# ucbrise/graphtrans

Hardware: AMD Instinct MI355X
Metric: graphs/sec (fwd+bwd) OGBG-Code2 GCN-Virtual b256 (higher is better)
Workload: dtype fp32+bf16; 1 GPU; OGBG-Code2-like synthetic, GraphTrans GCN-Virtual L5 D300 JK=cat cls norm_input, 4 enc layers d128; mode=mixed, graphs_per_gpu=256, global_batch=256, avg_nodes_per_batch=31598, avg_edges_per_batch=87502, parallelism=dp1, step=zero_grad+graph_prep+fwd+loss+bwd+allreduce+AdamW

## Files before the change

### graphtrans_amd/_lib.py

```python
import ctypes as C
import os

import torch

_HERE = os.path.dirname(os.path.abspath(__file__))
LIB_PATH = os.environ.get("GT_LIB_PATH") or os.path.join(_HERE, "libgraphtrans_hip.so")

GT_F32, GT_BF16 = 0, 1
GT_COMPUTE_F32_HIGH = 2
GT_CONV_GCN, GT_CONV_GIN = 0, 1
GT_EDGE_NONE, GT_EDGE_LINEAR, GT_EDGE_TABLES, GT_EDGE_DENSE = 0, 1, 2, 3

_p = C.c_void_p
_i64 = C.c_int64
_i = C.c_int
_f = C.c_float
_sz = C.c_size_t
_u64 = C.c_uint64
_d = C.c_double

SIGNATURES = {
    "gt_version": (_i, []),
    "gt_last_error": (C.c_char_p, []),
    "gt_option_set": (_i, [C.c_char_p, _i]),
    "gt_option_get": (_i, [C.c_char_p]),
    "gt_profile_enable": (_i, [C.c_uint]),
    "gt_profile_resume": (_i, [C.c_uint]),
    "gt_profile_count": (_i64, []),
    "gt_profile_get": (_i, [_i64, C.c_char_p, _i64, C.POINTER(C.c_float), C.POINTER(C.c_int64)]),
    "gt_attr_rank": (_i, [_p, _i64, _p, _p]),
    "gt_collate_workspace_bytes": (_sz, [_i64]),
    "gt_collate": (_i, [_p, _p, _i64, _i64, _i64, _p, _p, _sz, _p]),
    "gt_graph_prep_workspace_bytes": (_sz, [_i64, _i64, _i64]),
    "gt_graph_prep": (_i, [_p, _p, _i64, _i64, _i64, _p, _p, _p, _p, _p, _p, _p, _p, _p, _p, _p, _p, _sz, _p]),
    "gt_aggregate_fwd": (_i, [_i, _i, _i, _p, _i64, _i64, _i64, _p, _p, _p, _p, _p, _p, _p, _i64, _p, _p,
                              C.POINTER(C.c_int32), _i64, _p, _p, _p]),
    "gt_aggregate_bwd_workspace_bytes": (_sz, [_i, _i, _i64, _i64, _i64]),
    "gt_aggregate_bwd": (_i, [_i, _i, _i, _p, _p, _i64, _i64, _i64, _p, _p, _p, _p, _p, _p, _p, _i64, _p, _p,
                              C.POINTER(C.c_int32), _i64, _p, _p, _p, _p, _p, _p, _p, _sz, _p]),
    "gt_pna_aggregate_fwd": (_i, [_p, _p, _i64, _i64, _i, _p, _p, _p, _p, _p, _p, _p]),
    "gt_pna_aggregate_bwd": (_i, [_p, _p, _p, _p, _p, _i64, _i64, _i, _p, _p, _p, _p, _p, _p, _p]),
    "gt_scale_combine_fwd": (_i, [_p, _p, _i64, _i, _i, _i, _p, _p]),
    "gt_scale_combine_bwd": (_i, [_p, _p, _i64, _i, _i, _i, _p, _p]),
    "gt_embed_sum_fwd": (_i, [_i, _p, _p, _p, _p, _i64, _i64, _p, _p]),
    "gt_embed_sum_bwd_workspace_bytes": (_sz, [_i, _p, _i64]),
    "gt_embed_sum_bwd": (_i, [_i, _p, _p, _p, _p, _p, _i64, _i64, _p, _p, _sz, _p]),
    "gt_embed_sort_plan_bytes": (_sz, [_i, _p, _i64]),
    "gt_embed_sort_workspace_bytes": (_sz, [_i, _p, _i64]),
    "gt_embed_sort": (_i, [_i, _p, _p, _p, _p, _i64, _p, _sz, _p, _sz, _p]),
    "gt_embed_sum_bwd_sorted_workspace_bytes": (_sz, [_i, _i64, _i64]),
    "gt_embed_sum_bwd_sorted": (_i, [_i, _p, _p, _i64, _i64, _p, _p, _p, _sz, _p]),
    "gt_segment_bcast_add": (_i, [_i, _p, _p, _p, _i64, _i64, _i64, _p, _p]),
    "gt_segment_sum": (_i, [_i, _p, _p, _p, _i64, _i64, _i64, _p, _p]),
    "gt_seq_layout_packed": (_i, [_p, _i64, _i64, _i, _p, _p, _p, _i64, _p, _p]),
    "gt_segment_sum_workspace_bytes": (_sz, [_i64, _i64]),
    "gt_segment_sum_ws": (_i, [_i, _p, _p, _p, _i64, _i64, _i64, _p, _p, _sz, _p]),
    "gt_seq_gather": (_i, [_i, _p, _p, _p, _p, _i64, _i64, _i64, _i, _i64, _p, _p, _p]),
    "gt_seq_scatter": (_i, [_i, _p, _p, _p, _p, _p, _i64, _i64, _i, _i64, _i64, _p, _p, _p]),
    "gt_batchnorm_workspace_bytes": (_sz, [_i64, _i64]),
    "gt_batchnorm_fwd": (_i, [_i, _p, _p, _p, _p, _p, _p, _f, _f, _i, _i, _p, _i64, _i64, _p, _p, _p, _f, _u64, _p, _sz, _p]),
    "gt_batchnorm_apply": (_i, [_i, _p, _p, _p, _p, _p, _i, _p, _i64, _i64, _p, _f, _u64, _p]),
    "gt_batchnorm_bwd_apply": (_i, [_i, _p, _p, _p, _p, _p, _p, _p, _p, _d, _i, _i64, _i64, _p, _f, _u64, _p]),
    "gt_batchnorm_fwd_bcast": (_i, [_i, _p, _p, _p, _p, _p, _p, _f, _f, _i, _i, _p, _p, _p, _p, _i64, _i64, _p, _p, _p, _f, _u64, _p, _sz, _p]),
    "gt_batchnorm_bwd": (_i, [_i, _p, _p, _p, _p, _p, _p, _i, _i, _i64, _i64, _p, _p, _p, _f, _u64, _p, _sz, _p]),
    "gt_layernorm_fwd": (_i, [_i, _p, _p, _p, _p, _f, _f, _u64, _i64, _i64, _p, _p, _p, _p]),
    "gt_layernorm_bwd_workspace_bytes": (_sz, [_i64, _i64]),
    "gt_layernorm_bwd": (_i, [_i, _p, _p, _p, _p, _p, _p, _f, _u64, _i64, _i64, _p, _p, _p, _p, _p, _sz, _p]),
    "gt_linear_fwd": (_i, [_i, _i, _i, _p, _p, _p, _p, _i64, _i64, _i64, _i, _f, _u64, _p]),
    "gt_colsum_rows_f32": (_i, [_i, _p, _p, _i64, _i64, _p, _p]),
    "gt_seq_token_rows_layernorm": (_i, [_i, _p, _p, _p, _p, _i64, _i64, _i, _i64, _i64, _p, _p, _p, _p, _f, _p, _p, _p, _p]),
    "gt_seq_token_rows": (_i, [_i, _p, _p, _p, _p, _i64, _i64, _i, _i64, _i64, _p, _p, _p]),
    "gt_defer_begin": (_i, [_p, _sz]),
    "gt_defer_limit": (_i, [_sz]),
    "gt_defer_take": (_p, [_sz]),
    "gt_defer_push": (_i, [_p, _i, _i64, _i64, _p, _p, _i64, _i64, _p]),
    "gt_defer_push_strided": (_i, [_p, _i, _i64, _i64, _p, _i64]),
    "gt_defer_room": (_i, [_i]),
    "gt_defer_flush": (_i, [_p]),
    "gt_defer_end": (_i, []),
    "gt_linear_rows_ok": (_i, [_i, _i, _i, _p, _i64, _i64, _i64]),
    "gt_linear_products": (_i, [_i, _i, _i, _i, _p, _i64, _i64, _i64]),
    "gt_linear_set_rows": (_i, [_p]),
    "gt_linear_rows_layernorm_ok": (_i, [_i64]),
    "gt_linear_set_rows_layernorm": (_i, [_p, _p, _p, _f, _p, _p, _p]),
    "gt_linear_fwd_ld": (_i, [_i, _i, _i, _p, _p, _p, _p, _i64, _i64, _i64, _i64, _i, _f, _u64, _p]),
    "gt_linear_bwd_ld": (_i, [_i, _i, _i, _p, _p, _p, _p, _p, _p, _p, _p, _p, _i64, _i64, _i64, _i64, _f, _p, _sz, _p]),
    "gt_adamw_chunk_elems": (_i, []),
    "gt_adamw_step": (_i, [_p, _p, _p, _i64, _i64, _i, _i, _p, _f, _f, _f, _f, _f, _i64, _p, _p]),
    "gt_grad_sqnorm": (_i, [_p, _p, _p, _i64, _i64, _i, _i, _p, _p, _p]),
    "gt_grad_clip_coef": (_i, [_p, _i64, _f, _p, _p]),
    "gt_linear_fwd_gelu": (_i, [_i, _i, _i, _p, _p, _p, _p, _p, _i64, _i64, _i64, _i64, _i64, _f, _u64, _p]),
    "gt_linear_bwd_mul": (_i, [_i, _i, _i, _p, _p, _p, _p, _p, _p, _p, _p, _p, _i64, _i64, _i64, _i64, _i64, _p, _sz, _p]),
    "gt_stream_create": (_p, [_i]),
    "gt_stream_destroy": (None, [_p]),
    "gt_stream_priority_range": (_i, [C.POINTER(_i), C.POINTER(_i)]),
    "gt_linear_bwd_dw_forked": (_i, [_i, _i, _i, _p, _p, _p, _p, _p, _p, _i64, _i64, _i64, _i64, _i64, _f, _p, _sz, _p]),
    "gt_linear_bwd_mul_dw_forked": (_i, [_i, _i, _i, _p, _p, _p, _p, _p, _p, _i64, _i64, _i64, _i64, _i64, _p, _sz, _p]),
    "gt_linear_bwd_wt": (_i, [_i, _i, _i, _p, _p, _p, _p, _p, _p, _p, _p, _p, _p, _i64, _i64, _i64, _f, _p, _sz, _p]),
    "gt_transpose": (_i, [_p, _p, _i64, _i64, _p]),
    "gt_bn_sync_set": (_i, [_p, _p, _i]),
    "gt_vn_update_bwd_dt0": (_p, [_p, _p]),
    "gt_linear_bwd_bcast_ok": (_i, [_i, _i, _i, _p, _i64, _i64, _i64]),
    "gt_linear_bwd_bcast": (_i, [_p, _p]),
    "gt_linear_cat2_ok": (_i, [_i, _p, _i64, _i64, _i64, _i64]),
    "gt_linear_fwd_cat2": (_i, [_i, _i, _p, _i64, _i64, _p, _i64, _i64, _p, _p, _p, _i64, _i64, _i64, _p]),
    "gt_linear_bwd_cat2": (_i, [_i, _i, _p, _i64, _i64, _p, _i64, _i64, _p, _p, _p, _i64, _p, _i64, _p, _p, _i64, _i64, _i64, _p, _sz, _p]),
    "gt_w3_image_bytes": (_sz, [_i64, _i64]),
    "gt_w3_images": (_i, [_i, _p, _p, _p, _p, _p, _p]),
    "gt_w3_bind": (_i, [_i, _p, _p, _p, _p, _p]),
    "gt_w3_unbind": (_i, []),
    "gt_w1_image_bytes": (_sz, [_i64, _i64]),
    "gt_w1_images": (_i, [_i, _p, _p, _p, _p, _p, _p]),
    "gt_w1_bind": (_i, [_i, _p, _p, _p, _p, _p]),
    "gt_w1_unbind": (_i, []),
    "gt_linear_layernorm_fwd_ok": (_i, [_i, _i, _p, _i64, _i64, _i64]),
    "gt_linear_bwd_dx_layernorm_ok": (_i, [_i, _i, _p, _i64, _i64, _i64]),
    "gt_linear_bwd_dx_layernorm_workspace_bytes": (_sz, [_i64, _i64, _i64]),
    "gt_linear_bwd_dx_layernorm": (_i, [_i, _i, _p, _p, _p, _p, _i64, _i64, _i64, _p, _p, _p, _p, _p, _f, _u64, _p, _p, _p, _p, _p, _sz, _p]),
    "gt_layernorm_bwd_finish": (_i, [_p, _i, _i64, _p, _p, _p]),
    "gt_linear_layernorm_fwd": (_i, [_i, _i, _p, _p, _p, _p, _i64, _i64, _i64, _p, _p, _p, _f, _f, C.c_uint64, _p, _p, _p, _p]),
    "gt_linear_bwd_gate_out_ok": (_i, [_i, _i, _i, _p, _i64, _i64, _i64]),
    "gt_linear_bwd_gate_out": (_i, [_i, _i, _i, _p, _p, _p, _p, _p, _p, _p, _p, _p, _i64, _i64, _i64, _i64, _i64, _f, _p, _sz, _p]),
    "gt_dropout": (_i, [_i, _p, _p, _i64, _f, _u64, _p]),
    "gt_linear_bwd_bnstats_ok": (_i, [_i, _i, _i, _i64]),
    "gt_linear_bwd_bnstats_rows": (_i64, [_i64]),
    "gt_linear_bwd_bnstats_rows_for": (_i64, [_i, _i, _i, _p, _i64, _i64, _i64]),
    "gt_linear_bwd_bnstats": (_i, [_p, _i64, _p, _p, _p, _p, _i, _p]),
    "gt_batchnorm_bwd_parts": (_i, [_i, _p, _p, _p, _p, _p, _p, _i, _i, _i64, _i64, _p, _p, _p, _p, _i64, _p]),
    "gt_overlap_dw_begin": (_i, [_p, _p]),
    "gt_overlap_dw_sync": (_i, []),
    "gt_overlap_dw_release": (_i, [_p, _sz]),
    "gt_overlap_dw_urgent": (_i, [_i]),
    "gt_overlap_dw_fork": (_p, [_p, C.c_uint]),
    "gt_overlap_dw_booked": (None, [_p, _sz]),
    "gt_overlap_dw_end": (_i, []),
    "gt_linear_fwd_ld2": (_i, [_i, _i, _i, _p, _p, _p, _p, _i64, _i64, _i64, _i64, _i64, _i, _f, _u64, _p]),
    "gt_linear_fwd_grouped": (_i, [_i, _i, _i, _p, _p, _p, _p, _i64, _i64, _i64, _i64, _i64, _i, _i64, _i64, _i, _f, _u64, _p]),
    "gt_linear_bwd_grouped_workspace_bytes": (_sz, [_i, _i64, _i64, _i64, _i]),
    "gt_linear_bwd_grouped": (_i, [_i, _i, _i, _p, _p, _p, _p, _p, _p, _p, _p, _p, _i64, _i64, _i64, _i64, _i64, _i, _i64, _i64, _f,
                                   _p, _sz, _p]),
    "gt_linear_bwd_ld2": (_i, [_i, _i, _i, _p, _p, _p, _p, _p, _p, _p, _p, _p, _i64, _i64, _i64, _i64, _i64, _f, _p, _sz, _p]),
    "gt_xent_fwd": (_i, [_p, _i64, _i64, _i64, _i64, _p, _i64, _p, _p, _p, _p, _p]),
    "gt_xent_bwd": (_i, [_p, _p, _p, _p, _i64, _p, _i64, _i64, _i64, _i64, _p, _p]),
    "gt_bce_masked_fwd": (_i, [_p, _p, _i64, _i64, _i64, _i64, _p, _p, _p, _p, _p]),
    "gt_bce_masked_bwd": (_i, [_p, _p, _p, _p, _i64, _i64, _i64, _i64, _p, _p]),
    "gt_linear_bwd_workspace_bytes": (_sz, [_i, _i64, _i64, _i64]),
    "gt_linear_bwd": (_i, [_i, _i, _i, _p, _p, _p, _p, _p, _p, _p, _p, _p, _i64, _i64, _i64, _f, _p, _sz, _p]),
    "gt_encoder_layer_saved_bytes": (_sz, [_p]),
    "gt_encoder_layer_workspace_bytes": (_sz, [_p]),
    "gt_encoder_layer_grad_elems": (_i64, [_p]),
    "gt_encoder_layer_fwd": (_i, [_p, _p, _p, _p, _p]),
    "gt_encoder_layer_bwd": (_i, [_p, _p, _p, _p, _p, _p, _p, _sz, _p]),
    "gt_gcn_layer_saved_bytes": (_sz, [_p]),
    "gt_gcn_layer_workspace_bytes": (_sz, [_p]),
    "gt_gcn_layer_grad_elems": (_i64, [_p]),
    "gt_gcn_layer_fwd": (_i, [_p, _p, _p, _p, _p, _p, _p, _sz, _p]),
    "gt_gcn_layer_bwd": (_i, [_p, _p, _p, _p, _p, _p, _p, _p, _p, _sz, _p]),
    "gt_vn_update_saved_bytes": (_sz, [_p]),
    "gt_vn_update_workspace_bytes": (_sz, [_p]),
    "gt_vn_update_grad_elems": (_i64, [_p]),
    "gt_vn_update_fwd": (_i, [_p, _p, _p, _p, _p, _p, _sz, _p]),
    "gt_vn_update_bwd": (_i, [_p, _p, _p, _p, _p, _p, _p, _p, _sz, _p]),
    "gt_event_create": (_p, []),
    "gt_event_destroy": (None, [_p]),
    "gt_event_record": (_i, [_p, _p]),
    "gt_stream_wait_event": (_i, [_p, _p]),
    "gt_gin_layer_saved_bytes": (_sz, [_p]),
    "gt_gin_layer_workspace_bytes": (_sz, [_p]),
    "gt_gin_layer_grad_elems": (_i64, [_p]),
    "gt_gin_layer_fwd": (_i, [_p, _p, _p, _p, _p, _p, _p, _sz, _p]),
    "gt_gin_layer_bwd": (_i, [_p, _p, _p, _p, _p, _p, _p, _p, _p, _sz, _p]),
    "gt_add3": (_i, [_p, _p, _p, _i64, _p, _p]),
    "gt_copy2d": (_i, [_p, _i64, _p, _i64, _i64, _i64, _p]),
    "gt_repitch": (_i, [_p, _i64, _p, _i64, _i64, _i, _p]),
    "gt_rows_gather": (_i, [_i, _p, _p, _i64, _i64, _p, _p]),
    "gt_rows_scatter": (_i, [_i, _p, _p, _i64, _i64, _i64, _p, _p]),
    "gt_seq_layout_packed_host": (_i, [_p, _i64, _i64, _i, _p, _sz, _p]),
    "gt_pna_layer_saved_bytes": (_sz, [_p]),
    "gt_pna_layer_workspace_bytes": (_sz, [_p]),
    "gt_pna_layer_grad_elems": (_i64, [_p]),
    "gt_pna_layer_fwd": (_i, [_p, _p, _p, _p, _p, _sz, _p]),
    "gt_pna_layer_bwd": (_i, [_p, _p, _p, _p, _p, _p, _p, _sz, _p]),
    "gt_pna_scales": (_i, [_p, _i64, _i, _p, _f, _f, _p, _p]),
    "gt_gather_f32": (_i, [_p, _p, _p, _i64, _p]),
    "gt_pna_aggregate_fwd_uv": (_i, [_p, _p, _i64, _i64, _i, _p, _p, _p, _p, _p, _p, _p]),
    "gt_pna_aggregate_bwd_uv": (_i, [_p, _p, _p, _p, _p, _i64, _i64, _i, _p, _p, _p, _p, _p, _p, _p]),
    "gt_rows_take": (_i, [_i, _p, _p, _i64, _i64, _p, _p]),
    "gt_rows_put": (_i, [_i, _p, _p, _i64, _i64, _i64, _p, _p]),
    "gt_rows_add": (_i, [_i, _p, _p, _i64, _i64, _p, _p]),
    "gt_attn_fwd_last": (_i, [_i, _p, _p, _p, _i64, _i64, _i, _p, _i64, _i64, _i64, _f, _f, _u64, _p]),
    "gt_attn_bwd_last": (_i, [_i, _p, _p, _p, _p, _p, _p, _i64, _i64, _i, _p, _i64, _i64, _i64, _p, _i64, _f, _f, _u64, _p]),
    "gt_encoder_layer_pooled_saved_bytes": (_sz, [_p]),
    "gt_encoder_layer_pooled_workspace_bytes": (_sz, [_p]),
    "gt_encoder_layer_pooled_fwd": (_i, [_p, _p, _p, _p, _p, _p]),
    "gt_encoder_layer_pooled_bwd": (_i, [_p, _p, _p, _p, _p, _p, _p, _p, _sz, _p]),
    "gt_model_ctx_bytes": (_sz, []),
    "gt_model_abi_sizes": (_i, [_p]),
    "gt_model_grad_ranges": (_i, [_p, _p, _p]),
    "gt_model_prepare": (_i, [_p, _p, _p, _p]),
    "gt_model_forward": (_i, [_p, _p, _p, _p, _p]),
    "gt_model_backward": (_i, [_p, _p, _p, _p, _p, _i, _p]),
    "gt_seq_gather_cls32": (_i, [_i, _p, _p, _p, _p, _i64, _i64, _i64, _i, _i64, _p, _p]),
    "gt_colsum_f32": (_i, [_i, _p, _i64, _i64, _p, _p]),
    "gt_attn_head_dim_ok": (_i, [_i, _i64, _i]),
    "gt_attn_fwd": (_i, [_i, _p, _p, _p, _i64, _i64, _i, _p, _i64, _i64, _i64, _p, _i64, _p, _p, _f, _f, _f, _u64, _p]),
    "gt_attn_bwd": (_i, [_i, _p, _p, _p, _p, _p, _p, _i64, _i64, _i, _p, _i64, _i64, _i64, _p, _i64, _p, _p, _f, _f, _f,
                         _u64, _p]),
}

_lib = None


def lib():
    global _lib
    if _lib is None:
        if not os.path.exists(LIB_PATH):
            raise RuntimeError(
                f"{LIB_PATH} is missing: build it with `python -m graphtrans_amd.build` "
                "(graphtrans_amd has no CPU or eager fallback)")
        h = C.CDLL(LIB_PATH)
        for name, (res, args) in SIGNATURES.items():
            try:
                fn = getattr(h, name)
            except AttributeError:
                if not os.environ.get("GT_LIB_PATH"):
                    raise
                continue
            fn.restype = res
            fn.argtypes = args
        if os.environ.get("GT_F32_GEMM", "split") == "exact":
            h.gt_option_set(b"attn_f32_exact", 1)
        _lib = h
    return _lib


class KernelTimer:

    def __init__(self, names):
        self.names = set(names)
        self.records = []

    def summary(self):
        torch.cuda.synchronize()
        out = {}
# ... 66 lines not shown
```

### graphtrans_amd/csrc/common.hip

```cpp
#include <stdarg.h>
#include <atomic>
#include <mutex>
#include <string.h>

#include "gt_common.h"

static thread_local char g_err[512] = "";

void gt_set_error(const char* fmt, ...) {
  va_list ap;
  va_start(ap, fmt);
  vsnprintf(g_err, sizeof(g_err), fmt, ap);
  va_end(ap);
}

extern "C" int gt_version(void) { return 100;  }
extern "C" const char* gt_last_error(void) { return g_err; }

#include <mutex>
#include <vector>

namespace {
struct ProfRecord {
  const char* name;
  hipEvent_t e0, e1;
  int64_t dims[6];
};
std::mutex g_prof_mu;
std::vector<ProfRecord> g_prof;
std::vector<hipEvent_t> g_pool;
size_t g_pool_next = 0;
unsigned g_prof_mask = 0;
constexpr size_t POOL_EVENTS = 16384;
}

unsigned gt_prof_mask() { return g_prof_mask; }

int64_t gt_prof_begin(const char* name, hipStream_t stream, const int64_t* dims, int ndims) {
  ProfRecord r{};
  r.name = name;
  for (int i = 0; i < 6; ++i) r.dims[i] = i < ndims ? dims[i] : 0;
  std::lock_guard<std::mutex> lk(g_prof_mu);
  if (g_pool_next + 2 > g_pool.size()) return -1;
  r.e0 = g_pool[g_pool_next++];
  r.e1 = g_pool[g_pool_next++];
  (void)hipEventRecord(r.e0, stream);
  g_prof.push_back(r);
  return (int64_t)g_prof.size() - 1;
}

void gt_prof_end(int64_t id, hipStream_t stream) {
  if (id < 0) return;
  std::lock_guard<std::mutex> lk(g_prof_mu);
  if ((size_t)id < g_prof.size()) (void)hipEventRecord(g_prof[id].e1, stream);
}

namespace {
std::atomic<int> g_options[GT_OPT_COUNT];
const char* const OPTION_NAMES[GT_OPT_COUNT] = {"attn_f32_exact", "bnstats_rows_kernel", "lin_ring"};
int option_id(const char* name) {
  if (name)
    for (int i = 0; i < GT_OPT_COUNT; ++i)
      if (strcmp(name, OPTION_NAMES[i]) == 0) return i;
  return -1;
}
}
int gt_opt(int id) { return g_options[id].load(std::memory_order_relaxed); }
extern "C" int gt_option_set(const char* name, int value) {
  const int id = option_id(name);
  if (id < 0) { gt_set_error("gt_option_set: unknown option '%s'", name ? name : "(null)"); return GT_ERR_INVALID_ARG; }
  return g_options[id].exchange(value < 0 ? 0 : value);
}
extern "C" int gt_option_get(const char* name) {
  const int id = option_id(name);
  if (id < 0) { gt_set_error("gt_option_get: unknown option '%s'", name ? name : "(null)"); return GT_ERR_INVALID_ARG; }
  return gt_opt(id);
}

extern "C" int gt_profile_enable(unsigned mask) {
  std::lock_guard<std::mutex> lk(g_prof_mu);
  if (mask) {
    g_prof.clear();
    g_pool_next = 0;
    while (g_pool.size() < POOL_EVENTS) {
      hipEvent_t e;
      if (hipEventCreate(&e) != hipSuccess) break;
      g_pool.push_back(e);
    }
  }
  g_prof_mask = mask;
  return GT_OK;
}

extern "C" int gt_profile_resume(unsigned mask) {
  std::lock_guard<std::mutex> lk(g_prof_mu);
  g_prof_mask = mask;
  return GT_OK;
}

extern "C" int64_t gt_profile_count(void) {
  std::lock_guard<std::mutex> lk(g_prof_mu);
  return (int64_t)g_prof.size();
}

extern "C" int gt_profile_get(int64_t i, char* name_out, int64_t name_cap, float* ms, int64_t* dims6) {
  std::lock_guard<std::mutex> lk(g_prof_mu);
  if (i < 0 || (size_t)i >= g_prof.size() || !name_out || !ms || !dims6) return GT_ERR_INVALID_ARG;
  const ProfRecord& r = g_prof[i];
  snprintf(name_out, (size_t)name_cap, "%s", r.name);
  if (hipEventElapsedTime(ms, r.e0, r.e1) != hipSuccess) return GT_ERR_LAUNCH;
  for (int k = 0; k < 6; ++k) dims6[k] = r.dims[k];
  return GT_OK;
}


extern "C" void* gt_stream_create(int level) {
  int least = 0, greatest = 0;
  (void)hipDeviceGetStreamPriorityRange(&least, &greatest);
  const int prio = level < 0 ? greatest : (level > 0 ? least : 0);
  hipStream_t st = nullptr;
  if (hipStreamCreateWithPriority(&st, hipStreamNonBlocking, prio) != hipSuccess) return nullptr;
  return st;
}
extern "C" void gt_stream_destroy(void* stream) {
  if (stream) (void)hipStreamDestroy((hipStream_t)stream);
}
extern "C" int gt_stream_priority_range(int* least, int* greatest) {
  return hipDeviceGetStreamPriorityRange(least, greatest) == hipSuccess ? GT_OK : GT_ERR_LAUNCH;
}

extern "C" void* gt_event_create(void) {
  hipEvent_t ev = nullptr;
  if (hipEventCreateWithFlags(&ev, hipEventDisableTiming) != hipSuccess) return nullptr;
  return ev;
}
extern "C" void gt_event_destroy(void* event) {
  if (event) (void)hipEventDestroy((hipEvent_t)event);
}
extern "C" int gt_event_record(void* event, gt_stream_t stream) {
  GT_CHECK_ARG(event, "null event");
  if (hipEventRecord((hipEvent_t)event, (hipStream_t)stream) != hipSuccess) { gt_set_error("gt_event_record failed"); return GT_ERR_LAUNCH; }
  return GT_OK;
// ... 7 lines not shown
```

### graphtrans_amd/csrc/gt_common.h

```cpp
#pragma once
#include <hip/hip_runtime.h>
#ifdef GT_DEBUG_SKIP
#include <cstdlib>
#include <cstring>
static inline bool gt_dbg_skip(const char* kernel) {
  static const char* e = getenv("GT_SKIP");
  if (!e || !*e) return false;
  const char* p = e;
  while (*p) {
    const char* q = strchr(p, ',');
    const size_t n = q ? (size_t)(q - p) : strlen(p);
    char buf[128];
    if (n > 0 && n < sizeof(buf)) {
      memcpy(buf, p, n);
      buf[n] = 0;
      if (strstr(kernel, buf)) return true;
    }
    if (!q) break;
    p = q + 1;
  }
  return false;
}
static __global__ void gt_dbg_empty_kernel() {}
static inline bool gt_dbg_empty() {
  static const bool on = [] { const char* e = getenv("GT_EMPTY"); return e && *e && *e != '0'; }();
  return on;
}
#undef hipLaunchKernelGGL
#define hipLaunchKernelGGL(k, g, b, l, s, ...)                                                              \
  do {                                                                                                      \
    if (gt_dbg_empty()) hipLaunchKernelGGLInternal(gt_dbg_empty_kernel, dim3(1), dim3(64), 0, (s));        \
    else if (!gt_dbg_skip(#k)) hipLaunchKernelGGLInternal((k), (g), (b), (l), (s), __VA_ARGS__);           \
  } while (0)
#endif
#include <stdint.h>
#include <stdio.h>

#include <initializer_list>

#include "../../include/graphtrans_hip.h"

static inline int gt_compute_base(int compute) { return compute == GT_COMPUTE_F32_HIGH ? GT_F32 : compute; }

#define GT_WAVE 64

void gt_set_error(const char* fmt, ...);

#define GT_CHECK_ARG(cond, msg)                     \
  do {                                              \
    if (!(cond)) {                                  \
      gt_set_error("%s: %s", __func__, msg);        \
      return GT_ERR_INVALID_ARG;                    \
    }                                               \
  } while (0)

#define GT_CHECK_LAUNCH()                                                        \
  do {                                                                           \
    hipError_t e__ = hipGetLastError();                                          \
    if (e__ != hipSuccess) {                                                     \
      gt_set_error("%s: launch failed: %s", __func__, hipGetErrorString(e__));   \
      return GT_ERR_LAUNCH;                                                      \
    }                                                                            \
  } while (0)

enum { GT_PROF_AGGREGATE = 1, GT_PROF_ATTENTION = 2, GT_PROF_LINEAR = 4, GT_PROF_NORM = 8, GT_PROF_SEGMENT = 16,
       GT_PROF_GEMM_KERNEL = 32 };
unsigned gt_prof_mask();
enum { GT_OPT_ATTN_F32_EXACT = 0, GT_OPT_BNSTATS_ROWS_KERNEL = 1, GT_OPT_LIN_RING = 2, GT_OPT_COUNT };
int gt_opt(int id);
int64_t gt_prof_begin(const char* name, hipStream_t stream, const int64_t* dims, int ndims);
void gt_prof_end(int64_t id, hipStream_t stream);
struct GtProfScope {
  int64_t id;
  hipStream_t stream;
  GtProfScope(unsigned cat, const char* name, gt_stream_t st, std::initializer_list<int64_t> dims)
      : id(-1), stream((hipStream_t)st) {
    if (gt_prof_mask() & cat) id = gt_prof_begin(name, stream, dims.begin(), (int)dims.size());
  }
  ~GtProfScope() { gt_prof_end(id, stream); }
};

static inline int64_t gt_cdiv(int64_t a, int64_t b) { return (a + b - 1) / b; }

typedef uint16_t gt_bf16;

__device__ __forceinline__ float gt_bf16_to_f32(gt_bf16 v) { return __uint_as_float(((uint32_t)v) << 16); }
__device__ __forceinline__ gt_bf16 gt_f32_to_bf16(float f) {
  uint32_t u = __float_as_uint(f);
  if ((u & 0x7fffffffu) > 0x7f800000u) return (gt_bf16)((u >> 16) | 0x40);
  u += 0x7fffu + ((u >> 16) & 1u);
  return (gt_bf16)(u >> 16);
}

typedef __bf16 gt_v2bf __attribute__((ext_vector_type(2)));
typedef float gt_v2f __attribute__((ext_vector_type(2)));
__device__ __forceinline__ uint32_t gt_pack_bf16(float lo, float hi) {
  const gt_v2f f = {lo, hi};
  return __builtin_bit_cast(uint32_t, __builtin_convertvector(f, gt_v2bf));
}

__device__ __forceinline__ void gt_gelu(float z, float& y, float& dydz) {
  const float cdf = 0.5f * (1.f + erff(z * 0.70710678118654752f));
  y = z * cdf;
  dydz = cdf + z * 0.3989422804014327f * __expf(-0.5f * z * z);
}
__device__ __forceinline__ float gt_gate(float dy, float m, float inv_keep) {
  return inv_keep == 0.f ? dy * m : (m > 0.f ? dy * inv_keep : 0.f);
}

struct gt_f4 {
  float x, y, z, w;
};

template <typename T>
__device__ __forceinline__ float4 gt_load4(const T* p);
template <>
__device__ __forceinline__ float4 gt_load4<float>(const float* p) {
  return *reinterpret_cast<const float4*>(p);
}
template <>
__device__ __forceinline__ float4 gt_load4<gt_bf16>(const gt_bf16* p) {
  uint2 u = *reinterpret_cast<const uint2*>(p);
  float4 r;
  r.x = __uint_as_float(u.x << 16);
  r.y = __uint_as_float(u.x & 0xffff0000u);
  r.z = __uint_as_float(u.y << 16);
  r.w = __uint_as_float(u.y & 0xffff0000u);
  return r;
}
template <typename T>
__device__ __forceinline__ void gt_store4(T* p, float4 v);
template <>
__device__ __forceinline__ void gt_store4<float>(float* p, float4 v) {
  *reinterpret_cast<float4*>(p) = v;
}
template <>
__device__ __forceinline__ void gt_store4<gt_bf16>(gt_bf16* p, float4 v) {
  uint2 u;
  u.x = gt_pack_bf16(v.x, v.y);
  u.y = gt_pack_bf16(v.z, v.w);
  *reinterpret_cast<uint2*>(p) = u;
}

__device__ __forceinline__ float4 gt_zero4() { return make_float4(0.f, 0.f, 0.f, 0.f); }
__device__ __forceinline__ float4 gt_add4(float4 a, float4 b) { return make_float4(a.x + b.x, a.y + b.y, a.z + b.z, a.w + b.w); }
__device__ __forceinline__ float4 gt_scale4(float4 a, float s) { return make_float4(a.x * s, a.y * s, a.z * s, a.w * s); }
__device__ __forceinline__ float4 gt_fma4(float4 a, float s, float4 c) {
  return make_float4(fmaf(a.x, s, c.x), fmaf(a.y, s, c.y), fmaf(a.z, s, c.z), fmaf(a.w, s, c.w));
}
__device__ __forceinline__ float4 gt_relu4(float4 a) {
  return make_float4(fmaxf(a.x, 0.f), fmaxf(a.y, 0.f), fmaxf(a.z, 0.f), fmaxf(a.w, 0.f));
}
```

### graphtrans_amd/csrc/layers.hip

```cpp
#include "host_seq.h"
#include "linear_call.h"

namespace {

struct Bump {
  char* base;
  size_t off;
  explicit Bump(void* p) : base(reinterpret_cast<char*>(p)), off(0) {}
  void* take(size_t bytes) {
    void* p = base ? base + off : nullptr;
    off += (bytes + 255) & ~size_t(255);
    return p;
  }
};

struct EncRowsSaved {
  void *a, *x1, *f1, *f2, *g1;
  float *st1, *st2;
};
struct EncSaved {
  void *qkv, *ctx, *xp, *ctxp;
  float* lse;
  EncRowsSaved r;
  size_t bytes;
// ... 364 lines not shown
  Bump b(p);
  GinWork w;
  w.m = mlp2_work(L->compute, L->N, L->D, b);
  w.m.lin_ws1 = b.take(w.m.lin_ws_bytes);
  w.m.w1_t = L->w1_t; w.m.w2_t = L->w2_t;
  w.d_x = b.take((size_t)L->N * L->D * 4);
  w.agg_ws_bytes = gt_aggregate_bwd_workspace_bytes(GT_CONV_GIN, L->edge_mode, L->D, L->edge_cols, L->table_rows);
  w.agg_ws = b.take(w.agg_ws_bytes);
  w.seg_ws_bytes = gt_segment_sum_workspace_bytes(L->N, L->D);
  w.seg_ws = b.take(w.seg_ws_bytes);
  w.bytes = b.off;
  return w;
}

}

extern "C" size_t gt_encoder_layer_saved_bytes(const gt_encoder_layer* L) { return L ? enc_saved(L, false, nullptr).bytes : 0; }
extern "C" size_t gt_encoder_layer_workspace_bytes(const gt_encoder_layer* L) { return L ? enc_work(L, false, nullptr).bytes : 0; }
extern "C" int64_t gt_encoder_layer_grad_elems(const gt_encoder_layer* L) {
  if (!L) return 0;
  const int64_t d = L->d_model, F = L->ffn;
  return 3 * d * d + 3 * d + d * d + d + F * d + F + d * F + d + 4 * d;
}

extern "C" int gt_encoder_layer_fwd(const gt_encoder_layer* L, const void* x, void* y, void* saved, gt_stream_t st) {
  GT_TRY(enc_check("gt_encoder_layer_fwd", L));
  GT_CHECK_ARG(x && y && saved, "null buffer");
  if (L->rows == 0) return GT_OK;
  const EncSaved s = enc_saved(L, false, saved);
  const int t = L->dtype, c = t == GT_BF16 ? GT_BF16 : L->compute;
  const int64_t R = L->rows, d = L->d_model;
  const float p = L->training ? L->dropout_p : 0.f;
  const float scale = 1.0f / sqrtf((float)(d / L->nhead));
  GT_TRY(gt_linear_fwd(t, t, c, x, L->in_w, L->in_b, s.qkv, R, 3 * d, d, 0, 0.f, 0, st));
  GT_TRY(gt_attn_fwd(t, s.qkv, s.ctx, s.lse, R, d, L->nhead, L->seq_desc, L->num_seqs, L->row_stride, L->max_npos,
                     L->work_items, L->num_work, nullptr, nullptr, 0.f, scale, p, L->seed, st));
  return enc_rows_fwd(L, R, x, s.ctx, s.r, y, st);
}

extern "C" int gt_encoder_layer_bwd(const gt_encoder_layer* L, const void* x, const void* dy, const void* saved, void* dx,
                                    float* grads, void* workspace, size_t workspace_bytes, gt_stream_t st) {
  GT_TRY(enc_check("gt_encoder_layer_bwd", L));
  GT_CHECK_ARG(x && dy && saved && dx && grads && workspace, "null buffer");
  const EncWork w = enc_work(L, false, workspace);
  if (workspace_bytes < w.bytes) { gt_set_error("gt_encoder_layer_bwd: workspace too small"); return GT_ERR_WORKSPACE; }
  if (L->rows == 0) return GT_OK;
  const EncSaved s = enc_saved(L, false, const_cast<void*>(saved));
  const EncGrads g = enc_grads(L, grads);
  const int t = L->dtype, c = t == GT_BF16 ? GT_BF16 : L->compute;
  const int64_t R = L->rows, d = L->d_model;
  const float p = L->training ? L->dropout_p : 0.f;
  const float scale = 1.0f / sqrtf((float)(d / L->nhead));
  GT_TRY(enc_rows_bwd(L, R, x, s.ctx, dy, s.r, w.r, g, w.d_ctx, dx, true, st));
  GT_TRY(gt_attn_bwd(t, s.qkv, s.ctx, w.d_ctx, s.lse, w.delta, w.d_qkv, R, d, L->nhead, L->seq_desc, L->num_seqs,
                     L->row_stride, L->max_npos, L->work_items, L->num_work, nullptr, nullptr, 0.f, scale, p, L->seed, st));
  GT_TRY(gt_linear_bwd_dw_forked(t, t, c, x, L->in_w, w.d_qkv, nullptr, g.in_w, g.in_b, R, 3 * d, d, d, 3 * d, 0.f, w.lin_ws_in,
                                 w.lin_ws_in_bytes, st));
  return gt_linear_bwd(t, t, c, x, L->in_w, w.d_qkv, nullptr, dx, nullptr, dx, nullptr, nullptr, R, 3 * d, d, 0.f, w.lin_ws_in,
                       w.lin_ws_in_bytes, st);
}

extern "C" size_t gt_gcn_layer_saved_bytes(const gt_gcn_layer* L) { return L ? gcn_saved(L, nullptr).bytes : 0; }
extern "C" size_t gt_gcn_layer_workspace_bytes(const gt_gcn_layer* L) { return L ? gcn_work(L, nullptr).bytes : 0; }
extern "C" int64_t gt_gcn_layer_grad_elems(const gt_gcn_layer* L) {
  if (!L) return 0;
  return L->D * L->D + 2 * L->D + edge_w_elems(L) + edge_b_elems(L) + 2 * L->D;
}

extern "C" int gt_gcn_layer_fwd(const gt_gcn_layer* L, const void* h_in, const void* vn, void* x_out, void* y, void* saved,
                                void* workspace, size_t workspace_bytes, gt_stream_t st) {
  GT_TRY(gcn_check("gt_gcn_layer_fwd", L));
  GT_CHECK_ARG(h_in && y && saved && workspace, "null buffer");
  GT_CHECK_ARG(!L->has_vn || L->x_has_vn || (vn && x_out), "virtual-node layer needs vn and x_out");
  const GcnWork w = gcn_work(L, workspace);
  if (workspace_bytes < w.bytes) { gt_set_error("gt_gcn_layer_fwd: workspace too small"); return GT_ERR_WORKSPACE; }
  if (L->N == 0) return GT_OK;
  const GcnSaved s = gcn_saved(L, saved);
  const void* x;
  GT_TRY(conv_add_vn(L, h_in, vn, x_out, &x, st));
  GT_TRY(gt_linear_fwd(GT_F32, GT_F32, L->compute, x, L->lin_w, L->lin_b, s.lin, L->N, L->D, L->D, 0, 0.f, 0, st));
  if (L->ev_graph_ready) GT_TRY(gt_stream_wait_event(st, L->ev_graph_ready));
  GT_TRY(gt_aggregate_fwd(GT_CONV_GCN, L->edge_mode, GT_F32, s.lin, L->N, L->E, L->D, L->in_ptr, L->in_src, L->in_eid, L->deg,
                          L->dis, L->root, L->edge_attr, L->edge_cols, L->edge_w, L->edge_b, L->tab_off, L->table_rows, nullptr, s.agg, st));
  GT_TRY(gt_batchnorm_fwd_bcast(GT_F32, s.agg, L->bn_w, L->bn_b, L->bn_rm, L->bn_rv, L->training ? L->bn_nbt : nullptr,
                                L->bn_momentum, L->bn_eps, L->training, L->relu, L->residual ? x : nullptr, L->vn_next,
                                L->vn_next ? L->node_graph : nullptr, L->vn_next ? L->ev_vn_next : nullptr, L->N, L->D, y, s.stats,
                                s.stats + L->D, L->dropout_p, L->seed, w.bn_ws, w.bn_ws_bytes, st));
  return GT_OK;
}

extern "C" int gt_gcn_layer_bwd(const gt_gcn_layer* L, const void* x, const void* dy, const void* dx_extra,
                                const void* saved, void* d_h_in, void* d_vn, float* grads, void* workspace,
                                size_t workspace_bytes, gt_stream_t st) {
  GT_TRY(gcn_check("gt_gcn_layer_bwd", L));
  GT_CHECK_ARG(x && dy && saved && d_h_in && grads && workspace, "null buffer");
  const GcnWork w = gcn_work(L, workspace);
  if (workspace_bytes < w.bytes) { gt_set_error("gt_gcn_layer_bwd: workspace too small"); return GT_ERR_WORKSPACE; }
  if (L->N == 0) return GT_OK;
  const GcnSaved s = gcn_saved(L, const_cast<void*>(saved));
  const GcnGrads g = gcn_grads(L, grads);
  if (L->bn_part_in && L->bn_nparts_in > 0 && L->dropout_p == 0.f)
    GT_TRY(gt_batchnorm_bwd_parts(GT_F32, s.agg, dy, L->bn_w, L->bn_b, s.stats, s.stats + L->D, L->training, L->relu, L->N, L->D,
                                  w.d_agg, g.bn_w, g.bn_b, L->bn_part_in, L->bn_nparts_in, st));
  else
    GT_TRY(gt_batchnorm_bwd(GT_F32, s.agg, dy, L->bn_w, L->bn_b, s.stats, s.stats + L->D, L->training, L->relu, L->N, L->D,
                            w.d_agg, g.bn_w, g.bn_b, L->dropout_p, L->seed, w.bn_ws, w.bn_ws_bytes, st));
  GT_TRY(gt_aggregate_bwd(GT_CONV_GCN, L->edge_mode, GT_F32, s.lin, w.d_agg, L->N, L->E, L->D, L->out_ptr, L->out_dst,
                          L->out_eid, L->deg, L->dis, L->root, L->edge_attr, L->edge_cols, L->edge_w, L->edge_b, L->tab_off,
                          L->table_rows, nullptr, w.d_lin, g.root, g.edge_w, g.edge_b, nullptr, w.agg_ws, w.agg_ws_bytes, st));
  if (L->ev_dx_wait) GT_TRY(gt_stream_wait_event(st, L->ev_dx_wait));
  LinBwd lin{GT_F32, GT_F32, L->compute, x, L->lin_w, w.d_lin, nullptr, dx_extra, L->residual ? dy : nullptr, d_h_in, g.lin_w, g.lin_b,
               L->N, L->D, L->D, L->D, L->D, 1, 0, 0, 0.f, w.lin_ws, w.lin_ws_bytes, (hipStream_t)st};
  lin.weight_t = L->lin_wt;
  if (L->prev_saved && L->prev_bn_part) {
    const GcnSaved ps = gcn_saved(L, const_cast<void*>(L->prev_saved));
    lin.bn_x = (const float*)ps.agg; lin.bn_ldx = L->D; lin.bn_mean = ps.stats; lin.bn_rstd = ps.stats + L->D;
    lin.bn_w = L->prev_bn_w; lin.bn_b = L->prev_bn_b; lin.bn_relu = L->prev_relu; lin.bn_part = L->prev_bn_part;
  }
  lin.bcast = L->dx_bcast; lin.bcast_idx = L->dx_bcast_idx;
  GT_TRY(lin_bwd(lin));
  return conv_pool_d_vn(L, d_h_in, d_vn, w.seg_ws, w.seg_ws_bytes, st);
}

extern "C" size_t gt_vn_update_saved_bytes(const gt_vn_update* L) { return L ? mlp2_saved(L->B, L->D, nullptr).bytes : 0; }
extern "C" size_t gt_vn_update_workspace_bytes(const gt_vn_update* L) { return L ? vn_work(L, nullptr).bytes : 0; }
extern "C" int64_t gt_vn_update_grad_elems(const gt_vn_update* L) { return L ? 4 * L->D * L->D + 9 * L->D : 0; }

extern "C" int gt_vn_update_fwd(const gt_vn_update* L, const void* x, const void* vn, void* vn_out, void* saved,
                                void* workspace, size_t workspace_bytes, gt_stream_t st) {
  GT_CHECK_ARG(L && x && vn && vn_out && saved && workspace, "null buffer");
  GT_CHECK_ARG(L->D > 0 && L->D % 4 == 0 && L->B > 0, "bad sizes");
  const VnWork w = vn_work(L, workspace);
  if (workspace_bytes < w.bytes) { gt_set_error("gt_vn_update_fwd: workspace too small"); return GT_ERR_WORKSPACE; }
  const int64_t B = L->B, D = L->D;
  const Mlp2Saved s = mlp2_saved(B, D, saved);
  GT_TRY(gt_segment_sum_ws(GT_F32, x, vn, L->graph_ptr, L->N, B, D, s.in, w.seg_ws, w.seg_ws_bytes, st));
  GT_TRY(mlp2_fwd_head(L, B, s, w.m.bn_ws, w.m.bn_ws_bytes, st));
  GT_TRY(gt_batchnorm_fwd(GT_F32, s.z2, L->bn2_w, L->bn2_b, L->bn2_rm, L->bn2_rv, L->training ? L->bn2_nbt : nullptr,
                          L->bn_momentum, L->bn_eps, L->training, 1, L->residual ? vn : nullptr, B, D, vn_out, s.st2,
                          s.st2 + D, L->dropout_p, L->seed, w.m.bn_ws, w.m.bn_ws_bytes, st));
  return GT_OK;
}

extern "C" int gt_vn_update_bwd(const gt_vn_update* L, const void* d_vn_out, const void* saved, const void* d_x_add,
                                void* d_x, void* d_vn, float* grads, void* workspace, size_t workspace_bytes,
                                gt_stream_t st) {
  GT_CHECK_ARG(L && d_vn_out && saved && d_vn && grads && workspace, "null buffer");
  const VnWork w = vn_work(L, workspace);
  if (workspace_bytes < w.bytes) { gt_set_error("gt_vn_update_bwd: workspace too small"); return GT_ERR_WORKSPACE; }
  const int64_t B = L->B, D = L->D;
  const Mlp2Saved s = mlp2_saved(B, D, const_cast<void*>(saved));
  const Mlp2Grads g = mlp2_grads(D, grads);
  void* d_t0 = w.m.d_in;
  const bool defer = L->ev_dx_done != nullptr;
  GT_TRY(gt_batchnorm_bwd(GT_F32, s.z2, d_vn_out, L->bn2_w, L->bn2_b, s.st2, s.st2 + D, L->training, 1, B, D, w.m.d_z2, g.bn2_w,
                          g.bn2_b, L->dropout_p, L->seed, w.m.bn_ws, w.m.bn_ws_bytes, st));
  GT_TRY(mlp2_bwd(L, B, s, g, w.m, defer, st));
  if (d_x) GT_TRY(gt_segment_bcast_add(GT_F32, d_x_add, d_t0, L->node_graph, L->N, B, D, d_x, st));
  if (L->residual)
    GT_TRY(gt_segment_bcast_add(GT_F32, d_t0, d_vn_out, L->identity_graph, B, B, D, d_vn, st));
  else if (d_vn != d_t0)
    (void)hipMemcpyAsync(d_vn, d_t0, (size_t)B * D * 4, hipMemcpyDeviceToDevice, (hipStream_t)st);
  if (defer) {
    GT_TRY(gt_event_record(L->ev_dx_done, st));
    GT_TRY(mlp2_bwd_dw(L, B, s, g, w.m, st));
  }
  return GT_OK;
}

extern "C" const float* gt_vn_update_bwd_dt0(const gt_vn_update* L, void* workspace) {
  if (!L || !workspace) return nullptr;
  return (const float*)vn_work(L, workspace).m.d_in;
}

extern "C" size_t gt_gin_layer_saved_bytes(const gt_gin_layer* L) { return L ? mlp2_saved(L->N, L->D, nullptr).bytes : 0; }
extern "C" size_t gt_gin_layer_workspace_bytes(const gt_gin_layer* L) { return L ? gin_work(L, nullptr).bytes : 0; }
extern "C" int64_t gt_gin_layer_grad_elems(const gt_gin_layer* L) {
  if (!L) return 0;
  const int64_t D = L->D;
  return GIN_EPS_SLOT + edge_w_elems(L) + edge_b_elems(L) + 4 * D * D + 9 * D;
}

extern "C" int gt_gin_layer_fwd(const gt_gin_layer* L, const void* h_in, const void* vn, void* x_out, void* y, void* saved,
                                void* workspace, size_t workspace_bytes, gt_stream_t st) {
  GT_TRY(gin_check("gt_gin_layer_fwd", L));
  GT_CHECK_ARG(h_in && y && saved && workspace, "null buffer");
  GT_CHECK_ARG(!L->has_vn || L->x_has_vn || (vn && x_out), "virtual-node layer needs vn and x_out");
  const GinWork w = gin_work(L, workspace);
  if (workspace_bytes < w.bytes) { gt_set_error("gt_gin_layer_fwd: workspace too small"); return GT_ERR_WORKSPACE; }
  if (L->N == 0) return GT_OK;
  const int64_t N = L->N, D = L->D;
  const Mlp2Saved s = mlp2_saved(N, D, saved);
  const void* x;
  GT_TRY(conv_add_vn(L, h_in, vn, x_out, &x, st));
  GT_TRY(gt_aggregate_fwd(GT_CONV_GIN, L->edge_mode, GT_F32, x, N, L->E, D, L->in_ptr, L->in_src, L->in_eid, nullptr, nullptr,
                          L->eps, L->edge_attr, L->edge_cols, L->edge_w, L->edge_b, L->tab_off, L->table_rows, nullptr, s.in, st));
  GT_TRY(mlp2_fwd_head(L, N, s, w.m.bn_ws, w.m.bn_ws_bytes, st));
  GT_TRY(gt_batchnorm_fwd_bcast(GT_F32, s.z2, L->bn_w, L->bn_b, L->bn_rm, L->bn_rv, L->training ? L->bn_nbt : nullptr, L->bn_momentum,
                                L->bn_eps, L->training, L->relu, L->residual ? x : nullptr, L->vn_next,
                                L->vn_next ? L->node_graph : nullptr, L->vn_next ? L->ev_vn_next : nullptr, N, D, y, s.st2, s.st2 + D,
                                L->dropout_p, L->seed, w.m.bn_ws, w.m.bn_ws_bytes, st));
  return GT_OK;
}

extern "C" int gt_gin_layer_bwd(const gt_gin_layer* L, const void* x, const void* dy, const void* dx_extra,
                                const void* saved, void* d_h_in, void* d_vn, float* grads, void* workspace,
                                size_t workspace_bytes, gt_stream_t st) {
  GT_TRY(gin_check("gt_gin_layer_bwd", L));
  GT_CHECK_ARG(x && dy && saved && d_h_in && grads && workspace, "null buffer");
  const GinWork w = gin_work(L, workspace);
  if (workspace_bytes < w.bytes) { gt_set_error("gt_gin_layer_bwd: workspace too small"); return GT_ERR_WORKSPACE; }
  if (L->N == 0) return GT_OK;
  const int64_t N = L->N, D = L->D;
  const Mlp2Saved s = mlp2_saved(N, D, const_cast<void*>(saved));
  const GinGrads g = gin_grads(L, grads);
  GT_TRY(gt_batchnorm_bwd(GT_F32, s.z2, dy, L->bn_w, L->bn_b, s.st2, s.st2 + D, L->training, L->relu, N, D, w.m.d_z2, g.m.bn2_w,
                          g.m.bn2_b, L->dropout_p, L->seed, w.m.bn_ws, w.m.bn_ws_bytes, st));
  GT_TRY(mlp2_bwd(L, N, s, g.m, w.m, false, st));
  const bool adds = dx_extra || L->residual;
  void* dx_conv = adds ? w.d_x : d_h_in;
  GT_TRY(gt_aggregate_bwd(GT_CONV_GIN, L->edge_mode, GT_F32, x, w.m.d_in, N, L->E, D, L->out_ptr, L->out_dst, L->out_eid, nullptr,
                          nullptr, L->eps, L->edge_attr, L->edge_cols, L->edge_w, L->edge_b, L->tab_off, L->table_rows, nullptr,
                          dx_conv, g.eps, g.edge_w, g.edge_b, nullptr, w.agg_ws, w.agg_ws_bytes, st));
  if (L->ev_dx_wait) GT_TRY(gt_stream_wait_event(st, L->ev_dx_wait));
  if (adds) {
    const float* e1 = dx_extra ? (const float*)dx_extra : (const float*)dy;
    const float* e2 = (dx_extra && L->residual) ? (const float*)dy : nullptr;
    GT_TRY(gt_add3((const float*)w.d_x, e1, e2, N * D, (float*)d_h_in, st));
  }
  return conv_pool_d_vn(L, d_h_in, d_vn, w.seg_ws, w.seg_ws_bytes, st);
}

extern "C" size_t gt_encoder_layer_pooled_saved_bytes(const gt_encoder_layer* L) { return L ? enc_saved(L, true, nullptr).bytes : 0; }
extern "C" size_t gt_encoder_layer_pooled_workspace_bytes(const gt_encoder_layer* L) { return L ? enc_work(L, true, nullptr).bytes : 0; }

extern "C" int gt_encoder_layer_pooled_fwd(const gt_encoder_layer* L, const void* x, const int64_t* pool_rows, void* y_pool, void* saved,
                                           gt_stream_t st) {
  GT_TRY(enc_check("gt_encoder_layer_pooled_fwd", L));
  GT_CHECK_ARG(x && pool_rows && y_pool && saved, "null buffer");
  if (L->rows == 0 || L->num_seqs == 0) return GT_OK;
  const EncSaved s = enc_saved(L, true, saved);
  const int t = L->dtype, c = t == GT_BF16 ? GT_BF16 : L->compute;
  const int64_t R = L->rows, B = L->num_seqs, d = L->d_model;
  const float p = L->training ? L->dropout_p : 0.f;
  const float scale = 1.0f / sqrtf((float)(d / L->nhead));
  GT_TRY(gt_linear_fwd(t, t, c, x, L->in_w, L->in_b, s.qkv, R, 3 * d, d, 0, 0.f, 0, st));
  GT_TRY(gt_attn_fwd_last(t, s.qkv, s.ctx, s.lse, R, d, L->nhead, L->seq_desc, L->num_seqs, L->row_stride, L->max_npos, scale, p, L->seed, st));
  GT_TRY(gt_rows_take(t, x, pool_rows, B, d, s.xp, st));
  GT_TRY(gt_rows_take(t, s.ctx, pool_rows, B, d, s.ctxp, st));
  return enc_rows_fwd(L, B, s.xp, s.ctxp, s.r, y_pool, st);
}

extern "C" int gt_encoder_layer_pooled_bwd(const gt_encoder_layer* L, const void* x, const int64_t* pool_rows, const void* dy_pool,
                                           const void* saved, void* dx, float* grads, void* workspace, size_t workspace_bytes,
                                           gt_stream_t st) {
  GT_TRY(enc_check("gt_encoder_layer_pooled_bwd", L));
  GT_CHECK_ARG(x && pool_rows && dy_pool && saved && dx && grads && workspace, "null buffer");
  const EncWork w = enc_work(L, true, workspace);
  if (workspace_bytes < w.bytes) { gt_set_error("gt_encoder_layer_pooled_bwd: workspace too small"); return GT_ERR_WORKSPACE; }
  if (L->rows == 0 || L->num_seqs == 0) return GT_OK;
  const EncSaved s = enc_saved(L, true, const_cast<void*>(saved));
  const EncGrads g = enc_grads(L, grads);
  const int t = L->dtype, c = t == GT_BF16 ? GT_BF16 : L->compute;
  const int64_t R = L->rows, B = L->num_seqs, d = L->d_model;
  const float p = L->training ? L->dropout_p : 0.f;
  const float scale = 1.0f / sqrtf((float)(d / L->nhead));
  GT_TRY(enc_rows_bwd(L, B, s.xp, s.ctxp, dy_pool, s.r, w.r, g, w.d_ctxp, w.d_xp, false, st));
  GT_TRY(gt_rows_put(t, w.d_ctxp, pool_rows, B, R, d, w.d_ctx, st));
  if (hipMemsetAsync(w.d_qkv, 0, (size_t)R * 3 * d * gt_elt_bytes(t), (hipStream_t)st) != hipSuccess) {
    gt_set_error("gt_encoder_layer_pooled_bwd: memset failed");
    return GT_ERR_LAUNCH;
  }
  GT_TRY(gt_attn_bwd_last(t, s.qkv, s.ctx, w.d_ctx, s.lse, w.delta, w.d_qkv, R, d, L->nhead, L->seq_desc, L->num_seqs, L->row_stride,
                          L->max_npos, L->work_items, L->num_work, scale, p, L->seed, st));
  GT_TRY(gt_linear_bwd_dw_forked(t, t, c, x, L->in_w, w.d_qkv, nullptr, g.in_w, g.in_b, R, 3 * d, d, d, 3 * d, 0.f, w.lin_ws_in,
                                 w.lin_ws_in_bytes, st));
  GT_TRY(gt_linear_bwd(t, t, c, x, L->in_w, w.d_qkv, nullptr, nullptr, nullptr, dx, nullptr, nullptr, R, 3 * d, d, 0.f, w.lin_ws_in,
                       w.lin_ws_in_bytes, st));
  return gt_rows_add(t, w.d_xp, pool_rows, B, d, dx, st);
}
// ... 120 lines not shown
```

### graphtrans_amd/csrc/model.hip

```cpp
#include <algorithm>
#include <cstring>
#include <vector>

#include "host_seq.h"
#include "linear_call.h"

namespace {

constexpr int MAXL = GT_MODEL_MAX_LAYERS;
constexpr int MAXT = GT_MODEL_MAX_TABLES;
constexpr int64_t PREP_MIN_EDGES = 400000;
constexpr uint64_t SEED_STEP = 0x9E3779B97F4A7C15ULL;

struct Bump {
  size_t off = 0;
  size_t take(size_t bytes) {
    size_t o = off;
    off = (o + bytes + 255) / 256 * 256;
    return o;
  }
};
inline size_t c4(size_t n) { return (n + 3) / 4 * 4; }

struct Ctx {
  uint32_t magic;
  int prepared, forwarded, stages_done;
  gt_model_batch in;
  int64_t rows, max_npos, num_work;
  int exact, lay_host;
  int compute, tdt;
  size_t tsz;
  int use_prep, build_graph, build_layout_dev;
  void* stage_ptr;
  void* stage_event;
  size_t lay_bytes, lay_o_last, lay_o_work;
  gt_gcn_layer gcn[MAXL];
  gt_gin_layer gin[MAXL];
  gt_pna_layer pna[MAXL];
  gt_vn_update vn[MAXL];
  gt_encoder_layer enc[MAXL];
  size_t o_rowmap;
  int fuse_rows;
  size_t o_h[MAXL + 1], o_x0, o_vn[MAXL], o_vn_saved[MAXL], o_conv_saved[MAXL], o_cat, o_hn, o_tok, o_xin, o_st0, o_xe[MAXL],
      o_enc_saved[MAXL], o_hgin, o_sto, o_eplan, o_esort_ws, o_ne_x, o_ne_w, o_hg, o_ws, o_ws2, o_wt[MAXL], o_g2t_wt;
  size_t o_scales, q_dimg;
  size_t o_graph_ptr, o_node_graph, o_in_ptr, o_out_ptr, o_idx, o_dd, o_status, o_prep_ws, o_lay, o_lay_meta;
  size_t ws_bytes, ws2_bytes, eplan_bytes, esort_ws_bytes, prep_ws_bytes, arena_bytes;
  int cat2, want_wt, esort, late_wait;
  int64_t Kc;
  char* base;
  const int32_t *graph_ptr, *node_graph, *seq_desc, *work_items;
  const int64_t* last_rows;
  const void *xptr[MAXL], *enc_in[MAXL], *pre_out, *first, *node_rep, *h_last;
  const float *g2t_wt, *ne_x, *ne_w;
  int T;
  const int64_t* e_idx[MAXT + 1];
  int64_t e_str[MAXT + 1], e_clamp[MAXT + 1], e_rows[MAXT + 1];
  size_t q_d_hgin, q_dyp;
  size_t q_defer, defer_bytes, defer_small;
  size_t q_d_hg, q_dtok[2], q_d_hn, q_d_cls, q_d_rep, q_dA, q_dB, q_dC, q_dJ, q_dvn[4], q_ne_dw, q_bnpart[MAXL], q_heads_ws,
      q_ws[2], q_ws2, q_ws3;
  size_t bws_bytes, heads_ws_bytes, seg_ws_bytes, barena_bytes;
  int fuse_bn, bn_rows, ov;
  char* bb;
  int slot;
  void *dy, *d_vn_next, *d_h0;
};
constexpr uint32_t CTX_MAGIC = 0x67744d31u;

inline gt_gcn_layer* gcn_static(const gt_model* m) { return (gt_gcn_layer*)m->conv_layers; }
inline gt_gin_layer* gin_static(const gt_model* m) { return (gt_gin_layer*)m->conv_layers; }
inline gt_pna_layer* pna_static(const gt_model* m) { return (gt_pna_layer*)m->conv_layers; }

int model_check(const char* fn, const gt_model* m) {
  if (!m) { gt_set_error("%s: null model", fn); return GT_ERR_INVALID_ARG; }
  if (m->L < 1 || m->L > MAXL || m->n_enc < 1 || m->n_enc > MAXL || m->n_tables < 0 || m->n_tables > MAXT) {
    gt_set_error("%s: layer / table counts out of range", fn);
    return GT_ERR_INVALID_ARG;
  }
  if (!m->conv_layers || (m->n_enc && !m->enc) || (m->has_vn && m->L > 1 && !m->vn)) { gt_set_error("%s: null descriptor array", fn); return GT_ERR_INVALID_ARG; }
  if (m->D <= 0 || m->D % 4 || m->d <= 0 || m->d % 8) { gt_set_error("%s: bad widths", fn); return GT_ERR_INVALID_ARG; }
  if (m->conv != GT_CONV_GCN && m->conv != GT_CONV_GIN && m->conv != GT_CONV_PNA) { gt_set_error("%s: bad conv kind", fn); return GT_ERR_INVALID_ARG; }
  if (m->conv == GT_CONV_PNA && (m->has_vn || m->jk_cat || !m->residual || !m->pna_src || !m->pna_img || !m->pna_map || !m->pna_inv)) {
    gt_set_error("%s: the PNA stack runs without a virtual node, with JK = last, the residual connection and its weight images", fn);
    return GT_ERR_INVALID_ARG;
  }
  return GT_OK;
}

struct HostLayout {
  int64_t rows, max_npos, num_work;
  size_t o_last, o_work, bytes;
};
HostLayout layout_sizes(const int64_t* n, int64_t B, int64_t max_input_len, int cls, std::vector<int64_t>* kvlen_out) {
  int64_t S = 0;
  for (int64_t b = 0; b < B; ++b) S = std::max(S, n[b]);
  S = std::min(S, max_input_len);
  HostLayout h{};
  int64_t cnt[8] = {0, 0, 0, 0, 0, 0, 0, 0};
  std::vector<int64_t>& kv = *kvlen_out;
  kv.resize((size_t)B);
  for (int64_t b = 0; b < B; ++b) {
    kv[(size_t)b] = std::min(n[b], S) + cls;
    h.rows += kv[(size_t)b];
    h.max_npos = std::max(h.max_npos, kv[(size_t)b]);
  }
  std::vector<int32_t> order((size_t)B);
  for (int64_t b = 0; b < B; ++b) order[(size_t)b] = (int32_t)b;
  std::stable_sort(order.begin(), order.end(), [&](int32_t a, int32_t c) { return kv[(size_t)a] > kv[(size_t)c]; });
  for (int64_t r = 0; r < B; ++r) cnt[r % 8] += (kv[(size_t)order[(size_t)r]] + 63) / 64;
  int64_t wpx = 0;
  for (int x = 0; x < 8; ++x) wpx = std::max(wpx, cnt[x]);
  h.num_work = B ? 8 * wpx : 0;
  const size_t nd = (size_t)B * 16, nl = (size_t)B * 8, nw = (size_t)h.num_work * 8;
  h.o_last = (nd + 15) / 16 * 16;
  h.o_work = (h.o_last + nl + 15) / 16 * 16;
  h.bytes = std::max(h.o_work + nw, (size_t)16);
  return h;
}
void layout_fill(const std::vector<int64_t>& kv, int64_t B, const HostLayout& h, char* dst) {
  int32_t* desc = (int32_t*)dst;
  int64_t* last = (int64_t*)(dst + h.o_last);
  int32_t* work = (int32_t*)(dst + h.o_work);
  int64_t row = 0;
  for (int64_t b = 0; b < B; ++b) {
    const int64_t k = kv[(size_t)b];
    desc[b * 4 + 0] = (int32_t)row;
    desc[b * 4 + 1] = (int32_t)k;
    desc[b * 4 + 2] = 0;
    desc[b * 4 + 3] = (int32_t)k;
    last[b] = row + k - 1;
// ... 35 lines not shown
  }
};

size_t conv_saved_bytes(const gt_model* m, const Ctx* c, int l) {
  if (m->conv == GT_CONV_PNA) return gt_pna_layer_saved_bytes(&c->pna[l]);
  return m->conv == GT_CONV_GIN ? gt_gin_layer_saved_bytes(&c->gin[l]) : gt_gcn_layer_saved_bytes(&c->gcn[l]);
}
size_t conv_ws_bytes(const gt_model* m, const Ctx* c, int l) {
  if (m->conv == GT_CONV_PNA) return gt_pna_layer_workspace_bytes(&c->pna[l]);
  return m->conv == GT_CONV_GIN ? gt_gin_layer_workspace_bytes(&c->gin[l]) : gt_gcn_layer_workspace_bytes(&c->gcn[l]);
}

}

extern "C" size_t gt_model_ctx_bytes(void) { return sizeof(Ctx); }

extern "C" int gt_model_grad_ranges(const gt_model* m, int64_t* lo3, int64_t* hi3) {
  GT_TRY(model_check("gt_model_grad_ranges", m));
  GT_CHECK_ARG(lo3 && hi3, "null output");
  const int64_t gnn_lo = m->has_vn ? m->off_vn_emb : m->off_conv[0];
  lo3[0] = m->off_g2t_w; hi3[0] = m->grad_total;
  lo3[1] = gnn_lo;       hi3[1] = m->off_g2t_w;
  lo3[2] = 0;            hi3[2] = gnn_lo;
  return GT_OK;
}

extern "C" int gt_model_prepare(const gt_model* m, const gt_model_batch* b, void* ctx_, gt_model_sizes* out) {
  GT_TRY(model_check("gt_model_prepare", m));
  GT_CHECK_ARG(b && ctx_ && out, "null argument");
  GT_CHECK_ARG(b->N > 0 && b->B > 0 && b->E >= 0, "empty batch");
  GT_CHECK_ARG(b->x && ((b->edge_index && b->batch) || b->graph_ptr), "null batch arrays");
  Ctx* c = (Ctx*)ctx_;
  memset(c, 0, sizeof(Ctx));
  c->magic = CTX_MAGIC;
  c->in = *b;
  const int64_t N = b->N, E = b->E, B = b->B, D = m->D, d = m->d;
  const int L = m->L, nenc = m->n_enc;
  c->compute = b->compute;
  c->tdt = b->tdt;
  c->tsz = gt_elt_bytes(b->tdt);
  const size_t tsz = c->tsz;
  const int cls = m->with_cls ? 1 : 0;

  c->build_graph = b->graph_ptr == nullptr;
  c->use_prep = (m->st_prep && b->sizes_host && c->build_graph && E >= PREP_MIN_EDGES) ? 1 : 0;
  if (b->seq_desc) {
    c->rows = b->rows; c->max_npos = b->max_npos; c->num_work = b->num_work; c->exact = b->lay_exact;
  } else if (b->sizes_host) {
    std::vector<int64_t> kv;
    const HostLayout h = layout_sizes(b->sizes_host, B, m->max_input_len, cls, &kv);
    c->rows = h.rows; c->max_npos = h.max_npos; c->num_work = h.num_work; c->exact = 1;
    c->lay_host = 1;
    c->lay_bytes = h.bytes; c->lay_o_last = h.o_last; c->lay_o_work = h.o_work;
    gt_stage_ring* ring = b->ring;
    GT_CHECK_ARG(ring && ring->base && ring->slots > 0 && ring->slots <= 64, "host-built layout needs a staging ring");
    if ((int64_t)h.bytes > ring->slot_bytes) { gt_set_error("gt_model_prepare: layout of %zu bytes exceeds the staging slot", h.bytes); return GT_ERR_WORKSPACE; }
    const int i = ring->next;
    ring->next = (i + 1) % ring->slots;
    if (ring->events[i]) (void)hipEventSynchronize((hipEvent_t)ring->events[i]);
    c->stage_ptr = (char*)ring->base + (size_t)i * (size_t)ring->slot_bytes;
    c->stage_event = ring->events[i];
    layout_fill(kv, B, h, (char*)c->stage_ptr);
  } else {
    c->build_layout_dev = 1;
    c->rows = N + B * cls;
    c->max_npos = std::min<int64_t>(m->max_input_len, N) + cls;
    c->num_work = B + c->rows / 64;
    c->exact = 0;
  }
  const int64_t rows = c->rows;

  const int training = b->training ? 1 : 0;
  auto fill_conv = [&](auto& g, int l) {
    g.N = N; g.E = E; g.B = B;
    g.has_vn = m->has_vn; g.relu = l != L - 1; g.residual = m->residual;
    g.training = training; g.compute = c->compute;
    g.dropout_p = training ? b->gnn_p : 0.f;
    g.seed = b->gnn_seed + SEED_STEP * (uint64_t)(2 * l + 1);
    g.edge_attr = (g.edge_mode != GT_EDGE_NONE && E > 0) ? b->edge_attr : nullptr;
    g.ev_x_ready = nullptr;
    g.ev_dx_wait = (m->st_vn && m->has_vn && l < L - 1) ? m->ev_extra[l] : nullptr;
    g.x_has_vn = m->has_vn;
    g.vn_next = nullptr; g.ev_vn_next = nullptr;
  };
  for (int l = 0; l < L; ++l) {
    if (m->conv == GT_CONV_GCN) {
      gt_gcn_layer& g = c->gcn[l];
      g = gcn_static(m)[l];
      fill_conv(g, l);
      g.lin_wt = nullptr;
      g.prev_saved = nullptr; g.prev_bn_w = g.prev_bn_b = nullptr; g.prev_bn_part = nullptr; g.bn_part_in = nullptr;
      g.prev_relu = 0; g.bn_nparts_in = 0; g.ev_graph_ready = nullptr;
      g.dx_bcast = nullptr; g.dx_bcast_idx = nullptr;
    } else if (m->conv == GT_CONV_PNA) {
      gt_pna_layer& g = c->pna[l];
      g = pna_static(m)[l];
      g.N = N; g.E = E;
      g.training = training; g.compute = c->compute;
      g.dropout_p = training ? b->gnn_p : 0.f;
      g.seed = b->gnn_seed + SEED_STEP * (uint64_t)(2 * l + 1);
    } else {
      gt_gin_layer& g = c->gin[l];
      g = gin_static(m)[l];
      fill_conv(g, l);
      g.w1_t = g.w2_t = nullptr;
    }
  }
  const int nvn = m->has_vn ? L - 1 : 0;
  for (int l = 0; l < nvn; ++l) {
    gt_vn_update& v = c->vn[l];
    v = m->vn[l];
    v.N = N; v.B = B;
    v.residual = m->residual; v.training = training; v.compute = c->compute;
    v.dropout_p = training ? b->gnn_p : 0.f;
    v.seed = b->gnn_seed + SEED_STEP * (uint64_t)(2 * l + 2);
    v.identity_graph = b->ident_B;
    v.ev_dx_done = (m->st_vn && m->vn_defer_dw) ? m->ev_extra[l] : nullptr;
  }
  for (int i = 0; i < nenc; ++i) {
    gt_encoder_layer& e = c->enc[i];
    e = m->enc[i];
    e.rows = rows;
    e.dtype = c->tdt; e.compute = c->compute; e.training = training;
    e.num_seqs = B; e.row_stride = 1; e.max_npos = c->max_npos;
    e.num_work = c->num_work;
    e.dropout_p = training ? b->enc_p : 0.f;
    e.seed = b->enc_seed + SEED_STEP * (uint64_t)(i + 1);
  }

  Bump a;
  const size_t ND4 = (size_t)N * D * 4;
  for (int l = 0; l <= L; ++l) c->o_h[l] = a.take(ND4);
  if (m->has_vn) {
    c->o_x0 = a.take(m->vn0_in_embed ? 0 : ND4);
    for (int l = 0; l < L; ++l) c->o_vn[l] = a.take((size_t)B * D * 4);
    for (int l = 0; l < nvn; ++l) c->o_vn_saved[l] = a.take(gt_vn_update_saved_bytes(&c->vn[l]));
  }
  for (int l = 0; l < L; ++l) c->o_conv_saved[l] = a.take(conv_saved_bytes(m, c, l));
  const int64_t Kc = m->jk_cat ? 2 * D : D;
  c->Kc = Kc;
  c->cat2 = 0;
  if (m->jk_cat && b->use_w3) {
    BindGuard guard;
    GT_TRY(bind_images(m, c));
    c->cat2 = gt_linear_cat2_ok(c->compute, m->g2t_w, N, d, D, D) ? 1 : 0;
  }
  c->o_cat = a.take((m->jk_cat && !c->cat2) ? (size_t)N * Kc * 4 : 0);
  c->o_hn = a.take((size_t)N * d * tsz);
  c->o_rowmap = a.take((size_t)N * 4);
  c->o_tok = a.take((size_t)rows * d * tsz);
  if (m->nin_w) {
    c->o_xin = a.take((size_t)rows * d * tsz);
    c->o_st0 = a.take((size_t)2 * rows * 4);
  }
  for (int i = 0; i < nenc; ++i) c->o_xe[i] = a.take((size_t)(i == nenc - 1 ? B : rows) * d * tsz);
  for (int i = 0; i < nenc; ++i)
    c->o_enc_saved[i] = a.take(i == nenc - 1 ? gt_encoder_layer_pooled_saved_bytes(&c->enc[i]) : gt_encoder_layer_saved_bytes(&c->enc[i]));
  if (m->nout_w) {
    c->o_hgin = a.take((size_t)B * d * 4);
    c->o_sto = a.take((size_t)2 * B * 4);
  }
  c->T = m->embed_kind != 1 ? m->n_tables : 0;
  for (int t = 0; t < c->T; ++t) c->e_rows[t] = m->table_rows[t];
  c->esort = (b->will_bwd && m->embed_sorted && m->embed_kind != 1) ? 1 : 0;
  if (c->esort) {
    c->eplan_bytes = gt_embed_sort_plan_bytes(c->T, c->e_rows, N);
    c->esort_ws_bytes = gt_embed_sort_workspace_bytes(c->T, c->e_rows, N);
    c->o_eplan = a.take(c->eplan_bytes);
    c->o_esort_ws = a.take(c->esort_ws_bytes);
  }
  const int64_t Kp = (int64_t)c4((size_t)m->ne_K);
  if (m->embed_kind == 1 && Kp != m->ne_K) {
    c->o_ne_x = a.take((size_t)N * Kp * 4);
    c->o_ne_w = a.take((size_t)D * Kp * 4);
  }
  c->o_hg = a.take((size_t)B * d * 4);
  if (m->conv == GT_CONV_PNA) c->o_scales = a.take((size_t)N * c->pna[0].S * 4);
  size_t ws = 256, ws2 = 256;
  for (int l = 0; l < L; ++l) ws = std::max(ws, conv_ws_bytes(m, c, l));
  for (int l = 0; l < nvn; ++l) ws2 = std::max(ws2, gt_vn_update_workspace_bytes(&c->vn[l]));
  ws = std::max(ws, ws2);
  c->ws_bytes = ws; c->ws2_bytes = ws2;
  c->o_ws = a.take(ws);
  c->o_ws2 = a.take(ws2);
  const bool have_imgs = b->use_w3 != 0;
  c->want_wt = (m->conv != GT_CONV_PNA && b->will_bwd && gt_compute_base(c->compute) == GT_F32 && N >= 1024 && (!have_imgs || (!m->has_vn && m->conv == GT_CONV_GCN))) ? 1 : 0;
  if (c->want_wt) {
    for (int l = 0; l < L; ++l) c->o_wt[l] = a.take((size_t)(m->conv == GT_CONV_GIN ? 2 : 1) * 2 * D * D * 4);
    c->o_g2t_wt = a.take((size_t)d * Kc * 4);
  }
  if (c->build_graph) {
    c->o_graph_ptr = a.take((size_t)(B + 1) * 4);
    c->o_node_graph = a.take((size_t)N * 4);
    c->o_in_ptr = a.take((size_t)(N + 1) * 4);
    c->o_out_ptr = a.take((size_t)(N + 1) * 4);
    c->o_idx = a.take((size_t)4 * std::max<int64_t>(E, 1) * 4);
    c->o_dd = a.take((size_t)2 * N * 4);
    c->o_status = a.take(4);
    c->prep_ws_bytes = gt_graph_prep_workspace_bytes(N, E, B);
    c->o_prep_ws = a.take(c->prep_ws_bytes);
  }
  if (c->lay_host) c->o_lay = a.take(c->lay_bytes);
  if (c->build_layout_dev) {
    const size_t nd = (size_t)B * 16, nl = (size_t)B * 8, nw = (size_t)std::max<int64_t>(c->num_work, 1) * 8;
    c->lay_o_last = (nd + 15) / 16 * 16;
    c->lay_o_work = (c->lay_o_last + nl + 15) / 16 * 16;
    c->lay_bytes = c->lay_o_work + nw;
    c->o_lay = a.take(c->lay_bytes);
    c->o_lay_meta = a.take(16);
  }
  c->arena_bytes = std::max(a.off, (size_t)256);

  Bump q;
  c->q_d_hg = q.take((size_t)B * d * 4);
  c->q_d_hgin = q.take(m->nout_w ? (size_t)B * d * 4 : 0);
  c->q_dyp = q.take((size_t)B * d * tsz);
  c->q_dtok[0] = q.take((size_t)rows * d * tsz);
  c->q_dtok[1] = q.take((size_t)rows * d * tsz);
  c->q_d_hn = q.take((size_t)N * d * tsz);
  c->q_d_cls = q.take((size_t)B * d * tsz);
  c->q_d_rep = q.take((size_t)N * Kc * 4);
  c->q_dA = q.take(ND4); c->q_dB = q.take(ND4); c->q_dC = q.take(ND4);
  c->q_dJ = q.take(m->jk_cat ? ND4 : 0);
  for (int i = 0; i < 4; ++i) c->q_dvn[i] = q.take((size_t)B * D * 4);
  size_t enc_ws = 256;
  for (int i = 0; i < nenc; ++i)
    enc_ws = std::max(enc_ws, i == nenc - 1 ? gt_encoder_layer_pooled_workspace_bytes(&c->enc[i]) : gt_encoder_layer_workspace_bytes(&c->enc[i]));
  const size_t ln_ws = std::max(gt_layernorm_bwd_workspace_bytes(rows, d), gt_layernorm_bwd_workspace_bytes(B, d));
  const size_t lin_ws = std::max(gt_linear_bwd_workspace_bytes(c->compute, B, m->Nh, d), gt_linear_bwd_workspace_bytes(c->compute, N, d, Kc));
  size_t emb_ws;
  if (m->embed_kind == 1) {
    emb_ws = gt_linear_bwd_workspace_bytes(c->compute, N, D, Kp);
    c->q_ne_dw = q.take(Kp != m->ne_K ? (size_t)D * Kp * 4 : 0);
  } else if (c->esort) {
    emb_ws = gt_embed_sum_bwd_sorted_workspace_bytes(c->T, N, D);
  } else {
    emb_ws = gt_embed_sum_bwd_workspace_bytes(c->T, c->e_rows, D);
  }
  c->bws_bytes = std::max(std::max(std::max(c->ws_bytes, enc_ws), std::max(ln_ws, lin_ws)), emb_ws);
  c->fuse_bn = 0;
  c->bn_rows = 0;
  if (L > 1 && !b->sync_bn && m->conv == GT_CONV_GCN && training && c->gcn[0].dropout_p == 0.f &&
      gt_linear_bwd_bnstats_ok(c->compute, GT_F32, GT_F32, N)) {
    int64_t rows = gt_linear_bwd_bnstats_rows(N);
    bool on_rows_kernel = false;
    if (b->use_w3) {
      BindGuard guard;
      GT_TRY(bind_images(m, c));
      rows = gt_linear_bwd_bnstats_rows_for(c->compute, GT_F32, GT_F32, c->gcn[1].lin_w, N, D, D);
      on_rows_kernel = rows != gt_linear_bwd_bnstats_rows(N);
    }
    if (rows > 0 && (on_rows_kernel || (!m->has_vn && N <= 65536))) {
      c->fuse_bn = 1;
      c->bn_rows = (int)rows;
    }
  }
  for (int l = 0; l + 1 < L; ++l) c->q_bnpart[l] = q.take(c->fuse_bn ? (size_t)c->bn_rows * 2 * D * 4 : 0);
  c->heads_ws_bytes = gt_linear_bwd_workspace_bytes(c->compute, B, m->Nh, d);
  c->q_heads_ws = q.take(c->heads_ws_bytes);
  c->q_ws[0] = q.take(c->bws_bytes);
  c->q_ws[1] = q.take(c->bws_bytes);
  c->q_ws2 = q.take(c->ws2_bytes);
  c->seg_ws_bytes = m->has_vn ? gt_segment_sum_workspace_bytes(N, D) : 0;
  c->q_ws3 = q.take(c->seg_ws_bytes);
  c->q_dimg = q.take(m->conv == GT_CONV_PNA ? (size_t)m->pna_n_img * 4 : 0);
  {
    size_t need = lin_ws + emb_ws + (size_t)(2 * nenc + 2) * ln_ws;
// ... 129 lines not shown
      if (m->conv == GT_CONV_GIN) {
        gt_gin_layer& g = c->gin[l];
        g.w1_t = wt; g.w2_t = wt + 2 * D * D;
        GT_TRY(gt_transpose(g.w1, wt, 2 * D, D, tst));
        GT_TRY(gt_transpose(g.w2, wt + 2 * D * D, D, 2 * D, tst));
      } else {
        c->gcn[l].lin_wt = wt;
        GT_TRY(gt_transpose(c->gcn[l].lin_w, wt, D, D, tst));
      }
    }
    c->g2t_wt = (float*)P(c->o_g2t_wt);
    GT_TRY(gt_transpose(m->g2t_w, (float*)P(c->o_g2t_wt), d, c->Kc, tst));
    if (m->st_dw) GT_TRY(gt_event_record(m->ev_wt[1], tst));
  }
  const int T = c->T;
  c->ne_x = c->ne_w = nullptr;
  if (m->embed_kind == 1) {
    const int64_t K = m->ne_K, Kp = (int64_t)c4((size_t)K);
    const float *nx = (const float*)b.x, *nw = m->ne_w;
    if (Kp != K) {
      GT_TRY(gt_repitch(P(c->o_ne_x), Kp, b.x, K, N, 4, st));
      GT_TRY(gt_repitch(P(c->o_ne_w), Kp, m->ne_w, K, D, 4, st));
      nx = (const float*)P(c->o_ne_x); nw = (const float*)P(c->o_ne_w);
    }
    c->ne_x = nx; c->ne_w = nw;
    GT_TRY(gt_linear_fwd(GT_F32, GT_F32, compute, nx, nw, m->ne_b, P(c->o_h[0]), N, D, Kp, 0, 0.f, 0, st));
  } else {
    const int64_t* x = (const int64_t*)b.x;
    if (m->embed_kind == 2) {
      GT_CHECK_ARG(T == 3 && b.node_depth, "ASTNodeEncoder has three tables and needs node_depth");
      c->e_idx[0] = x; c->e_str[0] = b.x_stride0;
      c->e_idx[1] = x + b.x_stride1; c->e_str[1] = b.x_stride0;
      c->e_idx[2] = b.node_depth; c->e_str[2] = b.depth_stride;
    } else {
      for (int t = 0; t < T; ++t) { c->e_idx[t] = x + (int64_t)t * b.x_stride1; c->e_str[t] = b.x_stride0; }
    }
    const float* tabs[MAXT + 1];
    for (int t = 0; t < T; ++t) { c->e_clamp[t] = m->table_clamp[t]; tabs[t] = m->tables[t]; }
    int Tn = T;
    if (m->vn0_in_embed) {
      c->e_idx[T] = m->zero_i64; c->e_str[T] = 0; c->e_clamp[T] = -1; tabs[T] = m->vn_emb;
      Tn = T + 1;
    }
    GT_TRY(gt_embed_sum_fwd(Tn, c->e_idx, c->e_str, c->e_clamp, tabs, N, D, (float*)P(c->o_h[0]), st));
    if (c->esort) {
      gt_stream_t sst = st;
      if (m->st_dw) {
        sst = m->st_dw;
        GT_TRY(gt_event_record(m->ev_sort[0], st));
        GT_TRY(gt_stream_wait_event(sst, m->ev_sort[0]));
      }
      GT_TRY(gt_embed_sort(T, c->e_idx, c->e_str, c->e_clamp, c->e_rows, N, P(c->o_eplan), c->eplan_bytes, P(c->o_esort_ws),
                           c->esort_ws_bytes, sst));
      if (m->st_dw) GT_TRY(gt_event_record(m->ev_sort[1], sst));
    }
  }
  const bool late_wait = ev_graph && m->conv == GT_CONV_GCN && (!m->has_vn || m->vn0_in_embed);
  if (m->conv == GT_CONV_GCN) c->gcn[0].ev_graph_ready = late_wait ? ev_graph : nullptr;
  if (ev_graph) {
    if (!late_wait) GT_TRY(gt_stream_wait_event(st, ev_graph));
    else if (side) GT_TRY(gt_stream_wait_event(side, ev_graph));
  }
  auto X = [&](int l) -> void* {
    if (!m->has_vn) return P(c->o_h[l]);
    return (l == 0 && !m->vn0_in_embed) ? P(c->o_x0) : P(c->o_h[l]);
  };
  if (m->conv == GT_CONV_PNA)
    GT_TRY(gt_pna_scales(in_ptr, N, c->pna[0].S, m->pna_kinds, m->pna_avg_log, m->pna_avg_lin, (float*)P(c->o_scales), st));
  auto conv_fwd = [&](int l, const void* h_in, const void* vn, void* y) -> int {
    if (m->conv == GT_CONV_PNA) return gt_pna_layer_fwd(&c->pna[l], h_in, y, P(c->o_conv_saved[l]), P(c->o_ws), c->ws_bytes, st);
    if (m->conv == GT_CONV_GIN)
      return gt_gin_layer_fwd(&c->gin[l], h_in, vn, nullptr, y, P(c->o_conv_saved[l]), P(c->o_ws), c->ws_bytes, st);
    return gt_gcn_layer_fwd(&c->gcn[l], h_in, vn, nullptr, y, P(c->o_conv_saved[l]), P(c->o_ws), c->ws_bytes, st);
  };
  if (m->has_vn)
    GT_TRY(gt_segment_bcast_add(GT_F32, nullptr, m->vn_emb, b.zeros_B, B, 1, D, P(c->o_vn[0]), st));
  for (int l = 0; l < L; ++l) {
    if (m->has_vn) {
      const bool last = l == L - 1;
      const void* vn_next = last ? nullptr : P(c->o_vn[l + 1]);
      void* ev_next = (!last && side) ? m->ev_vn[l] : nullptr;
      if (m->conv == GT_CONV_GIN) { c->gin[l].vn_next = vn_next; c->gin[l].ev_vn_next = ev_next; }
      else { c->gcn[l].vn_next = vn_next; c->gcn[l].ev_vn_next = ev_next; }
      if (l == 0 && !m->vn0_in_embed)
        GT_TRY(gt_segment_bcast_add(GT_F32, P(c->o_h[0]), P(c->o_vn[0]), node_graph, N, B, D, P(c->o_x0), st));
      if (!last && side) {
        GT_TRY(gt_event_record(m->ev_x[l], st));
        GT_TRY(gt_stream_wait_event(side, m->ev_x[l]));
        GT_TRY(gt_vn_update_fwd(&c->vn[l], X(l), P(c->o_vn[l]), P(c->o_vn[l + 1]), P(c->o_vn_saved[l]), P(c->o_ws2), c->ws2_bytes, side));
        GT_TRY(gt_event_record(m->ev_vn[l], side));
      } else if (!last) {
        GT_TRY(gt_vn_update_fwd(&c->vn[l], X(l), P(c->o_vn[l]), P(c->o_vn[l + 1]), P(c->o_vn_saved[l]), P(c->o_ws), c->ws_bytes, st));
      }
      GT_TRY(conv_fwd(l, X(l), P(c->o_vn[l]), P(c->o_h[l + 1])));
    } else {
      GT_TRY(conv_fwd(l, P(c->o_h[l]), nullptr, P(c->o_h[l + 1])));
    }
    c->xptr[l] = X(l);
  }
  c->first = X(0);
  c->h_last = P(c->o_h[L]);
  if (ev_w1) GT_TRY(gt_stream_wait_event(st, ev_w1));
  c->fuse_rows = (!b.seq_desc && gt_linear_rows_ok(compute, GT_F32, tdt, m->g2t_w, N, d, c->Kc)) ? 1 : 0;
  void* g2t_out = P(c->o_hn);
  const bool fuse_nin = c->fuse_rows && m->nin_w && gt_linear_rows_layernorm_ok(d);
  LinRowMap map{};
  if (c->fuse_rows) {
    int32_t* rmap = (int32_t*)P(c->o_rowmap);
    if (fuse_nin) {
      float* st0 = (float*)P(c->o_st0);
      GT_TRY(gt_seq_token_rows_layernorm(tdt, m->cls, graph_ptr, node_graph, c->seq_desc, B, 1, m->with_cls ? 1 : 0, N, d, P(c->o_tok), rmap, m->nin_w,
                                         m->nin_b, m->nin_eps, P(c->o_xin), st0, st0 + rows, st));
      map = LinRowMap{rmap, m->nin_w, m->nin_b, P(c->o_xin), st0, st0 + rows, m->nin_eps};
    } else {
      GT_TRY(gt_seq_token_rows(tdt, m->cls, graph_ptr, node_graph, c->seq_desc, B, 1, m->with_cls ? 1 : 0, N, d, P(c->o_tok), rmap, st));
      map.rows = rmap;
    }
    g2t_out = P(c->o_tok);
  }
  LinFwd g2t{};
  if (c->cat2) {
    c->node_rep = nullptr;
    g2t = LinFwd{GT_F32, tdt, compute, c->first, m->g2t_w, m->g2t_b, g2t_out, N, d, 2 * D, D, d, 1, 0, 0, 0, 0.f, 0, (hipStream_t)st};
    g2t.x2 = c->h_last; g2t.x_split = D; g2t.ldx2 = D;
  } else {
    if (m->jk_cat) {
      GT_TRY(gt_copy2d(P(c->o_cat), c->Kc * 4, c->first, D * 4, D * 4, N, st));
      GT_TRY(gt_copy2d((char*)P(c->o_cat) + D * 4, c->Kc * 4, c->h_last, D * 4, D * 4, N, st));
      c->node_rep = P(c->o_cat);
    } else {
      c->node_rep = c->h_last;
    }
    g2t = LinFwd{GT_F32, tdt, compute, c->node_rep, m->g2t_w, m->g2t_b, g2t_out, N, d, c->Kc, c->Kc, d, 1, 0, 0, 0, 0.f, 0, (hipStream_t)st};
  }
  g2t.map = map;
  GT_TRY(lin_fwd(g2t));
  if (!c->fuse_rows)
    GT_TRY(gt_seq_gather_cls32(tdt, P(c->o_hn), m->cls, graph_ptr, c->seq_desc, B, 1, c->max_npos, m->with_cls ? 1 : 0, d, P(c->o_tok), st));
  const void* cur = P(c->o_tok);
  if (fuse_nin) {
    cur = P(c->o_xin);
  } else if (m->nin_w) {
    GT_TRY(gt_layernorm_fwd(tdt, cur, nullptr, m->nin_w, m->nin_b, m->nin_eps, 0.f, 0, rows, d, P(c->o_xin), (float*)P(c->o_st0),
                            (float*)P(c->o_st0) + rows, st));
    cur = P(c->o_xin);
  }
  for (int i = 0; i < nenc; ++i) {
    c->enc_in[i] = cur;
    if (i == nenc - 1) {
      GT_TRY(gt_encoder_layer_pooled_fwd(&c->enc[i], cur, c->last_rows, P(c->o_xe[i]), P(c->o_enc_saved[i]), st));
    } else {
      GT_TRY(gt_encoder_layer_fwd(&c->enc[i], cur, P(c->o_xe[i]), P(c->o_enc_saved[i]), st));
    }
    cur = P(c->o_xe[i]);
  }
  c->pre_out = cur;
  if (m->nout_w) {
    GT_TRY(gt_rows_gather(tdt, cur, nullptr, B, d, (float*)P(c->o_hgin), st));
    GT_TRY(gt_layernorm_fwd(GT_F32, P(c->o_hgin), nullptr, m->nout_w, m->nout_b, m->nout_eps, 0.f, 0, B, d, P(c->o_hg), (float*)P(c->o_sto),
                            (float*)P(c->o_sto) + B, st));
  } else {
    GT_TRY(gt_rows_gather(tdt, cur, nullptr, B, d, (float*)P(c->o_hg), st));
  }
  GT_TRY(gt_linear_fwd_ld(GT_F32, GT_F32, compute, P(c->o_hg), m->head_w, m->head_b, logits, B, m->Nh, d, m->ldy, 0, 0.f, 0, st));
  if (c->esort && m->st_dw) GT_TRY(gt_stream_wait_event(st, m->ev_sort[1]));
  else if (c->want_wt && m->st_dw) GT_TRY(gt_stream_wait_event(st, m->ev_wt[1]));
  (void)E;
  return GT_OK;
}

extern "C" int gt_model_backward(const gt_model* m, void* ctx_, const float* dlogits, float* grads, void* barena, int stages,
                                 gt_stream_t st) {
  GT_TRY(model_check("gt_model_backward", m));
  Ctx* c = (Ctx*)ctx_;
  GT_CHECK_ARG(c && c->magic == CTX_MAGIC && c->forwarded, "context without a forward");
// ... 240 lines not shown
```

### graphtrans_amd/csrc/norm.hip

```cpp
#include <stdlib.h>

#include "gt_common.h"

namespace {

constexpr int NT = 256;
constexpr int MAX_PART = 256;

struct ColMap {
  int C, CW, R, tc, tr;
  __device__ __forceinline__ ColMap(int64_t D) {
    C = (int)(D / 4);
    CW = C < NT ? C : NT;
    R = NT / CW;
    tc = threadIdx.x % CW;
    tr = threadIdx.x / CW;
  }
};

template <int NV>
__device__ __forceinline__ void block_rowlane_reduce(float4 (&v)[NV], const ColMap& m, float4* sm) {
  if (m.tr < m.R) {
#pragma unroll
    for (int i = 0; i < NV; ++i) sm[(m.tr * m.CW + m.tc) * NV + i] = v[i];
// ... 189 lines not shown
#pragma unroll
        for (int u = 0; u < 4; ++u) add_row(g[u], v[u], r + (int64_t)u * m.R);
      }
      for (; r < r1; r += m.R) {
        const int64_t o = r * D + (int64_t)c * 4;
        add_row(gt_load4<T>(dy + o), gt_load4<T>(x + o), r);
      }
    }
    block_rowlane_reduce<2>(acc, m, sm4);
    if (m.tr == 0 && cact) {
      float* p = part + (int64_t)blockIdx.x * 2 * D + (int64_t)c * 4;
      *reinterpret_cast<float4*>(p) = acc[0];
      *reinterpret_cast<float4*>(p + D) = acc[1];
    }
  }
}

__global__ void k_bn_bwd_finish(const float* __restrict__ part, int nblk, int64_t D, float* __restrict__ dbias,
                                float* __restrict__ dweight) {
  __shared__ float sm[FINK_LANES * FIN_COLS];
  const int64_t c = (int64_t)blockIdx.x * FIN_COLS + threadIdx.x % FIN_COLS;
  const float s1 = finish_sum<FINK_LANES>(part, nblk, 2 * D, c, c < D, sm);
  const float s2 = finish_sum<FINK_LANES>(part, nblk, 2 * D, D + c, c < D, sm);
  if (c >= D || threadIdx.x >= FIN_COLS) return;
  dbias[c] = s1;
  dweight[c] = s2;
}

template <typename T>
__global__ void __launch_bounds__(NT) k_bn_bwd_apply(const T* __restrict__ x, const T* __restrict__ dy,
                                                     const float* __restrict__ mean, const float* __restrict__ rstd,
                                                     const float* __restrict__ w, const float* __restrict__ b,
                                                     const float* __restrict__ dbias, const float* __restrict__ dweight,
                                                     int relu, float inv_n, BnDrop drop, int64_t N, int64_t D,
                                                     T* __restrict__ dx, const float* __restrict__ count_dev) {
  const int64_t C = D / 4, total = N * C;
  if (count_dev) inv_n = 1.0f / count_dev[0];
  for (int64_t i = (int64_t)blockIdx.x * NT + threadIdx.x; i < total; i += (int64_t)gridDim.x * NT) {
    const int64_t c = (i % C) * 4;
    float4 g = gt_load4<T>(dy + i * 4);
    const float4 v = gt_load4<T>(x + i * 4);
    const float4 mu = *reinterpret_cast<const float4*>(mean + c), rs = *reinterpret_cast<const float4*>(rstd + c);
    const float4 ww = *reinterpret_cast<const float4*>(w + c);
    if (drop.thr) g = bn_drop4(g, drop, (uint32_t)(i / C), (uint32_t)c);
    if (relu) g = bn_gate(g, v, mu, rs, ww, *reinterpret_cast<const float4*>(b + c));
    const float4 db = *reinterpret_cast<const float4*>(dbias + c), dw = *reinterpret_cast<const float4*>(dweight + c);
    float4 r;
    r.x = ww.x * rs.x * (g.x - db.x * inv_n - (v.x - mu.x) * rs.x * dw.x * inv_n);
    r.y = ww.y * rs.y * (g.y - db.y * inv_n - (v.y - mu.y) * rs.y * dw.y * inv_n);
    r.z = ww.z * rs.z * (g.z - db.z * inv_n - (v.z - mu.z) * rs.z * dw.z * inv_n);
    r.w = ww.w * rs.w * (g.w - db.w * inv_n - (v.w - mu.w) * rs.w * dw.w * inv_n);
    gt_store4<T>(dx + i * 4, r);
  }
}


constexpr int SMALL_ROWS = 1024;

template <typename T>
__device__ __forceinline__ float ld1(const T* p) {
  if constexpr (sizeof(T) == 4) return (float)*reinterpret_cast<const float*>(p);
  else return gt_bf16_to_f32(*reinterpret_cast<const gt_bf16*>(p));
}
template <typename T>
__device__ __forceinline__ void st1(T* p, float v) {
  if constexpr (sizeof(T) == 4) *reinterpret_cast<float*>(p) = v;
  else *reinterpret_cast<gt_bf16*>(p) = gt_f32_to_bf16(v);
}
constexpr int SM_COLS = 8;
constexpr int SM_LANES = 32;
__device__ __forceinline__ float lanes_sum(float v, float* sm) {
  const int cl = threadIdx.x % SM_COLS, p = threadIdx.x / SM_COLS;
  sm[p * SM_COLS + cl] = v;
  __syncthreads();
  float t = 0.f;
  if (p == 0) {
#pragma unroll
    for (int q = 0; q < SM_LANES; ++q) t += sm[q * SM_COLS + cl];
  }
  __syncthreads();
  return t;
}

template <typename T>
__global__ void __launch_bounds__(SM_COLS * SM_LANES) k_bn_small_fwd(
    const T* __restrict__ x, int64_t N, int64_t D, float eps, float momentum, const float* __restrict__ w,
    const float* __restrict__ b, const T* __restrict__ resid, int relu, BnDrop drop, float* __restrict__ mean,
    float* __restrict__ rstd, float* __restrict__ running_mean, float* __restrict__ running_var,
    int64_t* __restrict__ num_batches_tracked, T* __restrict__ y, const T* __restrict__ bcast, const int32_t* __restrict__ bidx) {
  __shared__ float sm[SM_LANES * SM_COLS];
  __shared__ float s_mu[SM_COLS], s_rs[SM_COLS];
  const int cl = threadIdx.x % SM_COLS, p = threadIdx.x / SM_COLS;
  const int64_t c = (int64_t)blockIdx.x * SM_COLS + cl;
  const bool act = c < D;
  if (blockIdx.x == 0 && threadIdx.x == 0 && num_batches_tracked) num_batches_tracked[0] += 1;
  const float piv = act ? ld1<T>(x + c) : 0.f;
  float a1[2] = {0.f, 0.f}, a2[2] = {0.f, 0.f};
  if (act) {
    int64_t r = p;
    for (; r + 3 * SM_LANES < N; r += 4 * SM_LANES) {
      float v[4];
#pragma unroll
      for (int u = 0; u < 4; ++u) v[u] = ld1<T>(x + (r + u * SM_LANES) * D + c) - piv;
#pragma unroll
      for (int u = 0; u < 4; ++u) { a1[u & 1] += v[u]; a2[u & 1] = fmaf(v[u], v[u], a2[u & 1]); }
    }
    for (; r < N; r += SM_LANES) {
      const float v0 = ld1<T>(x + r * D + c) - piv;
      a1[0] += v0; a2[0] = fmaf(v0, v0, a2[0]);
    }
  }
  const float s1 = lanes_sum(a1[0] + a1[1], sm), s2 = lanes_sum(a2[0] + a2[1], sm);
  if (p == 0 && act) {
    const float inv_n = 1.0f / (float)N;
    const float m1 = s1 * inv_n;
    float var = s2 * inv_n - m1 * m1;
    var = var < 0.f ? 0.f : var;
    const float mu = piv + m1, rs = 1.0f / sqrtf(var + eps);
    mean[c] = mu;
    rstd[c] = rs;
    s_mu[cl] = mu;
    s_rs[cl] = rs;
    if (running_mean) {
      running_mean[c] = (1.f - momentum) * running_mean[c] + momentum * mu;
      const float unbiased = N > 1 ? var * ((float)N / (float)(N - 1)) : var;
      running_var[c] = (1.f - momentum) * running_var[c] + momentum * unbiased;
    }
  }
  __syncthreads();
  if (!act) return;
  const float mu = s_mu[cl], rs = s_rs[cl], ww = w[c], bb = b[c];
  for (int64_t r = p; r < N; r += SM_LANES) {
    float v = (ld1<T>(x + r * D + c) - mu) * rs * ww + bb;
    if (relu) v = fmaxf(v, 0.f);
    if (drop.thr) v = bn_hash(drop.s0, drop.s1, (uint32_t)r, (uint32_t)c) >= drop.thr ? v * drop.inv_keep : 0.f;
    if (resid) v += ld1<T>(resid + r * D + c);
    if (bcast) v += ld1<T>(bcast + (int64_t)bidx[r] * D + c);
    st1<T>(y + r * D + c, v);
  }
}

template <typename T>
__global__ void __launch_bounds__(SM_COLS * SM_LANES) k_bn_small_bwd(
    const T* __restrict__ x, const T* __restrict__ dy, const float* __restrict__ mean, const float* __restrict__ rstd,
    const float* __restrict__ w, const float* __restrict__ b, int relu, int training, BnDrop drop, int64_t N, int64_t D,
    float* __restrict__ dbias, float* __restrict__ dweight, T* __restrict__ dx) {
  __shared__ float sm[SM_LANES * SM_COLS];
  __shared__ float s_db[SM_COLS], s_dw[SM_COLS];
  const int cl = threadIdx.x % SM_COLS, p = threadIdx.x / SM_COLS;
  const int64_t c = (int64_t)blockIdx.x * SM_COLS + cl;
  const bool act = c < D;
  const float mu = act ? mean[c] : 0.f, rs = act ? rstd[c] : 0.f, ww = act ? w[c] : 0.f, bb = act ? b[c] : 0.f;
  auto grad_at = [&](int64_t r, float& xh) {
    float g = ld1<T>(dy + r * D + c);
    const float v = ld1<T>(x + r * D + c);
    xh = (v - mu) * rs;
    if (drop.thr) g = bn_hash(drop.s0, drop.s1, (uint32_t)r, (uint32_t)c) >= drop.thr ? g * drop.inv_keep : 0.f;
    if (relu) g = (v - mu) * rs * ww + bb > 0.f ? g : 0.f;
    return g;
  };
  float a0[2] = {0.f, 0.f}, a1[2] = {0.f, 0.f};
  if (act) {
    int64_t r = p;
    for (; r + SM_LANES < N; r += 2 * SM_LANES) {
      float xh0, xh1;
      const float g0 = grad_at(r, xh0), g1 = grad_at(r + SM_LANES, xh1);
// ... 463 lines not shown
                                float* __restrict__ dbias) {
  __shared__ float sm[FINK_LANES * FIN_COLS];
  const int64_t c = (int64_t)blockIdx.x * FIN_COLS + threadIdx.x % FIN_COLS;
  const float s1 = finish_sum<FINK_LANES>(part, nblk, 2 * D, c, c < D, sm);
  const float s2 = finish_sum<FINK_LANES>(part, nblk, 2 * D, D + c, c < D, sm);
  if (c >= D || threadIdx.x >= FIN_COLS) return;
  dweight[c] = s1;
  dbias[c] = s2;
}

constexpr int LN_BWD_BLOCKS = 256;

template <typename T, bool BWD>
void ln_launch(const LnArgs& a, int grid_bwd, hipStream_t stream) {
  const int64_t D = a.D;
  if constexpr (BWD) {
    if (D == 128) {
      hipLaunchKernelGGL((k_ln_bwd_d128<T, 1024, 128>), dim3(grid_bwd), dim3(1024), (size_t)16 * 2 * 128 * 4, stream, a);
      return;
    }
    if (D == 256) {
      hipLaunchKernelGGL((k_ln_bwd_d128<T, 1024, 256>), dim3(grid_bwd), dim3(1024), (size_t)16 * 2 * 256 * 4, stream, a);
      return;
    }
  }
#define GT_LN(LPN, NCH)                                                                                      \
  do {                                                                                                       \
    if constexpr (BWD) {                                                                                     \
      if (D <= 256)                                                                                        \
        hipLaunchKernelGGL((k_ln_bwd<T, LPN, NCH, 1024>), dim3(grid_bwd), dim3(1024), (size_t)16 * 2 * D * 4, \
                           stream, a);                                                                       \
      else                                                                                                   \
        hipLaunchKernelGGL((k_ln_bwd<T, LPN, NCH, NT>), dim3(grid_bwd), dim3(NT), (size_t)(NT / 64) * 2 * D * 4, \
                           stream, a);                                                                       \
    } else {                                                                                                 \
      int64_t waves = gt_cdiv(a.rows, 64 / (LPN));                                                           \
      hipLaunchKernelGGL((k_ln_fwd<T, LPN, NCH>), dim3((unsigned)gt_cdiv(waves, NT / 64)), dim3(NT), 0,      \
                         stream, a);                                                                         \
    }                                                                                                        \
  } while (0)
  if (D <= 64) GT_LN(16, 1);
  else if (D <= 128) GT_LN(32, 1);
  else if (D <= 256) GT_LN(64, 1);
  else if (D <= 512) GT_LN(64, 2);
  else if (D <= 768) GT_LN(64, 3);
  else GT_LN(64, 4);
#undef GT_LN
}

void fill_drop(LnArgs& a, float dropout_p, uint64_t seed) {
  a.inv_keep = 1.0f / (1.0f - dropout_p);
  double thr = (double)dropout_p * 4294967296.0;
  a.thr = dropout_p > 0.f ? (uint32_t)(thr > 4294967295.0 ? 4294967295.0 : (thr < 1.0 ? 1.0 : thr)) : 0u;
  a.s0 = (uint32_t)seed;
  a.s1 = (uint32_t)(seed >> 32);
}

}

static BnDrop make_bn_drop(float dropout_p, uint64_t seed) {
  BnDrop d{};
  d.inv_keep = 1.0f / (1.0f - dropout_p);
  double thr = (double)dropout_p * 4294967296.0;
  d.thr = dropout_p > 0.f ? (uint32_t)(thr > 4294967295.0 ? 4294967295.0 : (thr < 1.0 ? 1.0 : thr)) : 0u;
  d.s0 = (uint32_t)seed;
  d.s1 = (uint32_t)(seed >> 32);
  return d;
}

extern "C" size_t gt_batchnorm_workspace_bytes(int64_t rows, int64_t dim) {
  return (size_t)part_blocks(rows) * 2 * dim * sizeof(float) + 256 + (size_t)(BN_SYNC_MAX_WORLD + 2) * (2 * dim + 4) * sizeof(float);
}

extern "C" int gt_batchnorm_fwd(int dtype, const void* x, const float* weight, const float* bias,
                                float* running_mean, float* running_var, int64_t* num_batches_tracked,
                                float momentum, float eps, int training, int relu, const void* resid, int64_t rows,
                                int64_t dim, void* y, float* save_mean, float* save_rstd, float dropout_p,
                                uint64_t seed, void* workspace, size_t workspace_bytes, gt_stream_t stream_) {
  return gt_batchnorm_fwd_bcast(dtype, x, weight, bias, running_mean, running_var, num_batches_tracked, momentum, eps, training,
                                relu, resid, nullptr, nullptr, nullptr, rows, dim, y, save_mean, save_rstd, dropout_p, seed, workspace,
                                workspace_bytes, stream_);
}

extern "C" int gt_batchnorm_fwd_bcast(int dtype, const void* x, const float* weight, const float* bias,
                                      float* running_mean, float* running_var, int64_t* num_batches_tracked,
                                      float momentum, float eps, int training, int relu, const void* resid,
                                      const void* bcast, const int32_t* bcast_index, void* ev_bcast_ready, int64_t rows,
                                      int64_t dim, void* y, float* save_mean, float* save_rstd, float dropout_p,
                                      uint64_t seed, void* workspace, size_t workspace_bytes, gt_stream_t stream_) {
  int rc = check_norm("gt_batchnorm_fwd", dtype, rows, dim);
  GT_CHECK_ARG(!bcast || bcast_index, "bcast needs bcast_index");

  if (rc) return rc;
  GT_CHECK_ARG(dropout_p >= 0.f && dropout_p < 1.f, "dropout_p must be in [0,1)");
  const BnDrop drop = make_bn_drop(training ? dropout_p : 0.f, seed);
  GT_CHECK_ARG(x && weight && bias && y && save_mean && save_rstd, "null buffer");
  GT_CHECK_ARG(training || (running_mean && running_var), "eval mode needs running statistics");
  const bool sync = training && g_bn_sync.fn && g_bn_sync.world > 1;
  if (rows == 0 && !sync) return GT_OK;
  hipStream_t stream = (hipStream_t)stream_;
  const int cgrid = (int)gt_cdiv(dim, FIN_COLS);
  if (training) {
    GT_CHECK_ARG(rows > 1 || sync, "BatchNorm in training mode needs more than 1 row");
    if (rows <= SMALL_ROWS && !sync) {
      if (bcast && ev_bcast_ready) {
        rc = gt_stream_wait_event(stream_, ev_bcast_ready);
        if (rc) return rc;
      }
      if (dtype == GT_F32)
        hipLaunchKernelGGL(k_bn_small_fwd<float>, dim3((unsigned)gt_cdiv(dim, SM_COLS)), dim3(SM_COLS * SM_LANES), 0, stream, (const float*)x, rows, dim,
                           eps, momentum, weight, bias, (const float*)resid, relu, drop, save_mean, save_rstd, running_mean,
                           running_var, num_batches_tracked, (float*)y, (const float*)bcast, bcast_index);
      else
        hipLaunchKernelGGL(k_bn_small_fwd<gt_bf16>, dim3((unsigned)gt_cdiv(dim, SM_COLS)), dim3(SM_COLS * SM_LANES), 0, stream, (const gt_bf16*)x, rows,
                           dim, eps, momentum, weight, bias, (const gt_bf16*)resid, relu, drop, save_mean, save_rstd,
                           running_mean, running_var, num_batches_tracked, (gt_bf16*)y, (const gt_bf16*)bcast, bcast_index);
      GT_CHECK_LAUNCH();
      return GT_OK;
    }
    const int nb = part_blocks(rows);
    if (!workspace || workspace_bytes < gt_batchnorm_workspace_bytes(rows, dim)) {
      gt_set_error("gt_batchnorm_fwd: workspace too small");
      return GT_ERR_WORKSPACE;
    }
    float* part = (float*)workspace;
    size_t lds = rowlane_lds(dim, 2);
    float* rm_l = sync ? nullptr : running_mean;
    float* rv_l = sync ? nullptr : running_var;
    int64_t* nbt_l = sync ? nullptr : num_batches_tracked;
    if (rows > 0) {
      if (dtype == GT_F32) {
        hipLaunchKernelGGL(k_bn_stats_partial<float>, dim3(nb), dim3(NT), lds, stream, (const float*)x, rows, dim, part);
        hipLaunchKernelGGL(k_bn_stats_finish<float>, dim3(cgrid), dim3(FIN_COLS * FINK_LANES), 0, stream, (const float*)x, part, nb, rows,
                           dim, eps, momentum, save_mean, save_rstd, rm_l, rv_l, nbt_l);
      } else {
        hipLaunchKernelGGL(k_bn_stats_partial<gt_bf16>, dim3(nb), dim3(NT), lds, stream, (const gt_bf16*)x, rows, dim, part);
        hipLaunchKernelGGL(k_bn_stats_finish<gt_bf16>, dim3(cgrid), dim3(FIN_COLS * FINK_LANES), 0, stream, (const gt_bf16*)x, part, nb,
                           rows, dim, eps, momentum, save_mean, save_rstd, rm_l, rv_l, nbt_l);
      }
    }
    if (sync) {
      float* sb = bn_sync_buf(workspace, rows, dim);
      const int64_t n = 2 * dim + 1;
      const unsigned cg = (unsigned)gt_cdiv(dim > 1 ? dim : 1, 256);
      if (rows > 0) hipLaunchKernelGGL(k_bn_sync_pack, dim3(cg), dim3(256), 0, stream, save_mean, save_rstd, (float)rows, eps, dim, sb);
      else (void)hipMemsetAsync(sb, 0, (size_t)n * sizeof(float), stream);
      GT_CHECK_LAUNCH();
      const int hrc = g_bn_sync.fn(g_bn_sync.user, 0, sb, n, stream_);
      if (hrc) { gt_set_error("gt_batchnorm_fwd: the statistics hook failed (%d)", hrc); return GT_ERR_LAUNCH; }
      hipLaunchKernelGGL(k_bn_sync_merge, dim3(cg), dim3(256), 0, stream, sb + n, g_bn_sync.world, dim, eps, momentum, save_mean, save_rstd,
                         running_mean, running_var, num_batches_tracked);
      if (rows == 0) { GT_CHECK_LAUNCH(); return GT_OK; }
    }
  } else {
    hipLaunchKernelGGL(k_bn_eval_stats, dim3(cgrid), dim3(256), 0, stream, running_mean, running_var, dim, eps, save_mean,
                       save_rstd);
  }
  const int g = flat_blocks(rows * (dim / 4));
  if (bcast && ev_bcast_ready) {
    rc = gt_stream_wait_event(stream_, ev_bcast_ready);
    if (rc) return rc;
  }
  if (dtype == GT_F32)
    hipLaunchKernelGGL(k_bn_apply<float>, dim3(g), dim3(NT), 0, stream, (const float*)x, save_mean, save_rstd, weight,
                       bias, (const float*)resid, relu, drop, rows, dim, (float*)y, (const float*)bcast, bcast_index);
  else
    hipLaunchKernelGGL(k_bn_apply<gt_bf16>, dim3(g), dim3(NT), 0, stream, (const gt_bf16*)x, save_mean, save_rstd, weight,
                       bias, (const gt_bf16*)resid, relu, drop, rows, dim, (gt_bf16*)y, (const gt_bf16*)bcast, bcast_index);
  GT_CHECK_LAUNCH();
  return GT_OK;
}

extern "C" int gt_batchnorm_bwd(int dtype, const void* x, const void* dy, const float* weight, const float* bias,
                                const float* save_mean, const float* save_rstd, int training, int relu, int64_t rows,
                                int64_t dim, void* dx, float* dweight, float* dbias, float dropout_p, uint64_t seed,
                                void* workspace, size_t workspace_bytes, gt_stream_t stream_) {
  int rc = check_norm("gt_batchnorm_bwd", dtype, rows, dim);
  if (rc) return rc;
  GT_CHECK_ARG(dropout_p >= 0.f && dropout_p < 1.f, "dropout_p must be in [0,1)");
  const BnDrop drop = make_bn_drop(training ? dropout_p : 0.f, seed);
  GT_CHECK_ARG(x && dy && weight && bias && save_mean && save_rstd && dx && dweight && dbias, "null buffer");
  const bool sync = training && g_bn_sync.fn && g_bn_sync.world > 1;
  if (rows == 0 && !sync) return GT_OK;
  if (!workspace || workspace_bytes < gt_batchnorm_workspace_bytes(rows, dim)) {
    gt_set_error("gt_batchnorm_bwd: workspace too small");
    return GT_ERR_WORKSPACE;
  }
  hipStream_t stream = (hipStream_t)stream_;
  const int nb = part_blocks(rows);
  float* part = (float*)workspace;
  const size_t lds = rowlane_lds(dim, 2);
  const int cgrid = (int)gt_cdiv(dim, FIN_COLS);
  const int g = flat_blocks(rows * (dim / 4));
  if (sync) {
    const unsigned cg = (unsigned)gt_cdiv(dim > 1 ? dim : 1, 256);
    float* sb = bn_sync_buf(workspace, rows, dim);
    if (rows > 0) {
      if (dtype == GT_F32)
        hipLaunchKernelGGL(k_bn_bwd_partial<float>, dim3(nb), dim3(NT), lds, stream, (const float*)x, (const float*)dy, weight, bias,
                           save_mean, save_rstd, relu, drop, rows, dim, part);
      else
        hipLaunchKernelGGL(k_bn_bwd_partial<gt_bf16>, dim3(nb), dim3(NT), lds, stream, (const gt_bf16*)x, (const gt_bf16*)dy, weight,
                           bias, save_mean, save_rstd, relu, drop, rows, dim, part);
      hipLaunchKernelGGL(k_bn_bwd_finish, dim3(cgrid), dim3(FIN_COLS * FINK_LANES), 0, stream, part, nb, dim, dbias, dweight);
      hipLaunchKernelGGL(k_bn_sync_copy2, dim3(cg), dim3(256), 0, stream, dbias, dweight, (float)rows, dim, sb);
    } else {
      (void)hipMemsetAsync(dbias, 0, (size_t)dim * sizeof(float), stream);
      (void)hipMemsetAsync(dweight, 0, (size_t)dim * sizeof(float), stream);
      (void)hipMemsetAsync(sb, 0, (size_t)(2 * dim + 1) * sizeof(float), stream);
    }
    GT_CHECK_LAUNCH();
    const int hrc = g_bn_sync.fn(g_bn_sync.user, 1, sb, 2 * dim + 1, stream_);
    if (hrc) { gt_set_error("gt_batchnorm_bwd: the statistics hook failed (%d)", hrc); return GT_ERR_LAUNCH; }
    if (rows > 0) {
      if (dtype == GT_F32)
        hipLaunchKernelGGL(k_bn_bwd_apply<float>, dim3(g), dim3(NT), 0, stream, (const float*)x, (const float*)dy, save_mean, save_rstd,
                           weight, bias, sb, sb + dim, relu, 1.0f, drop, rows, dim, (float*)dx, (const float*)(sb + 2 * dim));
      else
        hipLaunchKernelGGL(k_bn_bwd_apply<gt_bf16>, dim3(g), dim3(NT), 0, stream, (const gt_bf16*)x, (const gt_bf16*)dy, save_mean,
                           save_rstd, weight, bias, sb, sb + dim, relu, 1.0f, drop, rows, dim, (gt_bf16*)dx, (const float*)(sb + 2 * dim));
    }
    GT_CHECK_LAUNCH();
    return GT_OK;
  }
  if (rows <= SMALL_ROWS) {
    if (dtype == GT_F32)
      hipLaunchKernelGGL(k_bn_small_bwd<float>, dim3((unsigned)gt_cdiv(dim, SM_COLS)), dim3(SM_COLS * SM_LANES), 0, stream, (const float*)x,
                         (const float*)dy, save_mean, save_rstd, weight, bias, relu, training, drop, rows, dim, dbias, dweight,
                         (float*)dx);
    else
      hipLaunchKernelGGL(k_bn_small_bwd<gt_bf16>, dim3((unsigned)gt_cdiv(dim, SM_COLS)), dim3(SM_COLS * SM_LANES), 0, stream, (const gt_bf16*)x,
                         (const gt_bf16*)dy, save_mean, save_rstd, weight, bias, relu, training, drop, rows, dim, dbias,
                         dweight, (gt_bf16*)dx);
    GT_CHECK_LAUNCH();
    return GT_OK;
  }
  if (dtype == GT_F32) {
    hipLaunchKernelGGL(k_bn_bwd_partial<float>, dim3(nb), dim3(NT), lds, stream, (const float*)x, (const float*)dy,
                       weight, bias, save_mean, save_rstd, relu, drop, rows, dim, part);
    hipLaunchKernelGGL(k_bn_bwd_finish, dim3(cgrid), dim3(FIN_COLS * FINK_LANES), 0, stream, part, nb, dim, dbias, dweight);
    hipLaunchKernelGGL(k_bn_bwd_apply<float>, dim3(g), dim3(NT), 0, stream, (const float*)x, (const float*)dy,
                       save_mean, save_rstd, weight, bias, dbias, dweight, relu, training ? 1.0f / (float)rows : 0.f, drop, rows, dim, (float*)dx, (const float*)nullptr);
  } else {
    hipLaunchKernelGGL(k_bn_bwd_partial<gt_bf16>, dim3(nb), dim3(NT), lds, stream, (const gt_bf16*)x, (const gt_bf16*)dy,
                       weight, bias, save_mean, save_rstd, relu, drop, rows, dim, part);
    hipLaunchKernelGGL(k_bn_bwd_finish, dim3(cgrid), dim3(FIN_COLS * FINK_LANES), 0, stream, part, nb, dim, dbias, dweight);
    hipLaunchKernelGGL(k_bn_bwd_apply<gt_bf16>, dim3(g), dim3(NT), 0, stream, (const gt_bf16*)x, (const gt_bf16*)dy,
                       save_mean, save_rstd, weight, bias, dbias, dweight, relu, training ? 1.0f / (float)rows : 0.f, drop, rows, dim, (gt_bf16*)dx, (const float*)nullptr);
  }
  GT_CHECK_LAUNCH();
  return GT_OK;
}

// ... 146 lines not shown
```

### graphtrans_amd/csrc/segment.hip

```cpp
#include "gt_common.h"

namespace {

constexpr int SEG_THREADS = 256;

template <typename T>
__global__ void __launch_bounds__(SEG_THREADS) k_bcast_add(const T* __restrict__ x, const T* __restrict__ seg,
                                                           const int32_t* __restrict__ node_graph, int64_t N,
                                                           int64_t D, T* __restrict__ out) {
  const int64_t C = D / 4;
  const int64_t total = N * C;
  for (int64_t i = (int64_t)blockIdx.x * SEG_THREADS + threadIdx.x; i < total; i += (int64_t)gridDim.x * SEG_THREADS) {
    int64_t r = i / C, c = (i % C) * 4;
    float4 s = gt_load4<T>(seg + (int64_t)node_graph[r] * D + c);
    if (x) s = gt_add4(s, gt_load4<T>(x + r * D + c));
    gt_store4<T>(out + r * D + c, s);
  }
}

template <typename T>
__global__ void __launch_bounds__(SEG_THREADS) k_segment_sum(const T* __restrict__ x, const T* __restrict__ add,
                                                             const int32_t* __restrict__ gptr, int64_t D,
                                                             T* __restrict__ out) {
  __shared__ float4 sm[4][64];
  const int b = blockIdx.y;
  const int lane = threadIdx.x & 63, wid = threadIdx.x >> 6;
  const int64_t c = ((int64_t)blockIdx.x * 64 + lane) * 4;
  const bool act = c < D;
  const int beg = gptr[b], end = gptr[b + 1];
  float4 acc = gt_zero4();
  if (act) {
    int r = beg + wid;
    for (; r + 28 < end; r += 32) {
      float4 v[8];
#pragma unroll
      for (int u = 0; u < 8; ++u) v[u] = gt_load4<T>(x + (int64_t)(r + 4 * u) * D + c);
#pragma unroll
      for (int u = 0; u < 8; ++u) acc = gt_add4(acc, v[u]);
    }
    for (; r < end; r += 4) acc = gt_add4(acc, gt_load4<T>(x + (int64_t)r * D + c));
  }
  sm[wid][lane] = acc;
  __syncthreads();
  if (wid == 0 && act) {
    float4 t = gt_add4(gt_add4(sm[0][lane], sm[1][lane]), gt_add4(sm[2][lane], sm[3][lane]));
    if (add) t = gt_add4(t, gt_load4<T>(add + (int64_t)b * D + c));
    gt_store4<T>(out + (int64_t)b * D + c, t);
  }
}

constexpr int SS_CH = 64, SS_T = 320;

template <typename T>
__device__ __forceinline__ float ldf(const T* p) {
  if constexpr (sizeof(T) == 4) return (float)*reinterpret_cast<const float*>(p);
  else return gt_bf16_to_f32(*reinterpret_cast<const gt_bf16*>(p));
}
template <typename T>
__device__ __forceinline__ void stf(T* p, float v) {
  if constexpr (sizeof(T) == 4) *reinterpret_cast<float*>(p) = v;
  else *reinterpret_cast<gt_bf16*>(p) = gt_f32_to_bf16(v);
}

template <typename T>
__global__ void __launch_bounds__(SS_T) k_segsum_chunks(const T* __restrict__ x, const T* __restrict__ add,
                                                        const int32_t* __restrict__ gptr, int B, int64_t N, int64_t D,
                                                        T* __restrict__ out, float* __restrict__ head, float* __restrict__ tail) {
  const int64_t p0 = (int64_t)blockIdx.x * SS_CH;
  const int64_t p1 = p0 + SS_CH < N ? p0 + SS_CH : N;
  if (p0 >= p1) return;
  int lo = 0, hi = B;
  while (hi - lo > 1) {
    const int mid = (lo + hi) >> 1;
    if (gptr[mid] <= p0) lo = mid; else hi = mid;
  }
  const int g0 = lo;
  float* hd = head + (int64_t)blockIdx.x * D;
  float* tl = tail + (int64_t)blockIdx.x * D;
  for (int64_t c = threadIdx.x; c < D; c += SS_T) {
    int g = g0;
    int64_t gend = gptr[g + 1];
    float acc = 0.f;
    auto flush = [&](int gg, float v) {
      const bool before = gptr[gg] < p0, after = (int64_t)gptr[gg + 1] > p1;
      if (before) hd[c] = v;
      else if (after) tl[c] = v;
      else stf<T>(out + (int64_t)gg * D + c, v + (add ? ldf<T>(add + (int64_t)gg * D + c) : 0.f));
    };
    for (int64_t rb = p0; rb < p1; rb += 8) {
      float v[8];
#pragma unroll
      for (int u = 0; u < 8; ++u) v[u] = rb + u < p1 ? ldf<T>(x + (rb + u) * D + c) : 0.f;
#pragma unroll
      for (int u = 0; u < 8; ++u) {
        const int64_t r = rb + u;
        if (r >= p1) break;
        if (r == gend) {
          flush(g, acc);
          acc = 0.f;
          do { ++g; gend = gptr[g + 1]; } while (gend <= r);
        }
        acc += v[u];
      }
    }
    flush(g, acc);
  }
}

template <typename T>
__global__ void __launch_bounds__(SS_T) k_segsum_fixup(const T* __restrict__ add, const int32_t* __restrict__ gptr, int64_t D,
                                                       const float* __restrict__ head, const float* __restrict__ tail,
                                                       T* __restrict__ out) {
  const int b = blockIdx.x;
  const int64_t beg = gptr[b], end = gptr[b + 1];
  if (end > beg && beg / SS_CH == (end - 1) / SS_CH) return;
  const int64_t c0 = beg / SS_CH, c1 = end > beg ? (end - 1) / SS_CH : 0;
  for (int64_t c = threadIdx.x; c < D; c += SS_T) {
    float acc = 0.f;
    if (end > beg) {
      acc = tail[c0 * D + c];
      int64_t j = c0 + 1;
      for (; j + 7 <= c1; j += 8) {
        float v[8];
#pragma unroll
        for (int u = 0; u < 8; ++u) v[u] = head[(j + u) * D + c];
#pragma unroll
        for (int u = 0; u < 8; ++u) acc += v[u];
      }
      for (; j <= c1; ++j) acc += head[j * D + c];
    }
    stf<T>(out + (int64_t)b * D + c, acc + (add ? ldf<T>(add + (int64_t)b * D + c) : 0.f));
  }
}

// ... 251 lines not shown
      const float4 v = gt_load4<T>(tokens + row * D + c * 4);
      const float dx = v.x - mu, dy = v.y - mu, dz = v.z - mu, dw = v.w - mu;
      q += (dx * dx + dy * dy) + (dz * dz + dw * dw);
    }
#pragma unroll
    for (int sh = 32; sh > 0; sh >>= 1) q += __shfl_xor(q, sh, 64);
    const float rs = 1.0f / sqrtf(q / (float)D + ln_eps);
    for (int64_t c = lane; c < C; c += 64) {
      const float4 v = gt_load4<T>(tokens + row * D + c * 4);
      const float4 w4 = *reinterpret_cast<const float4*>(ln_w + c * 4), b4 = *reinterpret_cast<const float4*>(ln_b + c * 4);
      gt_store4<T>(ln_out + row * D + c * 4, make_float4((v.x - mu) * rs * w4.x + b4.x, (v.y - mu) * rs * w4.y + b4.y,
                                                          (v.z - mu) * rs * w4.z + b4.z, (v.w - mu) * rs * w4.w + b4.w));
    }
    if (lane == 0) {
      ln_mean[row] = mu;
      ln_rstd[row] = rs;
    }
  }
}
static int seq_token_rows_impl(const char* fn, int dtype, const float* cls32, const int32_t* graph_ptr, const int32_t* node_graph,
                               const int32_t* seq_desc, int64_t num_seqs, int64_t row_stride, int with_cls, int64_t N, int64_t D, void* tokens,
                               int32_t* rows, const float* ln_w, const float* ln_b, float ln_eps, void* ln_out, float* ln_mean, float* ln_rstd,
                               gt_stream_t stream_) {
  int rc = check(fn, dtype, D);
  if (rc) return rc;
  if (!(graph_ptr && node_graph && seq_desc && tokens && rows)) { gt_set_error("%s: null buffer", fn); return GT_ERR_INVALID_ARG; }
  if (with_cls && !cls32) { gt_set_error("%s: with_cls needs the cls row", fn); return GT_ERR_INVALID_ARG; }
  if (num_seqs == 0) return GT_OK;
  hipStream_t stream = (hipStream_t)stream_;
  int64_t items = N > num_seqs * (D / 4) ? N : num_seqs * (D / 4);
  if (ln_out && items < num_seqs * 64) items = num_seqs * 64;
  dim3 grid((unsigned)(gt_cdiv(items, SEG_THREADS) < 1024 ? gt_cdiv(items, SEG_THREADS) : 1024));
  if (dtype == GT_F32)
    hipLaunchKernelGGL(k_seq_token_rows<float>, grid, dim3(SEG_THREADS), 0, stream, cls32, graph_ptr, node_graph, seq_desc, num_seqs, row_stride,
                       with_cls, N, D, (float*)tokens, rows, ln_w, ln_b, ln_eps, (float*)ln_out, ln_mean, ln_rstd);
  else
    hipLaunchKernelGGL(k_seq_token_rows<gt_bf16>, grid, dim3(SEG_THREADS), 0, stream, cls32, graph_ptr, node_graph, seq_desc, num_seqs, row_stride,
                       with_cls, N, D, (gt_bf16*)tokens, rows, ln_w, ln_b, ln_eps, (gt_bf16*)ln_out, ln_mean, ln_rstd);
  GT_CHECK_LAUNCH();
  return GT_OK;
}
extern "C" int gt_seq_token_rows(int dtype, const float* cls32, const int32_t* graph_ptr, const int32_t* node_graph, const int32_t* seq_desc,
                                 int64_t num_seqs, int64_t row_stride, int with_cls, int64_t N, int64_t D, void* tokens, int32_t* rows,
                                 gt_stream_t stream_) {
  return seq_token_rows_impl("gt_seq_token_rows", dtype, cls32, graph_ptr, node_graph, seq_desc, num_seqs, row_stride, with_cls, N, D, tokens, rows,
                             nullptr, nullptr, 0.f, nullptr, nullptr, nullptr, stream_);
}
extern "C" int gt_seq_token_rows_layernorm(int dtype, const float* cls32, const int32_t* graph_ptr, const int32_t* node_graph,
                                           const int32_t* seq_desc, int64_t num_seqs, int64_t row_stride, int with_cls, int64_t N, int64_t D,
                                           void* tokens, int32_t* rows, const float* ln_w, const float* ln_b, float ln_eps, void* ln_out,
                                           float* ln_mean, float* ln_rstd, gt_stream_t stream_) {
  GT_CHECK_ARG(ln_w && ln_b && ln_out && ln_mean && ln_rstd, "null LayerNorm buffer");
  return seq_token_rows_impl("gt_seq_token_rows_layernorm", dtype, cls32, graph_ptr, node_graph, seq_desc, num_seqs, row_stride, with_cls, N, D,
                             tokens, rows, ln_w, ln_b, ln_eps, ln_out, ln_mean, ln_rstd, stream_);
}

extern "C" int gt_seq_scatter(int dtype, const void* tokens, const void* base, const int32_t* graph_ptr,
                              const int32_t* node_graph, const int32_t* seq_desc, int64_t num_seqs,
                              int64_t row_stride, int with_cls, int64_t N, int64_t D, void* h_out, void* cls_out,
                              gt_stream_t stream_) {
  int rc = check("gt_seq_scatter", dtype, D);
  if (rc) return rc;
  GT_CHECK_ARG(tokens && graph_ptr && node_graph && seq_desc && h_out, "null buffer");
  if (num_seqs == 0) return GT_OK;
  hipStream_t stream = (hipStream_t)stream_;
  int64_t items = (N > num_seqs ? N : num_seqs) * (D / 4);
  dim3 grid(flat_grid(items));
  if (dtype == GT_F32)
    hipLaunchKernelGGL(k_seq_scatter<float>, grid, dim3(SEG_THREADS), 0, stream, (const float*)tokens,
                       (const float*)base, graph_ptr, node_graph, seq_desc, num_seqs, row_stride, with_cls, N, D,
                       (float*)h_out, (float*)cls_out);
  else
    hipLaunchKernelGGL(k_seq_scatter<gt_bf16>, grid, dim3(SEG_THREADS), 0, stream, (const gt_bf16*)tokens,
                       (const gt_bf16*)base, graph_ptr, node_graph, seq_desc, num_seqs, row_stride, with_cls, N, D,
                       (gt_bf16*)h_out, (gt_bf16*)cls_out);
  GT_CHECK_LAUNCH();
  return GT_OK;
}

extern "C" size_t gt_segment_sum_workspace_bytes(int64_t N, int64_t D) {
  return (size_t)2 * gt_cdiv(N > 0 ? N : 1, SS_CH) * D * sizeof(float) + 256;
}

extern "C" int gt_segment_sum_ws(int dtype, const void* x, const void* add, const int32_t* graph_ptr, int64_t N, int64_t B,
                                 int64_t D, void* out, void* workspace, size_t workspace_bytes, gt_stream_t stream_) {
  if (N < 4096 || !workspace || workspace_bytes < gt_segment_sum_workspace_bytes(N, D))
    return gt_segment_sum(dtype, x, add, graph_ptr, N, B, D, out, stream_);
  int rc = check("gt_segment_sum_ws", dtype, D);
  if (rc) return rc;
  GT_CHECK_ARG(x && graph_ptr && out, "null buffer");
  if (B == 0) return GT_OK;
  GT_CHECK_ARG(B <= 0x7fffffff && N <= 0x7fffffff, "sizes beyond int32");
  hipStream_t stream = (hipStream_t)stream_;
  const int64_t nch = gt_cdiv(N, SS_CH);
  float* head = static_cast<float*>(workspace);
  float* tail = head + nch * D;
  if (dtype == GT_F32) {
    hipLaunchKernelGGL(k_segsum_chunks<float>, dim3((unsigned)nch), dim3(SS_T), 0, stream, (const float*)x, (const float*)add,
                       graph_ptr, (int)B, N, D, (float*)out, head, tail);
    hipLaunchKernelGGL(k_segsum_fixup<float>, dim3((unsigned)B), dim3(SS_T), 0, stream, (const float*)add, graph_ptr, D,
                       (const float*)head, (const float*)tail, (float*)out);
  } else {
    hipLaunchKernelGGL(k_segsum_chunks<gt_bf16>, dim3((unsigned)nch), dim3(SS_T), 0, stream, (const gt_bf16*)x,
                       (const gt_bf16*)add, graph_ptr, (int)B, N, D, (gt_bf16*)out, head, tail);
    hipLaunchKernelGGL(k_segsum_fixup<gt_bf16>, dim3((unsigned)B), dim3(SS_T), 0, stream, (const gt_bf16*)add, graph_ptr, D,
                       (const float*)head, (const float*)tail, (gt_bf16*)out);
  }
  GT_CHECK_LAUNCH();
  return GT_OK;
}

__global__ void __launch_bounds__(1024) k_seq_layout_packed(const int32_t* __restrict__ gptr, int B, int max_len, int cls,
                                                            int32_t* __restrict__ desc, int64_t* __restrict__ last_rows,
                                                            int32_t* __restrict__ work, int64_t work_cap, int32_t* __restrict__ meta) {
  __shared__ int sred[32];
  __shared__ int sscan[2][1024];
  __shared__ int scarry[2];
  const int t = threadIdx.x;
  int mx = 0;
  for (int b = t; b < B; b += 1024) mx = max(mx, gptr[b + 1] - gptr[b]);
  for (int o = 32; o > 0; o >>= 1) mx = max(mx, __shfl_xor(mx, o));
  if ((t & 63) == 0) sred[t >> 6] = mx;
  __syncthreads();
  if (t == 0) {
    int m = 0;
    for (int i = 0; i < 16; ++i) m = max(m, sred[i]);
    sred[16] = m < max_len ? m : max_len;
    scarry[0] = 0;
    scarry[1] = 0;
  }
  __syncthreads();
  const int S = sred[16];
  int max_kv = 0;
  for (int b0 = 0; b0 < B; b0 += 1024) {
    const int b = b0 + t;
    int kv = 0, tiles = 0;
    if (b < B) {
      const int n = gptr[b + 1] - gptr[b];
      kv = (n < S ? n : S) + cls;
      tiles = (kv + 63) >> 6;
      max_kv = max(max_kv, kv);
    }
    sscan[0][t] = kv;
    sscan[1][t] = tiles;
    __syncthreads();
    for (int o = 1; o < 1024; o <<= 1) {
      int a0 = 0, a1 = 0;
      if (t >= o) { a0 = sscan[0][t - o]; a1 = sscan[1][t - o]; }
      __syncthreads();
      sscan[0][t] += a0;
      sscan[1][t] += a1;
      __syncthreads();
    }
    const int row0 = scarry[0] + sscan[0][t] - kv, w0 = scarry[1] + sscan[1][t] - tiles;
    if (b < B) {
      desc[b * 4 + 0] = row0;
      desc[b * 4 + 1] = kv;
      desc[b * 4 + 2] = 0;
      desc[b * 4 + 3] = kv;
      last_rows[b] = (int64_t)row0 + kv - 1;
      for (int i = 0; i < tiles; ++i)
        if (w0 + i < work_cap) { work[(int64_t)(w0 + i) * 2] = b; work[(int64_t)(w0 + i) * 2 + 1] = i; }
    }
    __syncthreads();
    if (t == 1023) { scarry[0] += sscan[0][1023]; scarry[1] += sscan[1][1023]; }
    __syncthreads();
  }
  for (int o = 32; o > 0; o >>= 1) max_kv = max(max_kv, __shfl_xor(max_kv, o));
  if ((t & 63) == 0) sred[t >> 6] = max_kv;
  __syncthreads();
  const int rows = scarry[0], nwork = scarry[1];
  for (int64_t w = nwork + t; w < work_cap; w += 1024) { work[w * 2] = -1; work[w * 2 + 1] = -1; }
  if (t == 0) {
    int m = 0;
    for (int i = 0; i < 16; ++i) m = max(m, sred[i]);
    meta[0] = rows; meta[1] = nwork; meta[2] = m; meta[3] = S;
  }
}

extern "C" int gt_seq_layout_packed(const int32_t* graph_ptr, int64_t B, int64_t max_input_len, int with_cls, int32_t* seq_desc,
                                    int64_t* last_rows, int32_t* work_items, int64_t work_capacity, int32_t* meta,
                                    gt_stream_t stream_) {
  GT_CHECK_ARG(graph_ptr && seq_desc && last_rows && work_items && meta, "null buffer");
  GT_CHECK_ARG(B >= 0 && B <= 65535 && max_input_len > 0 && work_capacity >= 0, "bad sizes");
  if (B == 0) return GT_OK;
  hipLaunchKernelGGL(k_seq_layout_packed, dim3(1), dim3(1024), 0, (hipStream_t)stream_, graph_ptr, (int)B,
                     (int)(max_input_len > 0x3fffffff ? 0x3fffffff : max_input_len), with_cls ? 1 : 0, seq_desc, last_rows, work_items,
                     work_capacity, meta);
  GT_CHECK_LAUNCH();
  return GT_OK;
}
```

### graphtrans_amd/layers.py

```python
import ctypes as C

import torch

from . import _lib
from ._lib import GT_BF16, GT_EDGE_LINEAR, GT_EDGE_NONE, GT_EDGE_TABLES, GT_F32
from .graph import _ptr, _stream

_fp = C.c_void_p


class EncoderLayerDesc(C.Structure):
    _fields_ = [("rows", C.c_int64), ("d_model", C.c_int64), ("ffn", C.c_int64),
                ("nhead", C.c_int32), ("dtype", C.c_int32), ("compute", C.c_int32), ("training", C.c_int32),
                ("seq_desc", _fp), ("num_seqs", C.c_int64), ("row_stride", C.c_int64), ("max_npos", C.c_int64),
                ("work_items", _fp), ("num_work", C.c_int64), ("dropout_p", C.c_float), ("ln_eps", C.c_float),
                ("act", C.c_int32), ("reserved_", C.c_int32), ("seed", C.c_uint64)] + \
               [(n, _fp) for n in ("in_w", "in_b", "out_w", "out_b", "l1_w", "l1_b", "l2_w", "l2_b", "n1_w", "n1_b",
                                   "n2_w", "n2_b")]


class GcnLayerDesc(C.Structure):
    _fields_ = [("N", C.c_int64), ("E", C.c_int64), ("B", C.c_int64), ("D", C.c_int64),
                ("edge_mode", C.c_int32), ("has_vn", C.c_int32), ("relu", C.c_int32), ("residual", C.c_int32),
                ("training", C.c_int32), ("compute", C.c_int32),
                ("edge_cols", C.c_int64), ("table_rows", C.c_int64), ("tab_off", C.c_int32 * 4),
                ("bn_momentum", C.c_float), ("bn_eps", C.c_float)] + \
               [(n, _fp) for n in ("graph_ptr", "node_graph", "in_ptr", "in_src", "in_eid", "out_ptr", "out_dst", "out_eid",
                                   "deg", "dis", "edge_attr", "lin_w", "lin_b", "root", "edge_w", "edge_b", "bn_w", "bn_b",
                                   "bn_rm", "bn_rv", "bn_nbt", "ev_x_ready", "ev_dx_wait")] + \
               [("seed", C.c_uint64), ("dropout_p", C.c_float), ("x_has_vn", C.c_int32), ("vn_next", _fp), ("ev_vn_next", _fp),
                ("lin_wt", _fp), ("prev_saved", _fp), ("prev_bn_w", _fp), ("prev_bn_b", _fp), ("prev_bn_part", _fp),
                ("bn_part_in", _fp), ("prev_relu", C.c_int32), ("bn_nparts_in", C.c_int32), ("ev_graph_ready", _fp),
                ("dx_bcast", _fp), ("dx_bcast_idx", _fp)]


class GinLayerDesc(C.Structure):
    _fields_ = [("N", C.c_int64), ("E", C.c_int64), ("B", C.c_int64), ("D", C.c_int64),
                ("edge_mode", C.c_int32), ("has_vn", C.c_int32), ("relu", C.c_int32), ("residual", C.c_int32),
                ("training", C.c_int32), ("compute", C.c_int32),
                ("edge_cols", C.c_int64), ("table_rows", C.c_int64), ("tab_off", C.c_int32 * 4),
                ("bn_momentum", C.c_float), ("bn_eps", C.c_float)] + \
               [(n, _fp) for n in ("graph_ptr", "node_graph", "in_ptr", "in_src", "in_eid", "out_ptr", "out_dst", "out_eid",
                                   "edge_attr", "eps", "edge_w", "edge_b", "w1", "b1", "bn1_w", "bn1_b", "w2", "b2", "bn_w",
                                   "bn_b", "bn1_rm", "bn1_rv", "bn_rm", "bn_rv", "bn1_nbt", "bn_nbt", "ev_x_ready",
                                   "ev_dx_wait")] + \
               [("seed", C.c_uint64), ("dropout_p", C.c_float), ("x_has_vn", C.c_int32), ("vn_next", _fp), ("ev_vn_next", _fp),
                ("w1_t", _fp), ("w2_t", _fp)]


class VnUpdateDesc(C.Structure):
    _fields_ = [("N", C.c_int64), ("B", C.c_int64), ("D", C.c_int64),
                ("residual", C.c_int32), ("training", C.c_int32), ("compute", C.c_int32), ("pad_", C.c_int32),
                ("bn_momentum", C.c_float), ("bn_eps", C.c_float)] + \
               [(n, _fp) for n in ("graph_ptr", "node_graph", "identity_graph", "w1", "b1", "bn1_w", "bn1_b", "w2", "b2",
                                   "bn2_w", "bn2_b", "bn1_rm", "bn1_rv", "bn2_rm", "bn2_rv", "bn1_nbt", "bn2_nbt")] + \
               [("seed", C.c_uint64), ("dropout_p", C.c_float), ("pad2_", C.c_int32), ("ev_dx_done", _fp)]


class PnaLayerDesc(C.Structure):
    _fields_ = [("N", C.c_int64), ("E", C.c_int64), ("D", C.c_int64),
                ("T", C.c_int32), ("S", C.c_int32), ("training", C.c_int32), ("compute", C.c_int32),
                ("bn_momentum", C.c_float), ("bn_eps", C.c_float)] + \
               [(n, _fp) for n in ("in_ptr", "in_src", "in_eid", "out_ptr", "out_dst", "out_eid", "scales", "pre_w", "pre_b", "post_w",
                                   "post_b", "lin_w", "lin_b", "bn_w", "bn_b", "bn_rm", "bn_rv", "bn_nbt", "d_pre_w", "d_pre_b",
                                   "d_post_w", "d_post_b")] + \
               [("seed", C.c_uint64), ("dropout_p", C.c_float), ("pad_", C.c_int32)]


def _any_sync(*bns):
    from .modules.norm import any_sync
    return any_sync(*bns)


def _bind():
    return _lib.lib()


def _bytes(n, dev):
    return torch.empty(max(int(n), 16), dtype=torch.uint8, device=dev)


def _split(flat, params):
    out, off = [], 0
    for p in params:
        n = p.numel()
        out.append(flat[off:off + n].view(p.shape))
        off += n
    return out


def _compute_code():
    from . import ops
    return ops.f32_compute_code()


def _f32c(p):
    if p.dtype != torch.float32 or not p.is_contiguous():
        raise TypeError("composite layers need contiguous fp32 parameters")
    return p


ENC_PARAM_ORDER = ("self_attn.in_proj_weight", "self_attn.in_proj_bias", "self_attn.out_proj.weight",
                   "self_attn.out_proj.bias", "linear1.weight", "linear1.bias", "linear2.weight", "linear2.bias",
                   "norm1.weight", "norm1.bias", "norm2.weight", "norm2.bias")


def encoder_layer_params(mod):
    sa = mod.self_attn
    return [sa.in_proj_weight, sa.in_proj_bias, sa.out_proj.weight, sa.out_proj.bias, mod.linear1.weight, mod.linear1.bias,
            mod.linear2.weight, mod.linear2.bias, mod.norm1.weight, mod.norm1.bias, mod.norm2.weight, mod.norm2.bias]


ENC_ACT = {"relu": 0, "gelu": 1}


def _encoder_desc(x, lay, nhead, dropout_p, seed, training, ln_eps, act, params):
    rows, d = x.shape
    desc = EncoderLayerDesc()
    desc.rows, desc.d_model, desc.ffn = rows, d, params[4].shape[0]
    desc.nhead = nhead
    desc.dtype = GT_BF16 if x.dtype == torch.bfloat16 else GT_F32
    desc.compute = _compute_code()
    desc.training = 1 if training else 0
    desc.seq_desc = _ptr(lay.desc)
    desc.num_seqs, desc.row_stride, desc.max_npos = lay.B, lay.row_stride, lay.max_npos
    desc.work_items, desc.num_work = _ptr(getattr(lay, "work", None)), getattr(lay, "num_work", 0)
    desc.dropout_p, desc.ln_eps, desc.seed = float(dropout_p), float(ln_eps), int(seed)
    desc.act = ENC_ACT[act]
    for name, p in zip(("in_w", "in_b", "out_w", "out_b", "l1_w", "l1_b", "l2_w", "l2_b", "n1_w", "n1_b", "n2_w", "n2_b"), params):
        setattr(desc, name, _ptr(_f32c(p)))
# ... 242 lines not shown
```

### include/graphtrans_hip.h

```cpp
#ifndef GRAPHTRANS_HIP_H
#define GRAPHTRANS_HIP_H

#include <stddef.h>
#include <stdint.h>

#ifdef __cplusplus
extern "C" {
#endif

typedef void* gt_stream_t;

enum gt_status {
  GT_OK = 0,
  GT_ERR_INVALID_ARG = -1,
  GT_ERR_UNSUPPORTED = -2,
  GT_ERR_WORKSPACE = -3,
  GT_ERR_LAUNCH = -4
};

enum gt_dtype { GT_F32 = 0, GT_BF16 = 1 };
enum gt_compute { GT_COMPUTE_F32 = 0, GT_COMPUTE_BF16 = 1, GT_COMPUTE_F32_HIGH = 2 };
enum gt_conv { GT_CONV_GCN = 0, GT_CONV_GIN = 1, GT_CONV_PNA = 2  };
enum gt_edge_mode {
  GT_EDGE_NONE = 0,
// ... 36 lines not shown
  int32_t x_cols;
  int32_t ea_cols;
} gt_graph_store;

typedef struct gt_collate_out {
  int64_t* x;
  int64_t* node_depth;
  int64_t* batch;
  int64_t* ptr;
  int64_t* edge_index;
  float* edge_attr_f32;
  int64_t* edge_attr_i64;
  void* y;
} gt_collate_out;

int gt_attr_rank(const int64_t* node_is_attributed, int64_t num_nodes, int64_t* rank, gt_stream_t stream);
size_t gt_collate_workspace_bytes(int64_t num_graphs);
int gt_collate(const gt_graph_store* store, const int64_t* graph_ids, int64_t num_graphs, int64_t num_nodes,
               int64_t num_edges, const gt_collate_out* out, void* workspace, size_t workspace_bytes,
               gt_stream_t stream);

size_t gt_graph_prep_workspace_bytes(int64_t num_nodes, int64_t num_edges, int64_t num_graphs);
int gt_graph_prep(const int64_t* edge_index, const int64_t* batch, int64_t num_nodes, int64_t num_edges,
                  int64_t num_graphs, int32_t* graph_ptr, int32_t* node_graph, int32_t* in_ptr, int32_t* in_src,
                  int32_t* in_eid,
                  int32_t* out_ptr, int32_t* out_dst, int32_t* out_eid, float* deg, float* dis,
                  int32_t* status, void* workspace, size_t workspace_bytes, gt_stream_t stream);

int gt_aggregate_fwd(int conv, int edge_mode, int dtype, const void* h, int64_t num_nodes, int64_t num_edges,
                     int64_t dim, const int32_t* in_ptr, const int32_t* in_src, const int32_t* in_eid,
                     const float* deg, const float* dis, const float* self_param, const void* edge_attr,
                     int64_t edge_attr_cols, const float* edge_w, const float* edge_b,
                     const int32_t* tab_off_host, int64_t table_rows ,
                     const void* edge_dense, void* out, gt_stream_t stream);

size_t gt_aggregate_bwd_workspace_bytes(int conv, int edge_mode, int64_t dim, int64_t edge_attr_cols,
                                        int64_t table_rows);
int gt_aggregate_bwd(int conv, int edge_mode, int dtype, const void* h, const void* grad_out, int64_t num_nodes,
                     int64_t num_edges, int64_t dim, const int32_t* out_ptr, const int32_t* out_dst,
                     const int32_t* out_eid, const float* deg, const float* dis, const float* self_param,
                     const void* edge_attr, int64_t edge_attr_cols, const float* edge_w, const float* edge_b,
                     const int32_t* tab_off_host, int64_t table_rows, const void* edge_dense, void* grad_h,
                     float* d_self, float* d_edge_w, float* d_edge_b, void* d_dense, void* workspace,
                     size_t workspace_bytes, gt_stream_t stream);

int gt_pna_aggregate_fwd(const float* U, const float* V, int64_t num_nodes, int64_t dim, int towers,
                         const int32_t* in_ptr, const int32_t* in_src, const int32_t* in_eid, float* out,
                         float* mean_v, int32_t* arg, gt_stream_t stream);
int gt_pna_aggregate_bwd(const float* V, const float* out, const float* mean_v, const int32_t* arg,
                         const float* grad_out, int64_t num_nodes, int64_t dim, int towers, const int32_t* in_ptr,
                         const int32_t* out_ptr, const int32_t* out_dst, const int32_t* out_eid, float* dU, float* dV,
                         gt_stream_t stream);
int gt_scale_combine_fwd(const float* Y, const float* scales, int64_t num_nodes, int towers, int num_scalers, int F,
                         float* out, gt_stream_t stream);
int gt_scale_combine_bwd(const float* grad_out, const float* scales, int64_t num_nodes, int towers, int num_scalers, int F,
                         float* dY, gt_stream_t stream);

int gt_embed_sum_fwd(int num_tables, const int64_t* const* idx_ptrs_host, const int64_t* idx_strides_host,
                     const int64_t* clamp_max_host, const float* const* tables_host, int64_t num_nodes, int64_t dim,
                     float* out, gt_stream_t stream);
size_t gt_embed_sum_bwd_workspace_bytes(int num_tables, const int64_t* table_rows_host, int64_t dim);
int gt_embed_sum_bwd(int num_tables, const int64_t* const* idx_ptrs_host, const int64_t* idx_strides_host,
                     const int64_t* clamp_max_host, const int64_t* table_rows_host, const float* grad_out,
                     int64_t num_nodes, int64_t dim, float* const* d_tables_host, void* workspace,
                     size_t workspace_bytes, gt_stream_t stream);
size_t gt_embed_sort_plan_bytes(int num_tables, const int64_t* table_rows_host, int64_t num_nodes);
size_t gt_embed_sort_workspace_bytes(int num_tables, const int64_t* table_rows_host, int64_t num_nodes);
int gt_embed_sort(int num_tables, const int64_t* const* idx_ptrs_host, const int64_t* idx_strides_host,
                  const int64_t* clamp_max_host, const int64_t* table_rows_host, int64_t num_nodes, void* plan,
                  size_t plan_bytes, void* workspace, size_t workspace_bytes, gt_stream_t stream);
size_t gt_embed_sum_bwd_sorted_workspace_bytes(int num_tables, int64_t num_nodes, int64_t dim);
int gt_embed_sum_bwd_sorted(int num_tables, const int64_t* table_rows_host, const float* grad_out, int64_t num_nodes,
                            int64_t dim, const void* plan, float* const* d_tables_host, void* workspace,
                            size_t workspace_bytes, gt_stream_t stream);

int gt_segment_bcast_add(int dtype, const void* x, const void* seg, const int32_t* node_graph, int64_t num_nodes,
                         int64_t num_graphs, int64_t dim, void* out, gt_stream_t stream);
int gt_segment_sum(int dtype, const void* x, const void* add, const int32_t* graph_ptr, int64_t num_nodes,
                   int64_t num_graphs, int64_t dim, void* out, gt_stream_t stream);
size_t gt_segment_sum_workspace_bytes(int64_t num_nodes, int64_t dim);
int gt_segment_sum_ws(int dtype, const void* x, const void* add, const int32_t* graph_ptr, int64_t num_nodes,
                      int64_t num_graphs, int64_t dim, void* out, void* workspace, size_t workspace_bytes,
                      gt_stream_t stream);

int gt_seq_gather(int dtype, const void* h, const void* cls, const int32_t* graph_ptr, const int32_t* seq_desc,
                  int64_t num_seqs, int64_t row_stride, int64_t max_npos, int with_cls, int64_t dim,
                  void* tokens, uint8_t* pad_mask , gt_stream_t stream);
int gt_seq_scatter(int dtype, const void* tokens, const void* base, const int32_t* graph_ptr,
                   const int32_t* node_graph, const int32_t* seq_desc, int64_t num_seqs, int64_t row_stride,
                   int with_cls, int64_t num_nodes, int64_t dim, void* h_out, void* cls_out ,
                   gt_stream_t stream);
int gt_seq_layout_packed(const int32_t* graph_ptr, int64_t B, int64_t max_input_len, int with_cls, int32_t* seq_desc,
                         int64_t* last_rows, int32_t* work_items, int64_t work_capacity, int32_t* meta, gt_stream_t stream);

int gt_attn_head_dim_ok(int dtype, int64_t d_model, int nhead);
int gt_attn_fwd(int dtype, const void* qkv, void* ctx, float* lse, int64_t total_rows, int64_t d_model, int nhead,
                const int32_t* seq_desc, int64_t num_seqs, int64_t row_stride, int64_t max_npos,
                const int32_t* work_items, int64_t num_work, const float* dense_mask, const float* key_valid,
                float mask_value, float scale, float dropout_p, uint64_t seed, gt_stream_t stream);
int gt_attn_bwd(int dtype, const void* qkv, const void* ctx, const void* d_ctx, const float* lse, float* delta,
                void* d_qkv, int64_t total_rows, int64_t d_model, int nhead, const int32_t* seq_desc,
                int64_t num_seqs, int64_t row_stride, int64_t max_npos, const int32_t* work_items, int64_t num_work,
                const float* dense_mask, const float* key_valid, float mask_value, float scale, float dropout_p,
                uint64_t seed, gt_stream_t stream);
int gt_attn_fwd_last(int dtype, const void* qkv, void* ctx, float* lse, int64_t total_rows, int64_t d_model, int nhead,
                     const int32_t* seq_desc, int64_t num_seqs, int64_t row_stride, int64_t max_npos, float scale, float dropout_p,
                     uint64_t seed, gt_stream_t stream);
int gt_attn_bwd_last(int dtype, const void* qkv, const void* ctx, const void* d_ctx, const float* lse, float* delta, void* d_qkv,
                     int64_t total_rows, int64_t d_model, int nhead, const int32_t* seq_desc, int64_t num_seqs, int64_t row_stride,
                     int64_t max_npos, const int32_t* work_items, int64_t num_work, float scale, float dropout_p, uint64_t seed,
                     gt_stream_t stream);

size_t gt_batchnorm_workspace_bytes(int64_t rows, int64_t dim);
int gt_batchnorm_fwd(int dtype, const void* x, const float* weight, const float* bias, float* running_mean,
                     float* running_var, int64_t* num_batches_tracked, float momentum, float eps, int training,
                     int relu, const void* resid , int64_t rows, int64_t dim,
                     void* y, float* save_mean, float* save_rstd, float dropout_p, uint64_t seed, void* workspace,
                     size_t workspace_bytes, gt_stream_t stream);
int gt_batchnorm_fwd_bcast(int dtype, const void* x, const float* weight, const float* bias, float* running_mean,
                           float* running_var, int64_t* num_batches_tracked, float momentum, float eps, int training,
                           int relu, const void* resid, const void* bcast, const int32_t* bcast_index, void* ev_bcast_ready,
                           int64_t rows, int64_t dim, void* y, float* save_mean, float* save_rstd, float dropout_p,
                           uint64_t seed, void* workspace, size_t workspace_bytes, gt_stream_t stream);
int gt_batchnorm_bwd(int dtype, const void* x, const void* dy, const float* weight, const float* bias,
                     const float* save_mean, const float* save_rstd, int training, int relu, int64_t rows,
                     int64_t dim, void* dx, float* dweight, float* dbias, float dropout_p, uint64_t seed, void* workspace,
                     size_t workspace_bytes, gt_stream_t stream);
int gt_batchnorm_bwd_parts(int dtype, const void* x, const void* dy, const float* weight, const float* bias,
                           const float* save_mean, const float* save_rstd, int training, int relu, int64_t rows, int64_t dim,
                           void* dx, float* dweight, float* dbias, const float* part, int64_t nparts, gt_stream_t stream);
typedef int (*gt_bn_sync_fn)(void* user, int kind, float* buf, int64_t n, gt_stream_t stream);
int gt_bn_sync_set(gt_bn_sync_fn fn, void* user, int world);
int gt_batchnorm_apply(int dtype, const void* x, const float* mean, const float* rstd, const float* weight,
                       const float* bias, int relu, const void* resid, int64_t rows, int64_t dim, void* y, float dropout_p,
                       uint64_t seed, gt_stream_t stream);
int gt_batchnorm_bwd_apply(int dtype, const void* x, const void* dy, const float* weight, const float* bias,
                           const float* mean, const float* rstd, const float* sum_dy, const float* sum_dy_xhat, double count,
                           int relu, int64_t rows, int64_t dim, void* dx, float dropout_p, uint64_t seed, gt_stream_t stream);

int gt_layernorm_fwd(int dtype, const void* x, const void* resid, const float* weight, const float* bias, float eps,
                     float dropout_p, uint64_t seed, int64_t rows, int64_t dim, void* y, float* save_mean,
                     float* save_rstd, gt_stream_t stream);
size_t gt_layernorm_bwd_workspace_bytes(int64_t rows, int64_t dim);
int gt_layernorm_bwd(int dtype, const void* x, const void* resid, const void* dy, const float* weight,
                     const float* save_mean, const float* save_rstd, float dropout_p, uint64_t seed, int64_t rows,
                     int64_t dim, void* dx, void* dresid, float* dweight, float* dbias, void* workspace,
                     size_t workspace_bytes, gt_stream_t stream);
int gt_layernorm_bwd_finish(const float* part, int nblk, int64_t dim, float* dweight, float* dbias, gt_stream_t stream);

int gt_linear_fwd(int x_dtype, int y_dtype, int compute, const void* x, const float* weight, const float* bias,
                  void* y, int64_t M, int64_t N, int64_t K, int act, float dropout_p, uint64_t seed,
                  gt_stream_t stream);
int gt_linear_fwd_ld(int x_dtype, int y_dtype, int compute, const void* x, const float* weight, const float* bias,
                     void* y, int64_t M, int64_t N, int64_t K, int64_t ldy, int act, float dropout_p, uint64_t seed,
                     gt_stream_t stream);
int gt_linear_fwd_ld2(int x_dtype, int y_dtype, int compute, const void* x, const float* weight, const float* bias,
                      void* y, int64_t M, int64_t N, int64_t K, int64_t ldx, int64_t ldy, int act, float dropout_p,
                      uint64_t seed, gt_stream_t stream);
size_t gt_linear_bwd_workspace_bytes(int compute, int64_t M, int64_t N, int64_t K);
int gt_linear_bwd(int x_dtype, int y_dtype, int compute, const void* x, const float* weight, const void* dy,
                  const void* y_for_mask, const void* dx_add1, const void* dx_add2, void* dx, float* dweight,
                  float* dbias, int64_t M, int64_t N, int64_t K, float dropout_p, void* workspace,
                  size_t workspace_bytes, gt_stream_t stream);
int gt_linear_bwd_ld(int x_dtype, int y_dtype, int compute, const void* x, const float* weight, const void* dy,
                     const void* y_for_mask, const void* dx_add1, const void* dx_add2, void* dx, float* dweight,
                     float* dbias, int64_t M, int64_t N, int64_t K, int64_t ldy, float dropout_p, void* workspace,
                     size_t workspace_bytes, gt_stream_t stream);

int gt_linear_fwd_gelu(int x_dtype, int y_dtype, int compute, const void* x, const float* weight, const float* bias,
                       void* y, void* gmul, int64_t M, int64_t N, int64_t K, int64_t ldx, int64_t ldy, float dropout_p,
                       uint64_t seed, gt_stream_t stream);
int gt_linear_bwd_mul(int x_dtype, int y_dtype, int compute, const void* x, const float* weight, const void* dy,
                      const void* gmul, const void* dx_add1, const void* dx_add2, void* dx, float* dweight, float* dbias,
                      int64_t M, int64_t N, int64_t K, int64_t ldx, int64_t ldy, void* workspace, size_t workspace_bytes,
                      gt_stream_t stream);

int gt_overlap_dw_begin(gt_stream_t main_stream, gt_stream_t side_stream);
int gt_linear_bwd_bnstats_ok(int compute, int x_dtype, int y_dtype, int64_t M);
int64_t gt_linear_bwd_bnstats_rows(int64_t M);
int64_t gt_linear_bwd_bnstats_rows_for(int compute, int x_dtype, int y_dtype, const float* weight, int64_t M, int64_t N, int64_t K);
int gt_linear_bwd_bnstats(const float* bn_x, int64_t ldx, const float* mean, const float* rstd, const float* w, const float* b,
                          int relu, float* part);
int gt_linear_bwd_bcast_ok(int compute, int x_dtype, int y_dtype, const float* weight, int64_t M, int64_t N, int64_t K);
int gt_linear_bwd_bcast(const float* rows, const int32_t* idx);
int gt_linear_bwd_wt(int x_dtype, int y_dtype, int compute, const void* x, const float* weight, const float* weight_t,
                     const void* dy, const void* y_for_mask, const void* dx_add1, const void* dx_add2, void* dx,
                     float* dweight, float* dbias, int64_t M, int64_t N, int64_t K, float dropout_p, void* workspace,
                     size_t workspace_bytes, gt_stream_t stream);
int gt_transpose(const float* in , float* out , int64_t N, int64_t K, gt_stream_t stream);

int gt_linear_products(int which, int x_dtype, int y_dtype, int compute, const float* weight, int64_t M, int64_t N, int64_t K);
int gt_linear_cat2_ok(int compute, const float* weight, int64_t M, int64_t N, int64_t K1, int64_t K2);
int gt_linear_rows_ok(int compute, int x_dtype, int y_dtype, const float* weight, int64_t M, int64_t N, int64_t K);
int gt_linear_set_rows(const int32_t* rows);
int gt_linear_rows_layernorm_ok(int64_t N);
int gt_linear_set_rows_layernorm(const int32_t* rows, const float* ln_w, const float* ln_b, float eps, void* ln_out, float* ln_mean,
                                 float* ln_rstd);
int gt_linear_fwd_cat2(int y_dtype, int compute, const void* x1, int64_t K1, int64_t ldx1, const void* x2, int64_t K2, int64_t ldx2,
                       const float* weight, const float* bias, void* y, int64_t M, int64_t N, int64_t ldy, gt_stream_t stream);
int gt_linear_bwd_cat2(int y_dtype, int compute, const void* x1, int64_t K1, int64_t ldx1, const void* x2, int64_t K2, int64_t ldx2,
                       const float* weight, const void* dy, void* dx1, int64_t lddx1, void* dx2, int64_t lddx2, float* dweight,
                       float* dbias, int64_t M, int64_t N, int64_t ldy, void* workspace, size_t workspace_bytes, gt_stream_t stream);
size_t gt_w3_image_bytes(int64_t rows, int64_t contraction);
int gt_w3_images(int n, const float* const* weight, const int64_t* N, const int64_t* K, const int* transposed,
                 void* const* image, gt_stream_t stream);
int gt_w3_bind(int n, const float* const* weight, const int64_t* N, const int64_t* K, const void* const* image_fwd,
// ... 43 lines not shown
void gt_overlap_dw_booked(const void* workspace, size_t bytes);
int gt_overlap_dw_end(void);

int gt_linear_bwd_ld2(int x_dtype, int y_dtype, int compute, const void* x, const float* weight, const void* dy,
                      const void* y_for_mask, const void* dx_add1, const void* dx_add2, void* dx, float* dweight,
                      float* dbias, int64_t M, int64_t N, int64_t K, int64_t ldx, int64_t ldy, float dropout_p,
                      void* workspace, size_t workspace_bytes, gt_stream_t stream);
int gt_linear_fwd_grouped(int x_dtype, int y_dtype, int compute, const void* x, const float* weight, const float* bias,
                          void* y, int64_t M, int64_t N, int64_t K, int64_t ldx, int64_t ldy, int groups,
                          int64_t x_group_stride, int64_t y_group_stride, int act, float dropout_p, uint64_t seed,
                          gt_stream_t stream);
size_t gt_linear_bwd_grouped_workspace_bytes(int compute, int64_t M, int64_t N, int64_t K, int groups);
int gt_linear_bwd_grouped(int x_dtype, int y_dtype, int compute, const void* x, const float* weight, const void* dy,
                          const void* y_for_mask, const void* dx_add1, const void* dx_add2, void* dx, float* dweight,
                          float* dbias, int64_t M, int64_t N, int64_t K, int64_t ldx, int64_t ldy, int groups,
                          int64_t x_group_stride, int64_t y_group_stride, float dropout_p, void* workspace,
                          size_t workspace_bytes, gt_stream_t stream);

int gt_xent_fwd(const float* logits, int64_t B, int64_t L, int64_t C, int64_t ld, const int64_t* target,
                int64_t target_stride, float* lse, float* row_loss, float* head_scale, float* loss,
                gt_stream_t stream);
int gt_xent_bwd(const float* logits, const float* lse, const float* head_scale, const int64_t* target,
                int64_t target_stride, const float* grad_loss, int64_t B, int64_t L, int64_t C, int64_t ld,
                float* dlogits, gt_stream_t stream);

int gt_bce_masked_fwd(const float* logits, const float* target, int64_t B, int64_t T, int64_t ld, int64_t target_ld,
                      const float* den_in , float* row_sum, float* row_cnt, float* out2,
                      gt_stream_t stream);
int gt_bce_masked_bwd(const float* logits, const float* target, const float* out2, const float* grad_loss, int64_t B,
                      int64_t T, int64_t ld, int64_t target_ld, float* dlogits, gt_stream_t stream);

typedef struct gt_encoder_layer {
  int64_t rows, d_model, ffn;
  int32_t nhead, dtype , compute , training;
  const int32_t* seq_desc;
  int64_t num_seqs, row_stride, max_npos;
  const int32_t* work_items;
  int64_t num_work;
  float dropout_p, ln_eps;
  int32_t act , reserved_;
  uint64_t seed;
  const float *in_w, *in_b, *out_w, *out_b, *l1_w, *l1_b, *l2_w, *l2_b, *n1_w, *n1_b, *n2_w, *n2_b;
} gt_encoder_layer;
size_t gt_encoder_layer_saved_bytes(const gt_encoder_layer* layer);
size_t gt_encoder_layer_workspace_bytes(const gt_encoder_layer* layer);
int64_t gt_encoder_layer_grad_elems(const gt_encoder_layer* layer);
int gt_encoder_layer_fwd(const gt_encoder_layer* layer, const void* x, void* y, void* saved, gt_stream_t stream);
int gt_encoder_layer_bwd(const gt_encoder_layer* layer, const void* x, const void* dy, const void* saved, void* dx,
                         float* grads, void* workspace, size_t workspace_bytes, gt_stream_t stream);
size_t gt_encoder_layer_pooled_saved_bytes(const gt_encoder_layer* layer);
size_t gt_encoder_layer_pooled_workspace_bytes(const gt_encoder_layer* layer);
int gt_encoder_layer_pooled_fwd(const gt_encoder_layer* layer, const void* x, const int64_t* pool_rows, void* y_pool, void* saved,
                                gt_stream_t stream);
int gt_encoder_layer_pooled_bwd(const gt_encoder_layer* layer, const void* x, const int64_t* pool_rows, const void* dy_pool,
                                const void* saved, void* dx, float* grads, void* workspace, size_t workspace_bytes, gt_stream_t stream);

typedef struct gt_gcn_layer {
  int64_t N, E, B, D;
  int32_t edge_mode , has_vn, relu, residual, training, compute;
  int64_t edge_cols, table_rows;
  int32_t tab_off[4];
  float bn_momentum, bn_eps;
  const int32_t *graph_ptr, *node_graph, *in_ptr, *in_src, *in_eid, *out_ptr, *out_dst, *out_eid;
  const float *deg, *dis;
  const void* edge_attr;
  const float *lin_w, *lin_b, *root, *edge_w, *edge_b, *bn_w, *bn_b;
  float *bn_rm, *bn_rv;
  int64_t* bn_nbt;
  void *ev_x_ready, *ev_dx_wait;
  uint64_t seed;
  float dropout_p;
  int32_t x_has_vn;
  const void* vn_next;
  void* ev_vn_next;
  const float* lin_wt;
  const void* prev_saved;
  const float *prev_bn_w, *prev_bn_b;
  float* prev_bn_part;
  const float* bn_part_in;
  int32_t prev_relu, bn_nparts_in;
  void* ev_graph_ready;
  const float* dx_bcast;
  const int32_t* dx_bcast_idx;
} gt_gcn_layer;
size_t gt_gcn_layer_saved_bytes(const gt_gcn_layer* layer);
size_t gt_gcn_layer_workspace_bytes(const gt_gcn_layer* layer);
int64_t gt_gcn_layer_grad_elems(const gt_gcn_layer* layer);
int gt_gcn_layer_fwd(const gt_gcn_layer* layer, const void* h_in, const void* vn, void* x_out, void* y, void* saved,
                     void* workspace, size_t workspace_bytes, gt_stream_t stream);
int gt_gcn_layer_bwd(const gt_gcn_layer* layer, const void* x, const void* dy, const void* dx_extra, const void* saved,
                     void* d_h_in, void* d_vn, float* grads, void* workspace, size_t workspace_bytes,
                     gt_stream_t stream);

typedef struct gt_gin_layer {
  int64_t N, E, B, D;
  int32_t edge_mode , has_vn, relu, residual, training, compute;
  int64_t edge_cols, table_rows;
  int32_t tab_off[4];
  float bn_momentum, bn_eps;
  const int32_t *graph_ptr, *node_graph, *in_ptr, *in_src, *in_eid, *out_ptr, *out_dst, *out_eid;
  const void* edge_attr;
  const float *eps, *edge_w, *edge_b, *w1, *b1, *bn1_w, *bn1_b, *w2, *b2, *bn_w, *bn_b;
  float *bn1_rm, *bn1_rv, *bn_rm, *bn_rv;
  int64_t *bn1_nbt, *bn_nbt;
  void *ev_x_ready, *ev_dx_wait;
  uint64_t seed;
  float dropout_p;
  int32_t x_has_vn;
  const void* vn_next;
  void* ev_vn_next;
  const float *w1_t, *w2_t;
} gt_gin_layer;
size_t gt_gin_layer_saved_bytes(const gt_gin_layer* layer);
size_t gt_gin_layer_workspace_bytes(const gt_gin_layer* layer);
int64_t gt_gin_layer_grad_elems(const gt_gin_layer* layer);
int gt_gin_layer_fwd(const gt_gin_layer* layer, const void* h_in, const void* vn, void* x_out, void* y, void* saved,
                     void* workspace, size_t workspace_bytes, gt_stream_t stream);
int gt_gin_layer_bwd(const gt_gin_layer* layer, const void* x, const void* dy, const void* dx_extra, const void* saved,
                     void* d_h_in, void* d_vn, float* grads, void* workspace, size_t workspace_bytes,
                     gt_stream_t stream);

typedef struct gt_vn_update {
  int64_t N, B, D;
  int32_t residual, training, compute, pad_;
  float bn_momentum, bn_eps;
  const int32_t *graph_ptr, *node_graph, *identity_graph ;
  const float *w1, *b1, *bn1_w, *bn1_b, *w2, *b2, *bn2_w, *bn2_b;
  float *bn1_rm, *bn1_rv, *bn2_rm, *bn2_rv;
  int64_t *bn1_nbt, *bn2_nbt;
  uint64_t seed;
  float dropout_p;
  int32_t pad2_;
  void* ev_dx_done;
} gt_vn_update;
size_t gt_vn_update_saved_bytes(const gt_vn_update* layer);
size_t gt_vn_update_workspace_bytes(const gt_vn_update* layer);
int64_t gt_vn_update_grad_elems(const gt_vn_update* layer);
int gt_vn_update_fwd(const gt_vn_update* layer, const void* x, const void* vn, void* vn_out, void* saved,
                     void* workspace, size_t workspace_bytes, gt_stream_t stream);
int gt_vn_update_bwd(const gt_vn_update* layer, const void* d_vn_out, const void* saved, const void* d_x_add, void* d_x,
                     void* d_vn, float* grads, void* workspace, size_t workspace_bytes, gt_stream_t stream);
const float* gt_vn_update_bwd_dt0(const gt_vn_update* L, void* workspace);

typedef struct gt_pna_layer {
  int64_t N, E, D;
  int32_t T, S, training, compute;
  float bn_momentum, bn_eps;
  const int32_t *in_ptr, *in_src, *in_eid, *out_ptr, *out_dst, *out_eid;
  const float* scales;
  const float *pre_w, *pre_b, *post_w, *post_b;
  const float *lin_w, *lin_b, *bn_w, *bn_b;
  float *bn_rm, *bn_rv;
  int64_t* bn_nbt;
  float *d_pre_w, *d_pre_b, *d_post_w, *d_post_b;
  uint64_t seed;
  float dropout_p;
  int32_t pad_;
} gt_pna_layer;
size_t gt_pna_layer_saved_bytes(const gt_pna_layer* layer);
size_t gt_pna_layer_workspace_bytes(const gt_pna_layer* layer);
int64_t gt_pna_layer_grad_elems(const gt_pna_layer* layer);
int gt_pna_layer_fwd(const gt_pna_layer* layer, const void* x, void* y, void* saved, void* workspace, size_t workspace_bytes,
                     gt_stream_t stream);
int gt_pna_layer_bwd(const gt_pna_layer* layer, const void* x, const void* dy, const void* saved, void* dx, float* grads,
                     void* workspace, size_t workspace_bytes, gt_stream_t stream);
int gt_pna_scales(const int32_t* in_ptr, int64_t num_nodes, int num_scalers, const int32_t* kinds_host, float avg_log, float avg_lin,
                  float* scales, gt_stream_t stream);
int gt_gather_f32(float* dst, const float* src, const int32_t* map, int64_t n, gt_stream_t stream);
int gt_pna_aggregate_fwd_uv(const float* UV, const float* x, int64_t num_nodes, int64_t dim, int towers, const int32_t* in_ptr,
                            const int32_t* in_src, const int32_t* in_eid, float* in5, float* mean_v, int32_t* arg,
                            gt_stream_t stream);
int gt_pna_aggregate_bwd_uv(const float* UV, const float* in5, const float* mean_v, const int32_t* arg, const float* d_in5,
                            int64_t num_nodes, int64_t dim, int towers, const int32_t* in_ptr, const int32_t* out_ptr,
                            const int32_t* out_dst, const int32_t* out_eid, float* dUV, float* dxpart, gt_stream_t stream);

#define GT_MODEL_MAX_LAYERS 16
#define GT_MODEL_MAX_TABLES 16

typedef struct gt_image_set {
  int32_t n_jobs, n_bind;
  const float* const* job_w;
  const int64_t *job_N, *job_K;
  const int* job_T;
  void* const* job_img;
  const float* const* bind_w;
  const int64_t *bind_N, *bind_K;
  const void* const* bind_f;
  const void* const* bind_t;
} gt_image_set;

typedef struct gt_stage_ring {
  void* base;
  int64_t slot_bytes;
  int32_t slots, next;
  void* events[64];
} gt_stage_ring;

typedef struct gt_model {
  int32_t conv , L, n_enc, has_vn, jk_cat, residual;
  int32_t embed_kind , n_tables, vn0_in_embed, embed_sorted;
  int32_t with_cls, vn_defer_dw;
  int64_t D, d, Nh, ldy, ne_K, max_input_len, dw_overlap_min_elems;
  void* conv_layers;
  gt_vn_update* vn;
  gt_encoder_layer* enc;
  const float* tables[GT_MODEL_MAX_TABLES];
  int64_t table_rows[GT_MODEL_MAX_TABLES], table_clamp[GT_MODEL_MAX_TABLES];
  const float *vn_emb, *ne_w, *ne_b, *g2t_w, *g2t_b, *cls, *nin_w, *nin_b, *nout_w, *nout_b, *head_w, *head_b;
  const int64_t* zero_i64;
  float nin_eps, nout_eps;
  int64_t off_tables[GT_MODEL_MAX_TABLES], off_ne_w, off_ne_b, off_vn_emb, off_conv[GT_MODEL_MAX_LAYERS],
      off_vn[GT_MODEL_MAX_LAYERS], off_g2t_w, off_g2t_b, off_cls, off_nin_w, off_nin_b, off_enc[GT_MODEL_MAX_LAYERS],
      off_nout_w, off_nout_b, off_head_w, off_head_b, grad_total;
  void *st_vn, *st_dw, *st_prep;
  void *ev_x[GT_MODEL_MAX_LAYERS], *ev_vn[GT_MODEL_MAX_LAYERS], *ev_dvn[GT_MODEL_MAX_LAYERS], *ev_extra[GT_MODEL_MAX_LAYERS],
      *ev_pool[GT_MODEL_MAX_LAYERS];
  void *ev_vnemb, *ev_sort[2], *ev_wt[2], *ev_prep_begin, *ev_graph, *ev_w1;
  gt_image_set w3, w3_enc, w1;
  const float* pna_src;
  float* pna_img;
  const int32_t *pna_map, *pna_inv;
  int64_t pna_n_img, pna_n_src, off_pna_src;
// ... 92 lines not shown
```

Before: 76350 graphs/s.

## Fuse virtual-node segment-sum pooling into batchnorm apply epilogue of conv layers

The conv layer's batchnorm apply/broadcast pass now also sums its output rows per graph in chunks, writing complete per-graph sums straight into the next virtual-node update's saved input and partial head/tail sums into a workspace. The next virtual-node update then runs only the fixup kernel instead of re-reading the full node feature matrix for its segment sum. This removes a full N×D read per layer, at the cost of a more complex apply kernel with shared memory, an extra workspace, and a cross-layer dependency. An option flag keeps the separate path available.

```diff
diff --git a/graphtrans_amd/_lib.py b/graphtrans_amd/_lib.py
--- a/graphtrans_amd/_lib.py
+++ b/graphtrans_amd/_lib.py
@@ -55,6 +55,8 @@
     "gt_seq_layout_packed": (_i, [_p, _i64, _i64, _i, _p, _p, _p, _i64, _p, _p]),
     "gt_segment_sum_workspace_bytes": (_sz, [_i64, _i64]),
     "gt_segment_sum_ws": (_i, [_i, _p, _p, _p, _i64, _i64, _i64, _p, _p, _sz, _p]),
+    "gt_segment_sum_chunks": (_i, [_i, _p, _p, _p, _i64, _i64, _i64, _p, _p, _sz, _p]),
+    "gt_segment_sum_fixup": (_i, [_i, _p, _p, _i64, _i64, _i64, _p, _p, _sz, _p]),
     "gt_seq_gather": (_i, [_i, _p, _p, _p, _p, _i64, _i64, _i64, _i, _i64, _p, _p, _p]),
     "gt_seq_scatter": (_i, [_i, _p, _p, _p, _p, _p, _i64, _i64, _i, _i64, _i64, _p, _p, _p]),
     "gt_batchnorm_workspace_bytes": (_sz, [_i64, _i64]),
@@ -62,6 +64,8 @@
     "gt_batchnorm_apply": (_i, [_i, _p, _p, _p, _p, _p, _i, _p, _i64, _i64, _p, _f, _u64, _p]),
     "gt_batchnorm_bwd_apply": (_i, [_i, _p, _p, _p, _p, _p, _p, _p, _p, _d, _i, _i64, _i64, _p, _f, _u64, _p]),
     "gt_batchnorm_fwd_bcast": (_i, [_i, _p, _p, _p, _p, _p, _p, _f, _f, _i, _i, _p, _p, _p, _p, _i64, _i64, _p, _p, _p, _f, _u64, _p, _sz, _p]),
+    "gt_batchnorm_fwd_bcast_pool": (_i, [_i, _p, _p, _p, _p, _p, _p, _f, _f, _i, _i, _p, _p, _p, _p, _i64, _i64, _p, _p, _p, _f, _u64, _p, _sz,
+                                         _p, _i64, _p, _p, _p, _sz, _p]),
     "gt_batchnorm_bwd": (_i, [_i, _p, _p, _p, _p, _p, _p, _i, _i, _i64, _i64, _p, _p, _p, _f, _u64, _p, _sz, _p]),
     "gt_layernorm_fwd": (_i, [_i, _p, _p, _p, _p, _f, _f, _u64, _i64, _i64, _p, _p, _p, _p]),
     "gt_layernorm_bwd_workspace_bytes": (_sz, [_i64, _i64]),
@@ -160,6 +164,8 @@
     "gt_vn_update_workspace_bytes": (_sz, [_p]),
     "gt_vn_update_grad_elems": (_i64, [_p]),
     "gt_vn_update_fwd": (_i, [_p, _p, _p, _p, _p, _p, _sz, _p]),
+    "gt_vn_update_pool_out": (_p, [_p, _p]),
+    "gt_vn_update_fwd_pooled": (_i, [_p, _p, _p, _p, _p, _sz, _p, _sz, _p]),
     "gt_vn_update_bwd": (_i, [_p, _p, _p, _p, _p, _p, _p, _p, _sz, _p]),
     "gt_event_create": (_p, []),
     "gt_event_destroy": (None, [_p]),
diff --git a/graphtrans_amd/csrc/common.hip b/graphtrans_amd/csrc/common.hip
--- a/graphtrans_amd/csrc/common.hip
+++ b/graphtrans_amd/csrc/common.hip
@@ -57,7 +57,7 @@
 
 namespace {
 std::atomic<int> g_options[GT_OPT_COUNT];
-const char* const OPTION_NAMES[GT_OPT_COUNT] = {"attn_f32_exact", "bnstats_rows_kernel", "lin_ring"};
+const char* const OPTION_NAMES[GT_OPT_COUNT] = {"attn_f32_exact", "bnstats_rows_kernel", "lin_ring", "vn_pool_separate"};
 int option_id(const char* name) {
   if (name)
     for (int i = 0; i < GT_OPT_COUNT; ++i)
diff --git a/graphtrans_amd/csrc/gt_common.h b/graphtrans_amd/csrc/gt_common.h
--- a/graphtrans_amd/csrc/gt_common.h
+++ b/graphtrans_amd/csrc/gt_common.h
@@ -66,7 +66,7 @@
 enum { GT_PROF_AGGREGATE = 1, GT_PROF_ATTENTION = 2, GT_PROF_LINEAR = 4, GT_PROF_NORM = 8, GT_PROF_SEGMENT = 16,
        GT_PROF_GEMM_KERNEL = 32 };
 unsigned gt_prof_mask();
-enum { GT_OPT_ATTN_F32_EXACT = 0, GT_OPT_BNSTATS_ROWS_KERNEL = 1, GT_OPT_LIN_RING = 2, GT_OPT_COUNT };
+enum { GT_OPT_ATTN_F32_EXACT = 0, GT_OPT_BNSTATS_ROWS_KERNEL = 1, GT_OPT_LIN_RING = 2, GT_OPT_VN_POOL_SEPARATE = 3, GT_OPT_COUNT };
 int gt_opt(int id);
 int64_t gt_prof_begin(const char* name, hipStream_t stream, const int64_t* dims, int ndims);
 void gt_prof_end(int64_t id, hipStream_t stream);
@@ -81,6 +81,9 @@
 };
 
 static inline int64_t gt_cdiv(int64_t a, int64_t b) { return (a + b - 1) / b; }
+
+constexpr int GT_SEGSUM_CHUNK = 64;
+constexpr int64_t GT_SEGSUM_MIN_ROWS = 4096;
 
 typedef uint16_t gt_bf16;
 
diff --git a/graphtrans_amd/csrc/layers.hip b/graphtrans_amd/csrc/layers.hip
--- a/graphtrans_amd/csrc/layers.hip
+++ b/graphtrans_amd/csrc/layers.hip
@@ -470,6 +470,11 @@
   if (L->ev_graph_ready) GT_TRY(gt_stream_wait_event(st, L->ev_graph_ready));
   GT_TRY(gt_aggregate_fwd(GT_CONV_GCN, L->edge_mode, GT_F32, s.lin, L->N, L->E, L->D, L->in_ptr, L->in_src, L->in_eid, L->deg,
                           L->dis, L->root, L->edge_attr, L->edge_cols, L->edge_w, L->edge_b, L->tab_off, L->table_rows, nullptr, s.agg, st));
+  if (L->vn_next && L->pool_out)
+    return gt_batchnorm_fwd_bcast_pool(GT_F32, s.agg, L->bn_w, L->bn_b, L->bn_rm, L->bn_rv, L->training ? L->bn_nbt : nullptr,
+                                       L->bn_momentum, L->bn_eps, L->training, L->relu, L->residual ? x : nullptr, L->vn_next,
+                                       L->node_graph, L->ev_vn_next, L->N, L->D, y, s.stats, s.stats + L->D, L->dropout_p, L->seed,
+                                       w.bn_ws, w.bn_ws_bytes, L->graph_ptr, L->B, L->vn_next, L->pool_out, L->pool_ws, L->pool_ws_bytes, st);
   GT_TRY(gt_batchnorm_fwd_bcast(GT_F32, s.agg, L->bn_w, L->bn_b, L->bn_rm, L->bn_rv, L->training ? L->bn_nbt : nullptr,
                                 L->bn_momentum, L->bn_eps, L->training, L->relu, L->residual ? x : nullptr, L->vn_next,
                                 L->vn_next ? L->node_graph : nullptr, L->vn_next ? L->ev_vn_next : nullptr, L->N, L->D, y, s.stats,
@@ -514,20 +519,34 @@
 extern "C" size_t gt_vn_update_workspace_bytes(const gt_vn_update* L) { return L ? vn_work(L, nullptr).bytes : 0; }
 extern "C" int64_t gt_vn_update_grad_elems(const gt_vn_update* L) { return L ? 4 * L->D * L->D + 9 * L->D : 0; }
 
-extern "C" int gt_vn_update_fwd(const gt_vn_update* L, const void* x, const void* vn, void* vn_out, void* saved,
-                                void* workspace, size_t workspace_bytes, gt_stream_t st) {
-  GT_CHECK_ARG(L && x && vn && vn_out && saved && workspace, "null buffer");
-  GT_CHECK_ARG(L->D > 0 && L->D % 4 == 0 && L->B > 0, "bad sizes");
+static int vn_update_fwd(const char* fn, const gt_vn_update* L, const void* x, const void* vn, void* vn_out, void* saved, const void* pool_ws,
+                         size_t pool_ws_bytes, void* workspace, size_t workspace_bytes, gt_stream_t st) {
+  if (!(L && (x || pool_ws) && vn && vn_out && saved && workspace)) { gt_set_error("%s: null buffer", fn); return GT_ERR_INVALID_ARG; }
+  if (!(L->D > 0 && L->D % 4 == 0 && L->B > 0)) { gt_set_error("%s: bad sizes", fn); return GT_ERR_INVALID_ARG; }
   const VnWork w = vn_work(L, workspace);
-  if (workspace_bytes < w.bytes) { gt_set_error("gt_vn_update_fwd: workspace too small"); return GT_ERR_WORKSPACE; }
+  if (workspace_bytes < w.bytes) { gt_set_error("%s: workspace too small", fn); return GT_ERR_WORKSPACE; }
   const int64_t B = L->B, D = L->D;
   const Mlp2Saved s = mlp2_saved(B, D, saved);
-  GT_TRY(gt_segment_sum_ws(GT_F32, x, vn, L->graph_ptr, L->N, B, D, s.in, w.seg_ws, w.seg_ws_bytes, st));
+  if (x) GT_TRY(gt_segment_sum_ws(GT_F32, x, vn, L->graph_ptr, L->N, B, D, s.in, w.seg_ws, w.seg_ws_bytes, st));
+  else GT_TRY(gt_segment_sum_fixup(GT_F32, vn, L->graph_ptr, L->N, B, D, s.in, pool_ws, pool_ws_bytes, st));
   GT_TRY(mlp2_fwd_head(L, B, s, w.m.bn_ws, w.m.bn_ws_bytes, st));
   GT_TRY(gt_batchnorm_fwd(GT_F32, s.z2, L->bn2_w, L->bn2_b, L->bn2_rm, L->bn2_rv, L->training ? L->bn2_nbt : nullptr,
                           L->bn_momentum, L->bn_eps, L->training, 1, L->residual ? vn : nullptr, B, D, vn_out, s.st2,
                           s.st2 + D, L->dropout_p, L->seed, w.m.bn_ws, w.m.bn_ws_bytes, st));
   return GT_OK;
+}
+extern "C" int gt_vn_update_fwd(const gt_vn_update* L, const void* x, const void* vn, void* vn_out, void* saved,
+                                void* workspace, size_t workspace_bytes, gt_stream_t st) {
+  GT_CHECK_ARG(x, "null buffer");
+  return vn_update_fwd("gt_vn_update_fwd", L, x, vn, vn_out, saved, nullptr, 0, workspace, workspace_bytes, st);
+}
+extern "C" void* gt_vn_update_pool_out(const gt_vn_update* L, void* saved) {
+  return (L && saved) ? mlp2_saved(L->B, L->D, saved).in : nullptr;
+}
+extern "C" int gt_vn_update_fwd_pooled(const gt_vn_update* L, const void* vn, void* vn_out, void* saved, const void* pool_ws,
+                                       size_t pool_ws_bytes, void* workspace, size_t workspace_bytes, gt_stream_t st) {
+  GT_CHECK_ARG(pool_ws, "null buffer");
+  return vn_update_fwd("gt_vn_update_fwd_pooled", L, nullptr, vn, vn_out, saved, pool_ws, pool_ws_bytes, workspace, workspace_bytes, st);
 }
 
 extern "C" int gt_vn_update_bwd(const gt_vn_update* L, const void* d_vn_out, const void* saved, const void* d_x_add,
@@ -584,6 +603,11 @@
   GT_TRY(gt_aggregate_fwd(GT_CONV_GIN, L->edge_mode, GT_F32, x, N, L->E, D, L->in_ptr, L->in_src, L->in_eid, nullptr, nullptr,
                           L->eps, L->edge_attr, L->edge_cols, L->edge_w, L->edge_b, L->tab_off, L->table_rows, nullptr, s.in, st));
   GT_TRY(mlp2_fwd_head(L, N, s, w.m.bn_ws, w.m.bn_ws_bytes, st));
+  if (L->vn_next && L->pool_out)
+    return gt_batchnorm_fwd_bcast_pool(GT_F32, s.z2, L->bn_w, L->bn_b, L->bn_rm, L->bn_rv, L->training ? L->bn_nbt : nullptr, L->bn_momentum,
+                                       L->bn_eps, L->training, L->relu, L->residual ? x : nullptr, L->vn_next, L->node_graph, L->ev_vn_next,
+                                       N, D, y, s.st2, s.st2 + D, L->dropout_p, L->seed, w.m.bn_ws, w.m.bn_ws_bytes, L->graph_ptr, L->B,
+                                       L->vn_next, L->pool_out, L->pool_ws, L->pool_ws_bytes, st);
   GT_TRY(gt_batchnorm_fwd_bcast(GT_F32, s.z2, L->bn_w, L->bn_b, L->bn_rm, L->bn_rv, L->training ? L->bn_nbt : nullptr, L->bn_momentum,
                                 L->bn_eps, L->training, L->relu, L->residual ? x : nullptr, L->vn_next,
                                 L->vn_next ? L->node_graph : nullptr, L->vn_next ? L->ev_vn_next : nullptr, N, D, y, s.st2, s.st2 + D,
diff --git a/graphtrans_amd/csrc/model.hip b/graphtrans_amd/csrc/model.hip
--- a/graphtrans_amd/csrc/model.hip
+++ b/graphtrans_amd/csrc/model.hip
@@ -47,6 +47,8 @@
   size_t o_graph_ptr, o_node_graph, o_in_ptr, o_out_ptr, o_idx, o_dd, o_status, o_prep_ws, o_lay, o_lay_meta;
   size_t ws_bytes, ws2_bytes, eplan_bytes, esort_ws_bytes, prep_ws_bytes, arena_bytes;
   int cat2, want_wt, esort, late_wait;
+  int pool_fwd;
+  size_t o_poolws, poolws_bytes;
   int64_t Kc;
   char* base;
   const int32_t *graph_ptr, *node_graph, *seq_desc, *work_items;
@@ -248,6 +250,7 @@
     g.ev_dx_wait = (m->st_vn && m->has_vn && l < L - 1) ? m->ev_extra[l] : nullptr;
     g.x_has_vn = m->has_vn;
     g.vn_next = nullptr; g.ev_vn_next = nullptr;
+    g.pool_out = nullptr; g.pool_ws = nullptr; g.pool_ws_bytes = 0;
   };
   for (int l = 0; l < L; ++l) {
     if (m->conv == GT_CONV_GCN) {
@@ -349,6 +352,9 @@
   c->ws_bytes = ws; c->ws2_bytes = ws2;
   c->o_ws = a.take(ws);
   c->o_ws2 = a.take(ws2);
+  c->pool_fwd = (m->has_vn && m->conv != GT_CONV_PNA && nvn > 1 && N >= GT_SEGSUM_MIN_ROWS && !gt_opt(GT_OPT_VN_POOL_SEPARATE)) ? 1 : 0;
+  c->poolws_bytes = c->pool_fwd ? gt_segment_sum_workspace_bytes(N, D) : 0;
+  c->o_poolws = a.take(c->poolws_bytes);
   const bool have_imgs = b->use_w3 != 0;
   c->want_wt = (m->conv != GT_CONV_PNA && b->will_bwd && gt_compute_base(c->compute) == GT_F32 && N >= 1024 && (!have_imgs || (!m->has_vn && m->conv == GT_CONV_GCN))) ? 1 : 0;
   if (c->want_wt) {
@@ -644,15 +650,29 @@
       void* ev_next = (!last && side) ? m->ev_vn[l] : nullptr;
       if (m->conv == GT_CONV_GIN) { c->gin[l].vn_next = vn_next; c->gin[l].ev_vn_next = ev_next; }
       else { c->gcn[l].vn_next = vn_next; c->gcn[l].ev_vn_next = ev_next; }
+      const bool pool_out = c->pool_fwd && l + 1 < L - 1, pool_in = c->pool_fwd && l > 0;
+      {
+        void* po = pool_out ? gt_vn_update_pool_out(&c->vn[l + 1], P(c->o_vn_saved[l + 1])) : nullptr;
+        void* pw = pool_out ? P(c->o_poolws) : nullptr;
+        const size_t pb = pool_out ? c->poolws_bytes : 0;
+        if (m->conv == GT_CONV_GIN) { c->gin[l].pool_out = po; c->gin[l].pool_ws = pw; c->gin[l].pool_ws_bytes = pb; }
+        else { c->gcn[l].pool_out = po; c->gcn[l].pool_ws = pw; c->gcn[l].pool_ws_bytes = pb; }
+      }
+      auto vn_fwd = [&](void* ws, size_t ws_bytes, gt_stream_t s2) -> int {
+        if (pool_in)
+          return gt_vn_update_fwd_pooled(&c->vn[l], P(c->o_vn[l]), P(c->o_vn[l + 1]), P(c->o_vn_saved[l]), P(c->o_poolws), c->poolws_bytes, ws,
+                                         ws_bytes, s2);
+        return gt_vn_update_fwd(&c->vn[l], X(l), P(c->o_vn[l]), P(c->o_vn[l + 1]), P(c->o_vn_saved[l]), ws, ws_bytes, s2);
+      };
       if (l == 0 && !m->vn0_in_embed)
         GT_TRY(gt_segment_bcast_add(GT_F32, P(c->o_h[0]), P(c->o_vn[0]), node_graph, N, B, D, P(c->o_x0), st));
       if (!last && side) {
         GT_TRY(gt_event_record(m->ev_x[l], st));
         GT_TRY(gt_stream_wait_event(side, m->ev_x[l]));
-        GT_TRY(gt_vn_update_fwd(&c->vn[l], X(l), P(c->o_vn[l]), P(c->o_vn[l + 1]), P(c->o_vn_saved[l]), P(c->o_ws2), c->ws2_bytes, side));
+        GT_TRY(vn_fwd(P(c->o_ws2), c->ws2_bytes, side));
         GT_TRY(gt_event_record(m->ev_vn[l], side));
       } else if (!last) {
-        GT_TRY(gt_vn_update_fwd(&c->vn[l], X(l), P(c->o_vn[l]), P(c->o_vn[l + 1]), P(c->o_vn_saved[l]), P(c->o_ws), c->ws_bytes, st));
+        GT_TRY(vn_fwd(P(c->o_ws), c->ws_bytes, st));
       }
       GT_TRY(conv_fwd(l, X(l), P(c->o_vn[l]), P(c->o_h[l + 1])));
     } else {
diff --git a/graphtrans_amd/csrc/norm.hip b/graphtrans_amd/csrc/norm.hip
--- a/graphtrans_amd/csrc/norm.hip
+++ b/graphtrans_amd/csrc/norm.hip
@@ -295,6 +295,107 @@
   return t;
 }
 
+constexpr int POOL_NT = 512, POOL_SUB = 16, POOL_TILE = 512, POOL_U = 4;
+static_assert(POOL_SUB * POOL_TILE / 4 <= POOL_NT * POOL_U, "a slab is one trip of the block");
+template <typename T>
+__device__ __forceinline__ float4 bn_stored4(float4 v) {
+  if constexpr (sizeof(T) == 4) {
+    return v;
+  } else {
+    const uint32_t lo = gt_pack_bf16(v.x, v.y), hi = gt_pack_bf16(v.z, v.w);
+    return make_float4(__uint_as_float(lo << 16), __uint_as_float(lo & 0xffff0000u), __uint_as_float(hi << 16),
+                       __uint_as_float(hi & 0xffff0000u));
+  }
+}
+
+template <typename T>
+__global__ void __launch_bounds__(POOL_NT) k_bn_apply_pool(const T* __restrict__ x, const float* __restrict__ mean,
+                                                           const float* __restrict__ rstd, const float* __restrict__ w,
+                                                           const float* __restrict__ b, const T* __restrict__ resid, int relu,
+                                                           BnDrop drop, int64_t N, int64_t D, T* __restrict__ y,
+                                                           const T* __restrict__ bcast, const int32_t* __restrict__ bidx,
+                                                           const int32_t* __restrict__ gptr, int B, const T* __restrict__ add,
+                                                           T* __restrict__ pool, float* __restrict__ head, float* __restrict__ tail) {
+  extern __shared__ __attribute__((aligned(16))) float sy[];
+  const int64_t p0 = (int64_t)blockIdx.x * GT_SEGSUM_CHUNK;
+  const int64_t p1 = p0 + GT_SEGSUM_CHUNK < N ? p0 + GT_SEGSUM_CHUNK : N;
+  if (p0 >= p1) return;
+  int lo = 0, hi = B;
+  while (hi - lo > 1) {
+    const int mid = (lo + hi) >> 1;
+    if (gptr[mid] <= p0) lo = mid; else hi = mid;
+  }
+  const int g0 = lo;
+  float* hd = head + (int64_t)blockIdx.x * D;
+  float* tl = tail + (int64_t)blockIdx.x * D;
+  for (int64_t ct = 0; ct < D; ct += POOL_TILE) {
+    const int tw = (int)(D - ct < POOL_TILE ? D - ct : POOL_TILE), tc4 = tw / 4;
+    const bool owner = (int)threadIdx.x < tw;
+    const int64_t col = ct + threadIdx.x;
+    int g = g0;
+    int64_t gend = gptr[g + 1];
+    float acc = 0.f;
+    auto flush = [&](int gg, float v) {
+      const bool before = gptr[gg] < p0, after = (int64_t)gptr[gg + 1] > p1;
+      if (before) hd[col] = v;
+      else if (after) tl[col] = v;
+      else st1<T>(pool + (int64_t)gg * D + col, v + (add ? ld1<T>(add + (int64_t)gg * D + col) : 0.f));
+    };
+    float4 v[POOL_U], rv[POOL_U], bv[POOL_U];
+    auto load = [&](int64_t s0) {
+      const int nr = (int)(p1 - s0 < POOL_SUB ? p1 - s0 : POOL_SUB), items = nr * tc4;
+#pragma unroll
+      for (int u = 0; u < POOL_U; ++u) {
+        const int i = threadIdx.x + u * POOL_NT;
+        if (i < items) {
+          const int64_t r = s0 + i / tc4, c = ct + (int64_t)(i % tc4) * 4;
+          v[u] = gt_load4<T>(x + r * D + c);
+          if (resid) rv[u] = gt_load4<T>(resid + r * D + c);
+          if (bcast) bv[u] = gt_load4<T>(bcast + (int64_t)bidx[r] * D + c);
+        }
+      }
+    };
+    load(p0);
+    for (int64_t s0 = p0; s0 < p1; s0 += POOL_SUB) {
+      const int nr = (int)(p1 - s0 < POOL_SUB ? p1 - s0 : POOL_SUB), items = nr * tc4;
+#pragma unroll
+      for (int u = 0; u < POOL_U; ++u) {
+        const int i = threadIdx.x + u * POOL_NT;
+        if (i < items) {
+          const int lr = i / tc4, lc = (i % tc4) * 4;
+          const int64_t r = s0 + lr, c = ct + lc;
+          const float4 mu = *reinterpret_cast<const float4*>(mean + c), rs = *reinterpret_cast<const float4*>(rstd + c);
+          const float4 ww = *reinterpret_cast<const float4*>(w + c), bb = *reinterpret_cast<const float4*>(b + c);
+          float4 t = v[u];
+          t = make_float4((t.x - mu.x) * rs.x * ww.x + bb.x, (t.y - mu.y) * rs.y * ww.y + bb.y,
+                          (t.z - mu.z) * rs.z * ww.z + bb.z, (t.w - mu.w) * rs.w * ww.w + bb.w);
+          if (relu) t = gt_relu4(t);
+          if (drop.thr) t = bn_drop4(t, drop, (uint32_t)r, (uint32_t)c);
+          if (resid) t = gt_add4(t, rv[u]);
+          if (bcast) t = gt_add4(t, bv[u]);
+          gt_store4<T>(y + r * D + c, t);
+          *reinterpret_cast<float4*>(sy + lr * tw + lc) = bn_stored4<T>(t);
+        }
+      }
+      __syncthreads();
+      if (s0 + POOL_SUB < p1) load(s0 + POOL_SUB);
+      if (owner) {
+        for (int lr = 0; lr < nr; ++lr) {
+          const int64_t r = s0 + lr;
+          if (r == gend) {
+            flush(g, acc);
+            acc = 0.f;
+            do { ++g; gend = gptr[g + 1]; } while (gend <= r);
+          }
+          acc += sy[lr * tw + threadIdx.x];
+        }
+      }
+      __syncthreads();
+    }
+    if (owner) flush(g, acc);
+  }
+}
+
 template <typename T>
 __global__ void __launch_bounds__(SM_COLS * SM_LANES) k_bn_small_fwd(
     const T* __restrict__ x, int64_t N, int64_t D, float eps, float momentum, const float* __restrict__ w,
@@ -924,12 +1025,21 @@
                                 workspace_bytes, stream_);
 }
 
-extern "C" int gt_batchnorm_fwd_bcast(int dtype, const void* x, const float* weight, const float* bias,
-                                      float* running_mean, float* running_var, int64_t* num_batches_tracked,
-                                      float momentum, float eps, int training, int relu, const void* resid,
-                                      const void* bcast, const int32_t* bcast_index, void* ev_bcast_ready, int64_t rows,
-                                      int64_t dim, void* y, float* save_mean, float* save_rstd, float dropout_p,
-                                      uint64_t seed, void* workspace, size_t workspace_bytes, gt_stream_t stream_) {
+struct BnPool {
+  const int32_t* graph_ptr;
+  int64_t B;
+  const void* add;
+  void* out;
+  void* ws;
+  size_t ws_bytes;
+};
+
+static int bn_fwd_impl(int dtype, const void* x, const float* weight, const float* bias,
+                       float* running_mean, float* running_var, int64_t* num_batches_tracked,
+                       float momentum, float eps, int training, int relu, const void* resid,
+                       const void* bcast, const int32_t* bcast_index, void* ev_bcast_ready, int64_t rows,
+                       int64_t dim, void* y, float* save_mean, float* save_rstd, float dropout_p,
+                       uint64_t seed, void* workspace, size_t workspace_bytes, const BnPool* pool, gt_stream_t stream_) {
   int rc = check_norm("gt_batchnorm_fwd", dtype, rows, dim);
   GT_CHECK_ARG(!bcast || bcast_index, "bcast needs bcast_index");
 
@@ -958,6 +1068,7 @@
                            dim, eps, momentum, weight, bias, (const gt_bf16*)resid, relu, drop, save_mean, save_rstd,
                            running_mean, running_var, num_batches_tracked, (gt_bf16*)y, (const gt_bf16*)bcast, bcast_index);
       GT_CHECK_LAUNCH();
+      if (pool) return gt_segment_sum_chunks(dtype, y, pool->add, pool->graph_ptr, rows, pool->B, dim, pool->out, pool->ws, pool->ws_bytes, stream_);
       return GT_OK;
     }
     const int nb = part_blocks(rows);
@@ -1003,6 +1114,22 @@
     rc = gt_stream_wait_event(stream_, ev_bcast_ready);
     if (rc) return rc;
   }
+  if (pool) {
+    const int64_t nch = gt_cdiv(rows, GT_SEGSUM_CHUNK);
+    float* head = static_cast<float*>(pool->ws);
+    float* tail = head + nch * dim;
+    const size_t lds = (size_t)POOL_SUB * (dim < POOL_TILE ? dim : POOL_TILE) * sizeof(float);
+    if (dtype == GT_F32)
+      hipLaunchKernelGGL(k_bn_apply_pool<float>, dim3((unsigned)nch), dim3(POOL_NT), lds, stream, (const float*)x, save_mean, save_rstd, weight,
+                         bias, (const float*)resid, relu, drop, rows, dim, (float*)y, (const float*)bcast, bcast_index, pool->graph_ptr,
+                         (int)pool->B, (const float*)pool->add, (float*)pool->out, head, tail);
+    else
+      hipLaunchKernelGGL(k_bn_apply_pool<gt_bf16>, dim3((unsigned)nch), dim3(POOL_NT), lds, stream, (const gt_bf16*)x, save_mean, save_rstd,
+                         weight, bias, (const gt_bf16*)resid, relu, drop, rows, dim, (gt_bf16*)y, (const gt_bf16*)bcast, bcast_index,
+                         pool->graph_ptr, (int)pool->B, (const gt_bf16*)pool->add, (gt_bf16*)pool->out, head, tail);
+    GT_CHECK_LAUNCH();
+    return GT_OK;
+  }
   if (dtype == GT_F32)
     hipLaunchKernelGGL(k_bn_apply<float>, dim3(g), dim3(NT), 0, stream, (const float*)x, save_mean, save_rstd, weight,
                        bias, (const float*)resid, relu, drop, rows, dim, (float*)y, (const float*)bcast, bcast_index);
@@ -1011,6 +1138,34 @@
                        bias, (const gt_bf16*)resid, relu, drop, rows, dim, (gt_bf16*)y, (const gt_bf16*)bcast, bcast_index);
   GT_CHECK_LAUNCH();
   return GT_OK;
+}
+
+extern "C" int gt_batchnorm_fwd_bcast(int dtype, const void* x, const float* weight, const float* bias,
+                                      float* running_mean, float* running_var, int64_t* num_batches_tracked,
+                                      float momentum, float eps, int training, int relu, const void* resid,
+                                      const void* bcast, const int32_t* bcast_index, void* ev_bcast_ready, int64_t rows,
+                                      int64_t dim, void* y, float* save_mean, float* save_rstd, float dropout_p,
+                                      uint64_t seed, void* workspace, size_t workspace_bytes, gt_stream_t stream_) {
+  return bn_fwd_impl(dtype, x, weight, bias, running_mean, running_var, num_batches_tracked, momentum, eps, training, relu, resid, bcast,
+                     bcast_index, ev_bcast_ready, rows, dim, y, save_mean, save_rstd, dropout_p, seed, workspace, workspace_bytes, nullptr,
+                     stream_);
+}
+
+extern "C" int gt_batchnorm_fwd_bcast_pool(int dtype, const void* x, const float* weight, const float* bias,
+                                           float* running_mean, float* running_var, int64_t* num_batches_tracked,
+                                           float momentum, float eps, int training, int relu, const void* resid,
+                                           const void* bcast, const int32_t* bcast_index, void* ev_bcast_ready, int64_t rows,
+                                           int64_t dim, void* y, float* save_mean, float* save_rstd, float dropout_p,
+                                           uint64_t seed, void* workspace, size_t workspace_bytes, const int32_t* graph_ptr,
+                                           int64_t num_graphs, const void* pool_add, void* pool_out, void* pool_ws,
+                                           size_t pool_ws_bytes, gt_stream_t stream_) {
+  GT_CHECK_ARG(graph_ptr && pool_out && pool_ws, "null pool buffer");
+  GT_CHECK_ARG(num_graphs > 0 && num_graphs <= 0x7fffffff && rows <= 0x7fffffff, "bad pool sizes");
+  GT_CHECK_ARG(dim > 0 && pool_ws_bytes >= gt_segment_sum_workspace_bytes(rows, dim), "pool workspace too small");
+  const BnPool pool{graph_ptr, num_graphs, pool_add, pool_out, pool_ws, pool_ws_bytes};
+  return bn_fwd_impl(dtype, x, weight, bias, running_mean, running_var, num_batches_tracked, momentum, eps, training, relu, resid, bcast,
+                     bcast_index, ev_bcast_ready, rows, dim, y, save_mean, save_rstd, dropout_p, seed, workspace, workspace_bytes, &pool,
+                     stream_);
 }
 
 extern "C" int gt_batchnorm_bwd(int dtype, const void* x, const void* dy, const float* weight, const float* bias,
diff --git a/graphtrans_amd/csrc/segment.hip b/graphtrans_amd/csrc/segment.hip
--- a/graphtrans_amd/csrc/segment.hip
+++ b/graphtrans_amd/csrc/segment.hip
@@ -49,7 +49,7 @@
   }
 }
 
-constexpr int SS_CH = 64, SS_T = 320;
+constexpr int SS_CH = GT_SEGSUM_CHUNK, SS_T = 320;
 
 template <typename T>
 __device__ __forceinline__ float ldf(const T* p) {
@@ -467,32 +467,56 @@
   return (size_t)2 * gt_cdiv(N > 0 ? N : 1, SS_CH) * D * sizeof(float) + 256;
 }
 
-extern "C" int gt_segment_sum_ws(int dtype, const void* x, const void* add, const int32_t* graph_ptr, int64_t N, int64_t B,
-                                 int64_t D, void* out, void* workspace, size_t workspace_bytes, gt_stream_t stream_) {
-  if (N < 4096 || !workspace || workspace_bytes < gt_segment_sum_workspace_bytes(N, D))
-    return gt_segment_sum(dtype, x, add, graph_ptr, N, B, D, out, stream_);
-  int rc = check("gt_segment_sum_ws", dtype, D);
-  if (rc) return rc;
-  GT_CHECK_ARG(x && graph_ptr && out, "null buffer");
-  if (B == 0) return GT_OK;
+extern "C" int gt_segment_sum_chunks(int dtype, const void* x, const void* add, const int32_t* graph_ptr, int64_t N, int64_t B, int64_t D,
+                                     void* out, void* workspace, size_t workspace_bytes, gt_stream_t stream_) {
+  int rc = check("gt_segment_sum_chunks", dtype, D);
+  if (rc) return rc;
+  GT_CHECK_ARG(x && graph_ptr && out && workspace, "null buffer");
+  GT_CHECK_ARG(workspace_bytes >= gt_segment_sum_workspace_bytes(N, D), "workspace too small");
+  if (B == 0 || N == 0) return GT_OK;
   GT_CHECK_ARG(B <= 0x7fffffff && N <= 0x7fffffff, "sizes beyond int32");
   hipStream_t stream = (hipStream_t)stream_;
   const int64_t nch = gt_cdiv(N, SS_CH);
   float* head = static_cast<float*>(workspace);
   float* tail = head + nch * D;
-  if (dtype == GT_F32) {
+  if (dtype == GT_F32)
     hipLaunchKernelGGL(k_segsum_chunks<float>, dim3((unsigned)nch), dim3(SS_T), 0, stream, (const float*)x, (const float*)add,
                        graph_ptr, (int)B, N, D, (float*)out, head, tail);
-    hipLaunchKernelGGL(k_segsum_fixup<float>, dim3((unsigned)B), dim3(SS_T), 0, stream, (const float*)add, graph_ptr, D,
-                       (const float*)head, (const float*)tail, (float*)out);
-  } else {
+  else
     hipLaunchKernelGGL(k_segsum_chunks<gt_bf16>, dim3((unsigned)nch), dim3(SS_T), 0, stream, (const gt_bf16*)x,
                        (const gt_bf16*)add, graph_ptr, (int)B, N, D, (gt_bf16*)out, head, tail);
-    hipLaunchKernelGGL(k_segsum_fixup<gt_bf16>, dim3((unsigned)B), dim3(SS_T), 0, stream, (const gt_bf16*)add, graph_ptr, D,
-                       (const float*)head, (const float*)tail, (gt_bf16*)out);
-  }
-  GT_CHECK_LAUNCH();
-  return GT_OK;
+  GT_CHECK_LAUNCH();
+  return GT_OK;
+}
+
+extern "C" int gt_segment_sum_fixup(int dtype, const void* add, const int32_t* graph_ptr, int64_t N, int64_t B, int64_t D, void* out,
+                                    const void* workspace, size_t workspace_bytes, gt_stream_t stream_) {
+  int rc = check("gt_segment_sum_fixup", dtype, D);
+  if (rc) return rc;
+  GT_CHECK_ARG(graph_ptr && out && workspace, "null buffer");
+  GT_CHECK_ARG(workspace_bytes >= gt_segment_sum_workspace_bytes(N, D), "workspace too small");
+  if (B == 0) return GT_OK;
+  GT_CHECK_ARG(B <= 0x7fffffff && N <= 0x7fffffff, "sizes beyond int32");
+  hipStream_t stream = (hipStream_t)stream_;
+  const float* head = static_cast<const float*>(workspace);
+  const float* tail = head + gt_cdiv(N, SS_CH) * D;
+  if (dtype == GT_F32)
+    hipLaunchKernelGGL(k_segsum_fixup<float>, dim3((unsigned)B), dim3(SS_T), 0, stream, (const float*)add, graph_ptr, D, head, tail,
+                       (float*)out);
+  else
+    hipLaunchKernelGGL(k_segsum_fixup<gt_bf16>, dim3((unsigned)B), dim3(SS_T), 0, stream, (const gt_bf16*)add, graph_ptr, D, head, tail,
+                       (gt_bf16*)out);
+  GT_CHECK_LAUNCH();
+  return GT_OK;
+}
+
+extern "C" int gt_segment_sum_ws(int dtype, const void* x, const void* add, const int32_t* graph_ptr, int64_t N, int64_t B,
+                                 int64_t D, void* out, void* workspace, size_t workspace_bytes, gt_stream_t stream_) {
+  if (N < GT_SEGSUM_MIN_ROWS || !workspace || workspace_bytes < gt_segment_sum_workspace_bytes(N, D))
+    return gt_segment_sum(dtype, x, add, graph_ptr, N, B, D, out, stream_);
+  int rc = gt_segment_sum_chunks(dtype, x, add, graph_ptr, N, B, D, out, workspace, workspace_bytes, stream_);
+  if (rc) return rc;
+  return gt_segment_sum_fixup(dtype, add, graph_ptr, N, B, D, out, workspace, workspace_bytes, stream_);
 }
 
 __global__ void __launch_bounds__(1024) k_seq_layout_packed(const int32_t* __restrict__ gptr, int B, int max_len, int cls,
diff --git a/graphtrans_amd/layers.py b/graphtrans_amd/layers.py
--- a/graphtrans_amd/layers.py
+++ b/graphtrans_amd/layers.py
@@ -31,7 +31,7 @@
                [("seed", C.c_uint64), ("dropout_p", C.c_float), ("x_has_vn", C.c_int32), ("vn_next", _fp), ("ev_vn_next", _fp),
                 ("lin_wt", _fp), ("prev_saved", _fp), ("prev_bn_w", _fp), ("prev_bn_b", _fp), ("prev_bn_part", _fp),
                 ("bn_part_in", _fp), ("prev_relu", C.c_int32), ("bn_nparts_in", C.c_int32), ("ev_graph_ready", _fp),
-                ("dx_bcast", _fp), ("dx_bcast_idx", _fp)]
+                ("dx_bcast", _fp), ("dx_bcast_idx", _fp), ("pool_out", _fp), ("pool_ws", _fp), ("pool_ws_bytes", C.c_size_t)]
 
 
 class GinLayerDesc(C.Structure):
@@ -45,7 +45,7 @@
                                    "bn_b", "bn1_rm", "bn1_rv", "bn_rm", "bn_rv", "bn1_nbt", "bn_nbt", "ev_x_ready",
                                    "ev_dx_wait")] + \
                [("seed", C.c_uint64), ("dropout_p", C.c_float), ("x_has_vn", C.c_int32), ("vn_next", _fp), ("ev_vn_next", _fp),
-                ("w1_t", _fp), ("w2_t", _fp)]
+                ("w1_t", _fp), ("w2_t", _fp), ("pool_out", _fp), ("pool_ws", _fp), ("pool_ws_bytes", C.c_size_t)]
 
 
 class VnUpdateDesc(C.Structure):
diff --git a/include/graphtrans_hip.h b/include/graphtrans_hip.h
--- a/include/graphtrans_hip.h
+++ b/include/graphtrans_hip.h
@@ -142,6 +142,11 @@
 int gt_segment_sum_ws(int dtype, const void* x, const void* add, const int32_t* graph_ptr, int64_t num_nodes,
                       int64_t num_graphs, int64_t dim, void* out, void* workspace, size_t workspace_bytes,
                       gt_stream_t stream);
+int gt_segment_sum_chunks(int dtype, const void* x, const void* add, const int32_t* graph_ptr, int64_t num_nodes,
+                          int64_t num_graphs, int64_t dim, void* out, void* workspace, size_t workspace_bytes,
+                          gt_stream_t stream);
+int gt_segment_sum_fixup(int dtype, const void* add, const int32_t* graph_ptr, int64_t num_nodes, int64_t num_graphs,
+                         int64_t dim, void* out, const void* workspace, size_t workspace_bytes, gt_stream_t stream);
 
 int gt_seq_gather(int dtype, const void* h, const void* cls, const int32_t* graph_ptr, const int32_t* seq_desc,
                   int64_t num_seqs, int64_t row_stride, int64_t max_npos, int with_cls, int64_t dim,
@@ -182,6 +187,13 @@
                            int relu, const void* resid, const void* bcast, const int32_t* bcast_index, void* ev_bcast_ready,
                            int64_t rows, int64_t dim, void* y, float* save_mean, float* save_rstd, float dropout_p,
                            uint64_t seed, void* workspace, size_t workspace_bytes, gt_stream_t stream);
+int gt_batchnorm_fwd_bcast_pool(int dtype, const void* x, const float* weight, const float* bias, float* running_mean,
+                                float* running_var, int64_t* num_batches_tracked, float momentum, float eps, int training,
+                                int relu, const void* resid, const void* bcast, const int32_t* bcast_index, void* ev_bcast_ready,
+                                int64_t rows, int64_t dim, void* y, float* save_mean, float* save_rstd, float dropout_p,
+                                uint64_t seed, void* workspace, size_t workspace_bytes, const int32_t* graph_ptr,
+                                int64_t num_graphs, const void* pool_add, void* pool_out, void* pool_ws, size_t pool_ws_bytes,
+                                gt_stream_t stream);
 int gt_batchnorm_bwd(int dtype, const void* x, const void* dy, const float* weight, const float* bias,
                      const float* save_mean, const float* save_rstd, int training, int relu, int64_t rows,
                      int64_t dim, void* dx, float* dweight, float* dbias, float dropout_p, uint64_t seed, void* workspace,
@@ -391,6 +403,8 @@
   void* ev_graph_ready;
   const float* dx_bcast;
   const int32_t* dx_bcast_idx;
+  void *pool_out, *pool_ws;
+  size_t pool_ws_bytes;
 } gt_gcn_layer;
 size_t gt_gcn_layer_saved_bytes(const gt_gcn_layer* layer);
 size_t gt_gcn_layer_workspace_bytes(const gt_gcn_layer* layer);
@@ -419,6 +433,8 @@
   const void* vn_next;
   void* ev_vn_next;
   const float *w1_t, *w2_t;
+  void *pool_out, *pool_ws;
+  size_t pool_ws_bytes;
 } gt_gin_layer;
 size_t gt_gin_layer_saved_bytes(const gt_gin_layer* layer);
 size_t gt_gin_layer_workspace_bytes(const gt_gin_layer* layer);
@@ -447,6 +463,9 @@
 int64_t gt_vn_update_grad_elems(const gt_vn_update* layer);
 int gt_vn_update_fwd(const gt_vn_update* layer, const void* x, const void* vn, void* vn_out, void* saved,
                      void* workspace, size_t workspace_bytes, gt_stream_t stream);
+void* gt_vn_update_pool_out(const gt_vn_update* layer, void* saved);
+int gt_vn_update_fwd_pooled(const gt_vn_update* layer, const void* vn, void* vn_out, void* saved, const void* pool_ws,
+                            size_t pool_ws_bytes, void* workspace, size_t workspace_bytes, gt_stream_t stream);
 int gt_vn_update_bwd(const gt_vn_update* layer, const void* d_vn_out, const void* saved, const void* d_x_add, void* d_x,
                      void* d_vn, float* grads, void* workspace, size_t workspace_bytes, gt_stream_t stream);
 const float* gt_vn_update_bwd_dt0(const gt_vn_update* L, void* workspace);
```

Result: slower. 75390 graphs/s (-1.3%).
